# alenxav/bWGR

Measured on AMD Instinct MI355X. Metric: MCMC iter/sec (full marker sweep), higher is better.
Workload: dtype f32 scalars, fixed-point / f64 residual, int8 genotypes; 1 GPU; c4: synthetic n=10000 x p=1000000 int8, BayesB pi=0.99 (1.2% of the markers in the model at the last sweep), exact chain (blocked sweep, block=128, 40 slabs x 256 rows + 1 sequencer, the chain alone on the GPU: 80 streamers x 128 rows, engine generation 3, lag 12 blocks); n=10000, p=1000000, model=BayesB, df=5, chains=1

## Files before the change

### bwgr_amd/csrc/bwgr_hip.hip

```cpp
#include <hip/hip_runtime.h>
#include <stdint.h>
#include <stdio.h>
#include <stdarg.h>
#include <string.h>
#include <math.h>
#include <vector>
#include <random>
#include <chrono>
#include <algorithm>
#include <mutex>
#include <atomic>
#include <memory>
#include <utility>
#include <type_traits>
#include "../../include/bwgr.h"
#include "devbufs.h"
#include "traits.h"
#include "rng.hip.h"
#include "sweep.hip.h"
#include "sweep3.hip.h"
#include "sweep2w.hip.h"
#include "sweep3p.hip.h"
#include "mrr.hip.h"
#include "uvb.hip.h"
// ... 544 lines not shown
    const uint4 v0 = *reinterpret_cast<const uint4 *>(base + (size_t)j * R), v1 = *reinterpret_cast<const uint4 *>(base + (size_t)(j + 1) * R);
    const uint4 v2 = *reinterpret_cast<const uint4 *>(base + (size_t)(j + 2) * R), v3 = *reinterpret_cast<const uint4 *>(base + (size_t)(j + 3) * R);
    const double c0 = (double)coef[j], c1 = (double)coef[j + 1], c2 = (double)coef[j + 2], c3 = (double)coef[j + 3];
    GEMV_COL(v0, c0) GEMV_COL(v1, c1) GEMV_COL(v2, c2) GEMV_COL(v3, c3)
  }
  for (; j < jb; ++j) { const uint4 v0 = *reinterpret_cast<const uint4 *>(base + (size_t)j * R); const double c0 = (double)coef[j]; GEMV_COL(v0, c0) }
#undef GEMV_COL
#undef GEMV_ADD
  double *o = part + (int64_t)c * ld + i0;
#pragma unroll
  for (int k = 0; k < 16; ++k) o[k] = acc[k];
}
__global__ void k_hat_finish(const double *part, int64_t ld, int nchunks, int n, float MU, float *hat, const double *cen_off = nullptr) {
  const int i = blockIdx.x * blockDim.x + threadIdx.x;
  if (i >= n) return;
  double s = cen_off ? -*cen_off : 0.0;
  for (int c = 0; c < nchunks; ++c) s += part[(int64_t)c * ld + i];
  const float f = (float)s;
  hat[i] = f + MU;
}


struct WgrScalars {
  double mu, Ve, Va, Sb, Se, MSx, vy, bb, B0, VE, VA, sumD, cxx;
  double Vp, VP, Sk;
};
template <typename XT>
__global__ void k_stats64(const XT *X, int R, int n, int p, double *xx, double *vx) {
  const int lane = threadIdx.x & 63;
  const int64_t j = (int64_t)blockIdx.x * (blockDim.x >> 6) + (threadIdx.x >> 6);
  if (j >= p) return;
  double s1 = 0, s2 = 0;
  for (int i = lane; i < n; i += 64) { const double v = (double)xval(X, xoff(i, j, R, p)); s1 += v; s2 = fma(v, v, s2); }
  s1 = wave_sum(s1); s2 = wave_sum(s2);
  s1 = __shfl(s1, 0, 64); s2 = __shfl(s2, 0, 64);
  const double mean = s1 / (double)n;
  double sv = 0;
  for (int i = lane; i < n; i += 64) { const double dev = (double)xval(X, xoff(i, j, R, p)) - mean; sv = fma(dev, dev, sv); }
  sv = wave_sum(sv);
  if (lane == 0) { xx[j] = s2; vx[j] = sv / (double)(n - 1); }
}
__global__ void k_dsum_stage1(const double *v, int64_t n, double *part, int square) {
  __shared__ double red[17];
  double s = 0;
  for (int64_t i = (int64_t)blockIdx.x * blockDim.x + threadIdx.x; i < n; i += (int64_t)gridDim.x * blockDim.x) s += square ? v[i] * v[i] : v[i];
  s = block_sum(s, red);
  if (threadIdx.x == 0) part[blockIdx.x] = s;
}
__global__ void k_wgr_init(const double *y, double *eR, int n, int64_t ld, const double *part, const double *part2, int p,
                           double df, double R2, WgrScalars *ws) {
  __shared__ double red[17];
  double s = 0;
  for (int i = threadIdx.x; i < n; i += blockDim.x) s += y[i];
  s = block_sum(s, red);
  const double mu = s / (double)n;
  double sv = 0;
  for (int i = threadIdx.x; i < n; i += blockDim.x) { const double dev = y[i] - mu; sv += dev * dev; }
  sv = block_sum(sv, red);
  double ms = 0, sx = 0;
  for (int i = threadIdx.x; i < 256; i += blockDim.x) { ms += part[i]; sx += part2[i]; }
  ms = block_sum(ms, red);
  sx = block_sum(sx, red);
  for (int64_t i = threadIdx.x; i < ld; i += blockDim.x) eR[i] = (i < n) ? (y[i] - mu) : 0.0;
  if (threadIdx.x == 0) {
    WgrScalars w; memset(&w, 0, sizeof(w));
    w.mu = mu; w.vy = sv / (double)(n - 1); w.MSx = ms; w.Ve = 1.0; w.Va = ms;
    w.Sb = (R2) * df * w.vy / ms; w.Se = (1 - R2) * df * w.vy; w.cxx = sx / (double)p;
    w.Sk = R2 * w.vy * (df + 2); w.Vp = 1.0;
    *ws = w;
  }
}
__global__ void k_wgr_marker_init(double *bR, double *dR, double *VbR, double *LR, double *B, double *D, double *VB, int p, const WgrScalars *ws) {
  const double Va = ws->Va, Ve = ws->Ve;
  for (int j = blockIdx.x * blockDim.x + threadIdx.x; j < p; j += gridDim.x * blockDim.x) {
    bR[j] = 0; dR[j] = 1; VbR[j] = Va; LR[j] = Va / Ve; B[j] = 0; D[j] = 0; VB[j] = 0;
  }
}
__global__ void k_wgr_pre(const double *bR, const double *dR, const double *LR, const double *xx64, const double *eR, float *bf, float *df_,
                          float *Lf, float *xxf, double *e64, int p, int n, int64_t ld, float pi, const WgrScalars *ws, ChainScalars *sc) {
  const int64_t gid = (int64_t)blockIdx.x * blockDim.x + threadIdx.x, gsz = (int64_t)gridDim.x * blockDim.x;
  for (int64_t j = gid; j < p; j += gsz) { bf[j] = (float)bR[j]; df_[j] = (float)dR[j]; Lf[j] = (float)LR[j]; xxf[j] = (float)xx64[j]; }
  for (int64_t i = gid; i < ld; i += gsz) e64[i] = (i < n) ? (double)(float)eR[i] : 0.0;
  if (gid == 0) {
    ChainScalars c; memset(&c, 0, sizeof(c));
    const float Ve = (float)ws->Ve;
    c.ve = Ve; c.pi = pi; c.C = -0.5f / sqrtf(Ve); c.odds = pi / (1.0f - pi); c.dfp1 = 1.0f;
    c.inc_rate = 1.0f - pi;
    c.nredo = sc->nredo;
    *sc = c;
  }
}
__global__ void k_wgr_post(const float *bf, const float *df_, double *bR, double *dR, double *VbR, int p, int use_d, int iv, int de,
                           double dfv, uint32_t iter, Rng rng, const WgrScalars *ws) {
  const double Sb = ws->Sb, Ve = ws->Ve, MSx = ws->MSx;
  for (int j = blockIdx.x * blockDim.x + threadIdx.x; j < p; j += gridDim.x * blockDim.x) {
    const double b = (double)bf[j];
    bR[j] = b;
    if (use_d) dR[j] = (double)df_[j];
    if (iv) VbR[j] = de ? sqrt(b * b * Ve / MSx) : (Sb + b * b) / rng_chisq(rng, dfv + 1.0, (uint32_t)j, iter, RNG_CHI);
  }
}
__global__ __launch_bounds__(1024) void k_wgr_scal(const double *e64, int n, double n_dof, int p, const double *bbpart, int iv, double dfv, uint32_t iter, Rng rng, WgrScalars *ws) {
  __shared__ double red[17];
  double ee = 0;
  for (int i = threadIdx.x; i < n; i += blockDim.x) { const double v = (double)(float)e64[i]; ee += v * v; }
  ee = block_sum(ee, red);
  double bb = 0;
  for (int i = threadIdx.x; i < 256; i += blockDim.x) bb += bbpart[i];
  bb = block_sum(bb, red);
  if (threadIdx.x == 0) {
    if (!iv) ws->Va = (bb + ws->Sb) / rng_chisq(rng, dfv + (double)p, RNG_GLOBAL_MARKER, iter, RNG_G_VB);
    ws->Ve = (ee + ws->Se) / rng_chisq(rng, n_dof + dfv, RNG_GLOBAL_MARKER, iter, RNG_G_VE);
    ws->bb = bb;
  }
}
__global__ void k_wgr_L(const double *bR, const double *dR, double *VbR, double *LR, double *B, double *D, double *VB, int p, int iv, int accumulate, const WgrScalars *ws) {
  const double Ve = ws->Ve, Va = ws->Va;
  for (int j = blockIdx.x * blockDim.x + threadIdx.x; j < p; j += gridDim.x * blockDim.x) {
    if (!iv) VbR[j] = Va;
    LR[j] = Ve / VbR[j];
    if (accumulate) { B[j] += bR[j]; D[j] += dR[j]; if (iv) VB[j] += VbR[j]; }
  }
}
__global__ void k_wgr_efinish(const double *part, int64_t ld, int nchunks, int n, const double *y, double *eR, const WgrScalars *ws) {
  const int i = blockIdx.x * blockDim.x + threadIdx.x;
  if (i >= n) return;
  double s = 0;
  for (int c = 0; c < nchunks; ++c) s += part[(int64_t)c * ld + i];
  eR[i] = y[i] - ws->mu - s;
}
__global__ __launch_bounds__(1024) void k_wgr_mu(double *eR, int n, int iv, int accumulate, uint32_t iter, Rng rng, WgrScalars *ws) {
  __shared__ double red[17];
  double s = 0;
  for (int i = threadIdx.x; i < n; i += blockDim.x) s += eR[i];
  s = block_sum(s, red);
  const double mu0 = s / (double)n + (ws->Ve / (double)n) * rng_normal(rng, RNG_GLOBAL_MARKER, iter, RNG_G_MU, 0);
  for (int i = threadIdx.x; i < n; i += blockDim.x) eR[i] -= mu0;
  __syncthreads();
  if (threadIdx.x == 0) {
    ws->mu += mu0;
    if (accumulate) { ws->B0 += ws->mu; ws->VE += ws->Ve; if (!iv) ws->VA += ws->Va; }
  }
}
__global__ void k_wgr_pre_k(const double *hR, const double *Vd, const double *eR, float *hf, float *dhf, float *xxKf, float *Lkf, double *e64,
                            int pk, int n, int64_t ld, const WgrScalars *ws, ChainScalars *sc) {
  const int64_t gid = (int64_t)blockIdx.x * blockDim.x + threadIdx.x, gsz = (int64_t)gridDim.x * blockDim.x;
  const double Ve = ws->Ve, Vp = ws->Vp;
  for (int64_t k = gid; k < pk; k += gsz) { hf[k] = (float)hR[k]; dhf[k] = 0.0f; xxKf[k] = 1.0f; Lkf[k] = (float)(Ve / (Vd[k] * Vp)); }
  for (int64_t i = gid; i < ld; i += gsz) e64[i] = (i < n) ? (double)(float)eR[i] : 0.0;
  if (gid == 0) {
    ChainScalars c; memset(&c, 0, sizeof(c));
    const float Vef = (float)Ve;
    c.ve = Vef; c.pi = 0.0f; c.C = -0.5f / sqrtf(Vef); c.odds = 0.0f; c.dfp1 = 1.0f;
    *sc = c;
  }
}
__global__ void k_wgr_post_k(const float *hf, double *hR, const double *e64, double *eR, int pk, int n) {
  const int64_t gid = (int64_t)blockIdx.x * blockDim.x + threadIdx.x, gsz = (int64_t)gridDim.x * blockDim.x;
  for (int64_t k = gid; k < pk; k += gsz) hR[k] = (double)hf[k];
  for (int64_t i = gid; i < n; i += gsz) eR[i] = (double)(float)e64[i];
}
__global__ __launch_bounds__(1024) void k_wgr_vp(const double *hR, const double *Vd, int pk, double dfv, uint32_t iter, Rng rng, WgrScalars *ws) {
  __shared__ double red[17];
  double s = 0;
  for (int k = threadIdx.x; k < pk; k += blockDim.x) s += hR[k] * hR[k] / Vd[k];
  s = block_sum(s, red);
  if (threadIdx.x == 0) ws->Vp = (s + ws->Sk) / rng_chisq(rng, dfv + (double)pk, RNG_GLOBAL_MARKER, iter, RNG_G_VK);
}
__global__ void k_uh(const double *Ud, const double *coef, int n, int pk, double scale, double *out, int accumulate_into_neg) {
  const int i = blockIdx.x * blockDim.x + threadIdx.x;
  if (i >= n) return;
  double s = 0;
  for (int k = 0; k < pk; ++k) s = fma(Ud[(size_t)k * n + i], coef[k] * scale, s);
  if (accumulate_into_neg) out[i] -= s; else out[i] = s;
}
__global__ void k_wgr_accum_k(const double *hR, double *H, int pk, WgrScalars *ws) {
  for (int k = blockIdx.x * blockDim.x + threadIdx.x; k < pk; k += gridDim.x * blockDim.x) H[k] += hR[k];
  if (blockIdx.x == 0 && threadIdx.x == 0) ws->VP += ws->Vp;
}
__global__ void k_add_vec(double *a, const double *b, int n) {
  const int i = blockIdx.x * blockDim.x + threadIdx.x;
  if (i < n) a[i] += b[i];
}
template <typename XT>
__global__ void k_gather_rows(const XT *Xb, int Rb, const int *use, int nb, XT *Xo, int Ro, int64_t ldo, int64_t p) {
  const int64_t total = p * ldo;
  for (int64_t idx = (int64_t)blockIdx.x * blockDim.x + threadIdx.x; idx < total; idx += (int64_t)gridDim.x * blockDim.x) {
    const int64_t j = idx / ldo, i = idx - j * ldo;
    XT v = (XT)0;
    if (i < nb) v = Xb[xoff(use[i], j, Rb, p)];
    Xo[xoff(i, j, Ro, p)] = v;
  }
}
__global__ __launch_bounds__(256) void k_gather_rows_i8(const int8_t *Xb, int Rb, int64_t ldb, const int *use, int nb, int8_t *Xo, int Ro,
                                                         int64_t ldo, int64_t p, int mpw) {
  extern __shared__ __attribute__((aligned(16))) unsigned char col[];
  const int64_t j0 = (int64_t)blockIdx.x * mpw;
  const int nm = (int)min((int64_t)mpw, p - j0);
  const int cin = (int)(ldb / 16), cout = (int)(ldo / 16);
  for (int c = threadIdx.x; c < nm * cin; c += 256) {
    const int jj = c / cin, ci = c - jj * cin;
    const int64_t i = 16 * (int64_t)ci;
    reinterpret_cast<uint4 *>(col + (size_t)jj * ldb)[ci] = *reinterpret_cast<const uint4 *>(Xb + xoff(i, j0 + jj, Rb, p));
  }
  __syncthreads();
  for (int co = threadIdx.x; co < cout; co += 256) {
    int ui[16];
#pragma unroll
    for (int k = 0; k < 16; ++k) { const int i = 16 * co + k; ui[k] = (i < nb) ? use[i] : -1; }
    for (int jj = 0; jj < nm; ++jj) {
      const unsigned char *cj = col + (size_t)jj * ldb;
      uint32_t w[4];
#pragma unroll
      for (int q = 0; q < 4; ++q) {
        uint32_t v = 0;
#pragma unroll
        for (int k = 0; k < 4; ++k) { const int u = ui[4 * q + k]; v |= ((u >= 0) ? (uint32_t)cj[u] : 0u) << (8 * k); }
        w[q] = v;
      }
      *reinterpret_cast<uint4 *>(Xo + xoff(16 * (int64_t)co, j0 + jj, Ro, p)) = make_uint4(w[0], w[1], w[2], w[3]);
    }
  }
}
__global__ void k_gather_e(const double *eR, const int *use, int nb, int64_t ldo, double *e64) {
  for (int64_t i = (int64_t)blockIdx.x * blockDim.x + threadIdx.x; i < ldo; i += (int64_t)gridDim.x * blockDim.x)
    e64[i] = (i < nb) ? (double)(float)eR[use[i]] : 0.0;
}
__global__ void k_scale_d(double *v, int64_t n, double s) {
  for (int64_t i = (int64_t)blockIdx.x * blockDim.x + threadIdx.x; i < n; i += (int64_t)gridDim.x * blockDim.x) v[i] *= s;
}
__global__ void k_set_bg(ChainScalars *sc, float bg) { sc->bg = bg; }
__global__ void k_wgr_final(double *B, double *D, double *VB, int p, double mc, const double *dpart, int iv, WgrScalars *ws) {
  __shared__ double red[17];
  double sd = 0;
  for (int i = threadIdx.x; i < 256; i += blockDim.x) sd += dpart[i];
  sd = block_sum(sd, red);
  const double meanD = sd / mc / (double)p;
  for (int j = threadIdx.x; j < p; j += blockDim.x) { D[j] = D[j] / mc; B[j] = B[j] / mc / meanD; if (iv) VB[j] = VB[j] / mc; }
  if (threadIdx.x == 0) ws->sumD = sd;
}
__global__ void k_hat64_finish(const double *part, int64_t ld, int nchunks, int n, double B0, double *hat) {
  const int i = blockIdx.x * blockDim.x + threadIdx.x;
  if (i >= n) return;
  double s = 0;
  for (int c = 0; c < nchunks; ++c) s += part[(int64_t)c * ld + i];
  hat[i] = B0 + s;
}

__global__ void k_synth(int8_t *X, int64_t ld, int n, int64_t p, int64_t col0, uint32_t k0, uint32_t k1, float *freq) {
  const int64_t quads = ld / 4;
  const int64_t total = p * quads;
  for (int64_t idx = (int64_t)blockIdx.x * blockDim.x + threadIdx.x; idx < total; idx += (int64_t)gridDim.x * blockDim.x) {
    const int64_t j = idx / quads, q = idx - j * quads;
    const uint32_t jg = (uint32_t)(col0 + j);
    const uint4 fj = philox4x32_10(jg, 0u, 33u, 0u, k0, k1);
    const float f = 0.05f + 0.45f * ((float)(fj.x >> 8) * (1.0f / 16777216.0f));
    const uint32_t thr = (uint32_t)(f * 16777216.0f);
    if (q == 0 && freq) freq[j] = f;
    const uint4 a = philox4x32_10((uint32_t)q, jg, 32u, 0u, k0, k1);
    const uint4 c = philox4x32_10((uint32_t)q, jg, 32u, 1u, k0, k1);
    const uint32_t w[8] = {a.x, a.y, a.z, a.w, c.x, c.y, c.z, c.w};
    uint32_t packed = 0;
#pragma unroll
    for (int r = 0; r < 4; ++r) {
      uint32_t g = ((w[2 * r] >> 8) < thr) + ((w[2 * r + 1] >> 8) < thr);
      if (q * 4 + r >= n) g = 0;
      packed |= g << (8 * r);
    }
    *reinterpret_cast<uint32_t *>(X + j * ld + q * 4) = packed;
  }
}

__global__ void k_debug_variates(Rng g, int kind, double nu, uint32_t marker0, uint32_t iter, uint32_t purpose, int count, double *out) {
  const int i = blockIdx.x * blockDim.x + threadIdx.x;
  if (i >= count) return;
  const uint32_t mk = marker0 + (uint32_t)i;
  double v;
  if (kind == 0) v = rng_normal(g, mk, iter, purpose, 0);
  else if (kind == 1) v = rng_uniform(g, mk, iter, purpose, 0);
  else v = rng_chisq(g, nu, mk, iter, purpose);
  out[i] = v;
}

}

namespace {
struct SnapArgs { double *e, *se; float *b, *d, *vb, *sb, *sd, *svb; int64_t ld; int j0, j1; ChainScalars *sc; };
__global__ void k_range_snapshot(const SnapArgs s) {
  const int64_t nt = (int64_t)gridDim.x * blockDim.x, t0 = (int64_t)blockIdx.x * blockDim.x + threadIdx.x;
  for (int64_t i = t0; i < s.ld; i += nt) s.se[i] = s.e[i];
  for (int64_t j = s.j0 + t0; j < s.j1; j += nt) { s.sb[j] = s.b[j]; s.sd[j] = s.d[j]; if (s.vb) s.svb[j] = s.vb[j]; }
  if (t0 == 0) { s.sc->snap_sum_d = s.sc->sum_d; s.sc->snap_sum_b2 = s.sc->sum_b2; }
}
__global__ void k_range_recover(const SnapArgs s) {
  if (s.sc->error != 2u) return;
  const int64_t nt = (int64_t)gridDim.x * blockDim.x, t0 = (int64_t)blockIdx.x * blockDim.x + threadIdx.x;
  for (int64_t i = t0; i < s.ld; i += nt) s.e[i] = s.se[i];
  for (int64_t j = s.j0 + t0; j < s.j1; j += nt) { s.b[j] = s.sb[j]; s.d[j] = s.sd[j]; if (s.vb) s.vb[j] = s.svb[j]; }
}
__global__ void k_range_flag(ChainScalars *sc) {
  if (sc->error == 2u) { sc->error = 0u; sc->redo = 1u; sc->nredo += 1u; sc->sum_d = sc->snap_sum_d; sc->sum_b2 = sc->snap_sum_b2; }
}
__global__ void k_redo_clear(ChainScalars *sc) { sc->redo = 0u; }
}

struct Switches {
  int sweep = -1, lag = -1, solo3 = -1, stream3 = -1, pf3 = -1;
  int r3 = 0, d3 = 0, nfeed = 0, sh_add = 0, max_concurrent = 0, max_pairs = 0;
  float eng3_thr = 0.03f;
  bool occ_guard = true, pf3b = true, draws = true, gram16 = true;
  bool winv = true, wfx = true;
#ifdef BWGR_EXPERIMENTS
  bool fixed3 = false;
#else
  bool fixed3 = true;
#endif
  int wpf = 4, wahead = 5, wnq = 0, wlag_cap = 4;
  bool group_allow_uncentred = false, group_force_comm = false, em_debug = false;
  int64_t kchunk = 0;
#ifdef BWGR_EXPERIMENTS
  int dbg3 = 0, dbgw = 0, wlag_timing = 0; bool no_recover = false;
#endif
};
static Switches read_switches() {
  const auto chr = [](const char *v) { return v ? (int)(unsigned char)v[0] : -1; };
  const auto num = [](const char *v) { return v ? atoi(v) : 0; };
  Switches s;
  s.sweep = chr(getenv("BWGR_SWEEP")); s.lag = chr(getenv("BWGR_LAG")); s.solo3 = chr(getenv("BWGR_SOLO3"));
  s.stream3 = chr(getenv("BWGR_STREAM3")); s.pf3 = chr(getenv("BWGR_PF3"));
  s.r3 = num(getenv("BWGR_R3")); s.d3 = num(getenv("BWGR_D3")); s.nfeed = num(getenv("BWGR_NFEED")); s.sh_add = num(getenv("BWGR_DEBUG_SH_ADD"));
  s.max_concurrent = num(getenv("BWGR_MAX_CONCURRENT")); s.max_pairs = num(getenv("BWGR_MAX_PAIRS"));
  if (const char *v = getenv("BWGR_ENG3_THR")) { const float t = (float)atof(v); if (t > 0.0f) s.eng3_thr = t; }
  s.occ_guard = chr(getenv("BWGR_OCC_GUARD")) != '0'; s.pf3b = chr(getenv("BWGR_PF3B")) != '0'; s.draws = chr(getenv("BWGR_DRAWS")) != '0';
  s.gram16 = chr(getenv("BWGR_GRAM16")) != '0';
  { const int c = chr(getenv("BWGR_FIXED3")); if (c == '0') s.fixed3 = false; else if (c == '1') s.fixed3 = true; }
  s.winv = chr(getenv("BWGR_WINV")) != '0'; s.wfx = chr(getenv("BWGR_WFX")) != '0';
  if (const char *v = getenv("BWGR_WPF")) s.wpf = std::max(0, std::min(8, atoi(v)));
  if (const char *v = getenv("BWGR_WAHEAD")) s.wahead = std::max(1, atoi(v));
  { const int v = num(getenv("BWGR_WNQ")), c = chr(getenv("BWGR_WLAG")); if (v == 1 || v == 2 || v == 4) s.wnq = v; if (c >= '2' && c <= '6') s.wlag_cap = c - '0'; }
  s.group_allow_uncentred = chr(getenv("BWGR_GROUP_ALLOW_UNCENTRED")) == '1'; s.group_force_comm = chr(getenv("BWGR_GROUP_FORCE_COMM")) == '1';
  s.em_debug = getenv("BWGR_EM_DEBUG") != nullptr;
  if (const char *v = getenv("BWGR_KCHUNK")) s.kchunk = std::max<long long>(0, atoll(v));
#ifdef BWGR_EXPERIMENTS
  s.dbg3 = num(getenv("BWGR_DBG3")); s.dbgw = num(getenv("BWGR_DBGW")); s.wlag_timing = num(getenv("BWGR_WLAG_TIMING"));
  s.no_recover = getenv("BWGR_NO_RECOVER") != nullptr;
#endif
  return s;
}

enum PanelKind { PANEL_MAIN = 0, PANEL_ROWS = 1, PANEL_EM = 2 };
struct PanelPlan {
  int m = 0, K = 0, R = 0;
  int64_t ld = 0, nblocks = 0;
  int pstride = 0, nfeed = 2;
  bool lag4_ok = false;
  size_t lds = 0, lds2 = 0, ldsw = 0;
  size_t x_bytes = 0, gram_bytes = 0;
  bool pipelined = false;
  int xdist = 1;
  bool has16 = false;
  int wdist = 0;
  bool try3 = false;
};
template <typename XT> static int max_slab_rows(int m) {
  int best = 0;
  for (int R = 128; R <= 4096; R += 128)
    if (sweep_lds_bytes<XT>(m, R) <= (size_t)160 * 1024 && (size_t)m * R * sizeof(XT) <= (size_t)SW_TCH * 16 * (SW_THREADS - 64)) best = R;
  return best;
}
static int panel_range(int64_t n, int64_t p) {
  if (n < 2 || p < 1) return fail(BWGR_EINVAL, "panel: need n >= 2, p >= 1 (n=%lld p=%lld)", (long long)n, (long long)p);
  if (n > 0x7FFFFF00ll || p > 0x7FFFFF00ll) return fail(BWGR_EINVAL, "panel: n and p must fit 31 bits");
  return BWGR_OK;
}
static int plan_panel(PanelPlan &pl, bool is_f32, int64_t n, int64_t p, int block, int nwg, PanelKind kind, const Switches &sw) {
  pl = PanelPlan();
  CHK(panel_range(n, p));
  const auto lds2_of = [&](int m, int R) { return is_f32 ? sweep2_lds_bytes<float>(m, R) : sweep2_lds_bytes<int8_t>(m, R); };
  const int mmax = is_f32 ? 64 : SW_MAXM;
  int m = block > 0 ? block : mmax;
  if (m > mmax) return fail(BWGR_EINVAL, "panel_create: block %d > %d (limit for this genotype type)", m, mmax);
  m = ((int)std::min<int64_t>(m, ((p + 15) / 16) * 16) + 15) / 16 * 16;
  const int Rmax = is_f32 ? max_slab_rows<float>(m) : max_slab_rows<int8_t>(m);
  int Rpick = Rmax, R2 = 0;
  for (int Rt = 128; Rt <= Rmax; Rt += 128)
    if (lds2_of(m, Rt) <= (size_t)160 * 1024 && (is_f32 || (size_t)m * Rt <= S2I_TILE_BYTES_MAX)) R2 = Rt;
  if (sw.sweep != '1' && R2 > 0 && (n + R2 - 1) / R2 + 1 + 6 <= 256) Rpick = R2;
  const int K = nwg > 0 ? nwg : (int)((n + Rpick - 1) / Rpick);
  const int R = (int)((((n + K - 1) / K) + 127) / 128) * 128;
  if (K > 256 || R > Rmax) return fail(BWGR_EINVAL, "panel_create: n=%lld needs %d slab workgroups of %d rows (limits: 256 workgroups, %d rows)", (long long)n, K, R, Rmax);
  pl.m = m; pl.K = K; pl.R = R; pl.ld = (int64_t)K * R;
  pl.nblocks = (p + m - 1) / m;
  if (pl.nblocks >= (1ll << 24)) return fail(BWGR_EINVAL, "panel_create: %lld marker blocks; the delta granules carry a 24-bit block epoch", (long long)pl.nblocks);
  pl.pstride = ((m * (m - 1) / 2 + 7) / 8) * 8;
  pl.lds = is_f32 ? sweep_lds_bytes<float>(m, R) : sweep_lds_bytes<int8_t>(m, R);
  pl.lds2 = lds2_of(m, R);
  pl.lag4_ok = !is_f32 && s2i_lds_bytes(m, R, 4) <= (size_t)160 * 1024;
  if (pl.lag4_ok) pl.lds2 = std::max(pl.lds2, s2i_lds_bytes(m, R, 4));
#ifdef BWGR_EXPERIMENTS
  if (!is_f32) pl.ldsw = s2w_lds_bytes(m, R, sw.wlag_timing ? sw.wlag_timing : 6);
#else
  if (!is_f32) pl.ldsw = s2w_lds_bytes(m, R, 6);
#endif
  pl.nfeed = std::min(6, std::max(2, (K + 39) / 40 + 1));
  if (sw.nfeed >= 1 && sw.nfeed <= 6) pl.nfeed = sw.nfeed;
  pl.pipelined = sw.sweep != '1' && pl.lds2 <= (size_t)160 * 1024 && K + 1 + pl.nfeed <= 256 && (is_f32 || (size_t)m * R <= S2I_TILE_BYTES_MAX);
  pl.x_bytes = (size_t)pl.ld * (size_t)p * (is_f32 ? 4 : 1);
  pl.gram_bytes = (size_t)pl.nblocks * m * m * (is_f32 ? 8 : 4);
  if (pl.pipelined && kind != PANEL_EM) {
    if (pl.nblocks > 2) pl.xdist = 2;
    if (!is_f32 && pl.nblocks > 3 && pl.lag4_ok && sw.lag != '2' && sw.lag != '3') pl.xdist = 3;
    pl.has16 = !is_f32;
  }
  if (pl.has16 && sw.winv && m <= SW_MAXM)
    for (int d = 1; d <= S2W_MAXDIST && d < pl.nblocks; ++d) {
      if (d <= S2W_NEARD ? d > pl.xdist : (kind != PANEL_MAIN || d > sw.wlag_cap - 1)) break;
      pl.wdist = d;
    }
  pl.try3 = kind == PANEL_MAIN && !is_f32 && pl.pipelined && sw.sweep != '2';
  return BWGR_OK;
}

struct Panel3Plan {
  bool fits = false;
  int R3 = 0, sub3 = 0, K3 = 0;
  int D = 0;
  size_t lds3 = 0;
  bool solo3 = true;
};
static Panel3Plan plan_panel3(const PanelPlan &pp, const Switches &sw, bool gram16) {
  Panel3Plan q;
  if (!pp.try3) return q;
  q.R3 = (pp.R % 256 == 0) ? 256 : 128;
  if ((sw.r3 == 64 || sw.r3 == 128 || sw.r3 == 256) && pp.R % sw.r3 == 0) { q.R3 = sw.r3; q.solo3 = false; }
  q.sub3 = pp.R / q.R3; q.K3 = pp.K * q.sub3;
  q.D = 12;
  if (sw.d3 >= 2 && sw.d3 <= S3_MAXD) q.D = sw.d3;
  q.D = (int)std::min<int64_t>(q.D, std::max<int64_t>(2, pp.nblocks));
  q.lds3 = std::max(std::max(s3_streamer_lds(q.R3), std::max(s3_streamer_dma_lds(128), q.R3 == 256 ? s3_streamer_dma_lds(256) : (size_t)0)), s3_seq_lds(q.D, gram16));
  q.fits = q.K3 <= 255 && q.lds3 <= (size_t)160 * 1024 && (size_t)pp.m * q.R3 <= (size_t)4 * 16 * SW_THREADS;
  if (q.fits && sw.solo3 >= 0) q.solo3 = sw.solo3 != '0';
  return q;
}

extern "C" int bwgr_debug_panel_plan(int is_f32, int64_t n, int64_t p, int block, int nwg, int kind, int xmax, int gram16, int64_t out[BWGR_PANEL_PLAN_NOUT]) {
  if (!out || kind < PANEL_MAIN || kind > PANEL_EM) return fail(BWGR_EINVAL, "debug_panel_plan: null pointer or bad kind");
  const Switches sw = read_switches();
  PanelPlan pl;
  CHK(plan_panel(pl, is_f32 != 0, n, p, block, nwg, (PanelKind)kind, sw));
  const Panel3Plan q = xmax >= 0 ? plan_panel3(pl, sw, gram16 != 0) : Panel3Plan();
  const int64_t v[BWGR_PANEL_PLAN_NOUT] = {pl.m, pl.K, pl.R, pl.ld, pl.nblocks, pl.pstride, pl.nfeed, pl.lag4_ok, (int64_t)pl.lds, (int64_t)pl.lds2, (int64_t)pl.ldsw,
                                           (int64_t)pl.x_bytes, (int64_t)pl.gram_bytes, pl.pipelined, pl.xdist, pl.has16, pl.wdist, pl.try3,
                                           q.fits, q.R3, q.sub3, q.K3, q.D, (int64_t)q.lds3, q.solo3};
  std::copy(v, v + BWGR_PANEL_PLAN_NOUT, out);
  return BWGR_OK;
}

namespace {
struct HipBackend {
  using stream_t = hipStream_t;
  using event_t = hipEvent_t;
  static inline std::atomic<int64_t> live[3];
  static inline thread_local hipError_t last = hipSuccess;
  static void *alloc(size_t bytes) {
    void *q = nullptr;
    const hipError_t e = hipMalloc(&q, bytes);
    if (e != hipSuccess) { last = e; (void)hipGetLastError(); return nullptr; }
    ++live[0];
    return q;
  }
  static void free(void *q) { (void)hipFree(q); --live[0]; }
  static bool stream_create(hipStream_t *s, unsigned flags, int priority) {
    if ((priority ? hipStreamCreateWithPriority(s, flags, priority) : hipStreamCreateWithFlags(s, flags)) != hipSuccess) { (void)hipGetLastError(); return false; }
    ++live[1];
    return true;
  }
  static void stream_sync(hipStream_t s) { (void)hipStreamSynchronize(s); }
  static void stream_destroy(hipStream_t s) { (void)hipStreamDestroy(s); --live[1]; }
  static bool event_create(hipEvent_t *e, unsigned flags) {
    if (hipEventCreateWithFlags(e, flags) != hipSuccess) { (void)hipGetLastError(); return false; }
    ++live[2];
    return true;
  }
  static void event_destroy(hipEvent_t e) { (void)hipEventDestroy(e); --live[2]; }
};
using DevBufs = DevHolder<HipBackend>;
template <typename F> struct Guard {
  F f;
  bool armed = true;
  explicit Guard(F f_) : f(f_) {}
  Guard(const Guard &) = delete;
  ~Guard() { if (armed) f(); }
  void release() { armed = false; }
};
}
extern "C" int bwgr_debug_live(int64_t out[3]) {
  if (!out) return fail(BWGR_EINVAL, "debug_live: null pointer");
  for (int i = 0; i < 3; ++i) out[i] = HipBackend::live[i].load();
  return BWGR_OK;
}
static int no_memory(const char *who) { return fail(BWGR_ENOMEM, "%s: device allocation failed (%s)", who, hipGetErrorString(HipBackend::last)); }
template <typename T> static int own_array(DevBufs &own, T *&ptr, size_t count, const char *who) {
  return (ptr = own.get<std::conditional_t<std::is_void<T>::value, unsigned char, T>>(count)) ? BWGR_OK : no_memory(who);
}

struct PanelData {
  DevBufs own;
  int device = 0, is_f32 = 0;
  int64_t n = 0, p = 0;
  PanelPlan plan;
  Panel3Plan plan3;
  float MSx = 0;
  int xmax = 0;
  bool gram16 = false;
  int winv_nd = 0;
  bool e3_ready = false;
  bool crowded = false;
  void *X = nullptr, *gram = nullptr, *gramp = nullptr;
  void *gx[S2W_NEARD + 1] = {};
  uint16_t *gramp16 = nullptr, *gramx16 = nullptr;
  int *gram16_bad = nullptr;
  void *g3x[S3_MAXD] = {};
  unsigned char *gx12 = nullptr;
  unsigned char *gxt[S2W_MAXDIST] = {};
  float *xx = nullptr, *vx = nullptr, *msx_dev = nullptr;
  int *xmax_dev = nullptr;
  bool cen = false;
  int32_t *csum = nullptr; float *xxc = nullptr;
  Switches sw;
  int nclones = 0;
  int nchains_all = 0;
  std::vector<hipStream_t> pair_streams;
};

struct bwgr_panel {
  PanelData *data = nullptr;
  bool is_root = false;
  DevBufs own;
  hipStream_t stream = nullptr;
  hipStream_t pre_pair_stream = nullptr; bool pre_pair_set = false;
  double *xspec2 = nullptr, *xspec3 = nullptr;
  PreStage ps = {};
  const void *ps_owner = nullptr; int ps_iter = -1;
  double *xpart = nullptr, *qpart = nullptr;
  unsigned long long *dgran = nullptr;
  uint32_t *xflags = nullptr;
  unsigned char *xchg = nullptr; size_t xchg_bytes = 0;
  unsigned long long *stamps = nullptr;
  unsigned long long *qsum3 = nullptr, *lists3 = nullptr;
  uint32_t epoch3 = 0;
  double *snap_e = nullptr; float *snap_b = nullptr, *snap_d = nullptr, *snap_vb = nullptr;
  double *winv = nullptr;
  unsigned long long *qsumw = nullptr;
  double *cpre = nullptr;
  double *draws = nullptr; hipStream_t draws_stream = nullptr; hipEvent_t draws_ready = nullptr, draws_free = nullptr;
  bool draws_valid = false; Rng draws_rng = {}; uint32_t draws_iter = 0, draws_marker0 = 0; int draws_flags = 0, draws_j0 = 0, draws_j1 = 0; const void *draws_sc = nullptr;
  hipEvent_t guard_ev = nullptr; int guard_cus = 0; hipStream_t guard_stream = nullptr; bool guard_listed = false;
  bool force3 = false;
  int debug_withhold = 0;
  int nchains = 0;
};

struct bwgr_chain {
  bwgr_panel *P = nullptr;
  DevBufs own;
  int model = 0, iit = 0, ibi = 0, done = 0, rng_mode = 0;
  float itf = 0, bif = 0, pi = 0, df = 0, R2 = 0, Phi = 0;
  uint64_t seed = 0;
  float *y = nullptr, *b = nullptr, *d = nullptr, *vb = nullptr, *lam = nullptr;
  double *e = nullptr;
  float *B = nullptr, *D = nullptr, *VB = nullptr;
  ChainScalars *sc = nullptr;
  int64_t marker0 = 0, p_total = 0;
  float MSx_eff = 0;
  double *e0 = nullptr;
  int flags_extra = 0;
  std::vector<hipEvent_t> ev;
  float ms_acc = 0; int launch_acc = 0;
  bool finalized = false;
};

__attribute__((constructor)) static void bwgr_more_hw_queues() { setenv("GPU_MAX_HW_QUEUES", "8", 0); }

static hipError_t d2h(hipStream_t st, void *dst, const void *src, size_t bytes) {
  hipError_t e = hipMemcpyAsync(dst, src, bytes, hipMemcpyDeviceToHost, st);
  return e != hipSuccess ? e : hipStreamSynchronize(st);
}
template <typename T> static hipError_t h2d(hipStream_t st, T *dst, const T *src, size_t count) { return hipMemcpyAsync(dst, src, sizeof(T) * count, hipMemcpyHostToDevice, st); }
template <typename T> static hipError_t zero(hipStream_t st, T *dst, size_t count) { return hipMemsetAsync(dst, 0, sizeof(T) * count, st); }

static Rng make_rng(uint64_t seed, int mode) {
  Rng g; g.k0 = (uint32_t)seed; g.k1 = (uint32_t)(seed >> 32); g.degenerate = (mode == BWGR_RNG_DEGENERATE); return g;
}

static int sum_floats(hipStream_t st, const float *v, int64_t n, double *part, float *sum_dev, float *sum) {
  hipLaunchKernelGGL(k_sum_stage1, dim3(256), dim3(256), 0, st, v, n, part);
  hipLaunchKernelGGL(k_sum_stage2, dim3(1), dim3(256), 0, st, part, 256, sum_dev);
  HIPCHK(hipGetLastError());
  HIPCHK(d2h(st, sum, sum_dev, sizeof(float)));
  return BWGR_OK;
}

static int refuse_centred(const char *who) {
  return fail(BWGR_EINVAL, "%s: this panel sweeps implicitly centred columns (bwgr_panel_set_centred), which only the fused chains do; call bwgr_panel_set_centred(P, 0) first", who);
}

static int require_device(int device) {
  int c = 0; bwgr_device_count(&c);
  if (c <= 0) return fail(BWGR_ENODEV, "no HIP device visible: libbwgr_hip has no CPU fallback");
  if (device < 0 || device >= c) return fail(BWGR_EINVAL, "device %d out of range (%d visible)", device, c);
  hipDeviceProp_t prop;
  HIPCHK(hipGetDeviceProperties(&prop, device));
  if (strncmp(prop.gcnArchName, "gfx950", 6) != 0)
    return fail(BWGR_ENODEV, "device %d is %s; this library is built for gfx950 (MI355X) only", device, prop.gcnArchName);
  HIPCHK(hipSetDevice(device));
  return BWGR_OK;
}

static int alloc_exchange(bwgr_panel *P) {
  const size_t K = (size_t)P->data->plan.K;
  const size_t fb = (sizeof(uint32_t) * (K + 1) * SW_FLAG_STRIDE + 255) & ~(size_t)255;
  const size_t gb = (sizeof(unsigned long long) * S2_NSLOT * SW_MAXM + 255) & ~(size_t)255;
  const size_t qb = sizeof(double) * S2_NSLOT * (K + 1) * SW_MAXM;
  P->xchg_bytes = fb + gb + qb;
  CHK(own_array(P->own, P->xchg, P->xchg_bytes, "panel scratch"));
  P->xflags = reinterpret_cast<uint32_t *>(P->xchg);
  P->dgran = reinterpret_cast<unsigned long long *>(P->xchg + fb);
  P->qpart = reinterpret_cast<double *>(P->xchg + fb + gb);
  return BWGR_OK;
}
struct SpinLaunch { const void *fn; int grid, resident, threads; size_t lds; };
struct SweepPlan {
  int engine = 1;
  float gate3 = 0.0f;
  int lag = 2, nfeed = 0;
  bool g16 = false;
  int R3 = 0, K3 = 0, sub = 0, pf = -1, pf2 = -1, dbg3 = 0, qsplit = 0, skip_vb = 0;
  bool fixed3 = false;
  int fx = 0, nd = 0, npf = 0, ahead = 0, nq = 0, wsub = 0, wK3 = 0;
  bool guarded = false;
  bool draws = false;
  int nspins = 0; SpinLaunch spins[3];
};
static void spin_launch(const SpinLaunch &L, hipStream_t st, void **args) { (void)hipLaunchKernel(L.fn, dim3(L.grid), dim3(L.threads), args, L.lds, st); }

static std::mutex g_guard_mu;
static std::vector<bwgr_panel *> g_guard_panels;
static int occupancy_fits(int grid, int per_cu, int cus, int busy, int *need) {
  if (need) *need = 0;
  if (grid < 1 || cus < 1 || busy < 0) return BWGR_EINVAL;
  if (per_cu < 1) return BWGR_EINVAL;
  const int nd = (grid + per_cu - 1) / per_cu;
  if (need) *need = nd;
  return (nd + busy <= cus) ? BWGR_OK : BWGR_EINVAL;
}
extern "C" int bwgr_debug_occupancy_fits(int grid, int per_cu, int cus, int busy, int *need) { return occupancy_fits(grid, per_cu, cus, busy, need); }
static int guard_per_cu(const SpinLaunch &L) {
  static std::mutex mu; static std::vector<std::pair<SpinLaunch, int>> cache;
  std::lock_guard<std::mutex> lk(mu);
  for (auto &c : cache) if (c.first.fn == L.fn && c.first.threads == L.threads && c.first.lds == L.lds) return c.second;
  int nb = 0;
  if (hipOccupancyMaxActiveBlocksPerMultiprocessor(&nb, L.fn, L.threads, L.lds) != hipSuccess) { (void)hipGetLastError(); nb = 0; }
  cache.push_back({L, nb});
  return nb;
}
static int device_cus(int device) {
  static std::mutex mu; static std::vector<int> cus;
  std::lock_guard<std::mutex> lk(mu);
  if ((int)cus.size() <= device) cus.resize(device + 1, 0);
  if (!cus[device]) { hipDeviceProp_t prop; if (hipGetDeviceProperties(&prop, device) == hipSuccess) cus[device] = prop.multiProcessorCount; else (void)hipGetLastError(); }
  return cus[device];
}
static int plan_cus(const SweepPlan &pl, int cus, int busy, int *need_out) {
  int need = 0;
  for (int i = 0; i < pl.nspins; ++i) {
    const SpinLaunch &L = pl.spins[i];
    const int per = guard_per_cu(L);
    int nd = 0;
    if (per < 1) return fail(BWGR_EINVAL, "occupancy guard: a sweep kernel (%d threads, %zu bytes of LDS) does not fit a compute unit", L.threads, L.lds);
    if (occupancy_fits(L.resident, per, cus, busy, &nd) != BWGR_OK)
      return fail(BWGR_EINVAL, "occupancy guard: a sweep launch of %d workgroups (%d per compute unit) needs %d compute units; %d of %d are held by other handles' sweeps "
                  "in flight (their workgroups wait for one another, so all must be resident at once: run fewer chains side by side -- bwgr_panel_max_concurrent -- or "
                  "wait for the others)", L.resident, per, nd, busy, cus);
    need = std::max(need, nd);
  }
  *need_out = need;
  return BWGR_OK;
}
static int guard_busy(const bwgr_panel *P, hipStream_t mine, const bwgr_panel *partner = nullptr) {
  std::vector<std::pair<hipStream_t, int>> per_stream;
  for (bwgr_panel *Q : g_guard_panels) {
    if (Q == P || Q == partner || Q->data->device != P->data->device || Q->guard_cus == 0) continue;
    if (hipEventQuery(Q->guard_ev) == hipSuccess) { Q->guard_cus = 0; continue; }
    (void)hipGetLastError();
    if (Q->guard_stream == mine) continue;
    bool seen = false;
    for (auto &ps : per_stream) if (ps.first == Q->guard_stream) { ps.second = std::max(ps.second, Q->guard_cus); seen = true; }
    if (!seen) per_stream.push_back({Q->guard_stream, Q->guard_cus});
  }
  int busy = 0;
  for (auto &ps : per_stream) busy += ps.second;
  return busy;
}
static int sweep_guard(const bwgr_panel *P, const SweepPlan &pl, hipStream_t st, const bwgr_panel *partner, int *need) {
  *need = 0;
  if (!P->data->sw.occ_guard) return BWGR_OK;
  const int cus = device_cus(P->data->device);
  if (cus < 1) return BWGR_OK;
  std::lock_guard<std::mutex> lk(g_guard_mu);
  return plan_cus(pl, cus, guard_busy(P, st, partner), need);
}
static void guard_mark(bwgr_panel *P, hipStream_t st, int need) {
  if (need <= 0) return;
  std::lock_guard<std::mutex> lk(g_guard_mu);
  if (!P->guard_ev) { if (hipEventCreateWithFlags(&P->guard_ev, hipEventDisableTiming) != hipSuccess) { (void)hipGetLastError(); P->guard_ev = nullptr; return; } }
  if (!P->guard_listed) { g_guard_panels.push_back(P); P->guard_listed = true; }
  if (P->guard_cus > 0 && P->guard_stream == st && hipEventQuery(P->guard_ev) != hipSuccess) { (void)hipGetLastError(); need = std::max(need, P->guard_cus); }
  P->guard_cus = need; P->guard_stream = st;
  (void)hipEventRecord(P->guard_ev, st);
}
static void guard_forget(bwgr_panel *P) {
  std::lock_guard<std::mutex> lk(g_guard_mu);
  for (size_t i = 0; i < g_guard_panels.size(); ++i) if (g_guard_panels[i] == P) { g_guard_panels.erase(g_guard_panels.begin() + i); break; }
  if (P->guard_ev) { (void)hipEventDestroy(P->guard_ev); P->guard_ev = nullptr; }
  P->guard_listed = false; P->guard_cus = 0;
}

static int reset_exchange(bwgr_panel *P) {
  if (P->data->plan.pipelined) {
    HIPCHK(hipMemsetAsync(P->xchg, 0, P->xchg_bytes, P->stream));
  } else if (P->data->plan.K > 1) {
    HIPCHK(hipMemsetAsync(P->xflags, 0, sizeof(uint32_t) * ((size_t)P->data->plan.K + 1) * SW_FLAG_STRIDE, P->stream));
  }
  return BWGR_OK;
}

static void launch_gram(bwgr_panel *P, void *g, int dist);
static int sweep3_build(bwgr_panel *P) {
  PanelData *D = P->data; const PanelPlan &pl = D->plan;
  D->e3_ready = false;
  D->plan3 = plan_panel3(pl, D->sw, D->gram16);
  if (!D->plan3.fits) return BWGR_OK;
  const int m = pl.m; const bool g16 = D->gram16;
  const size_t blk_elems = (size_t)pl.nblocks * m * m;
  int bad = 0;
  std::vector<void *> far;
  {
    DevBufs bufs;
    int32_t *tmp = nullptr;
    for (int d = 1; d < D->plan3.D && d < pl.nblocks; ++d) {
      void *have32 = d <= pl.xdist ? D->gx[d] : nullptr, *have = g16 ? (d == 1 ? (void *)D->gramx16 : nullptr) : have32;
      if (have) { D->g3x[d - 1] = have; continue; }
      void *arr = nullptr;
      CHK(own_array(D->own, arr, blk_elems * (g16 ? 2 : 4), "panel_create"));
      D->g3x[d - 1] = arr; far.push_back(arr);
      if (g16) {
        if (!have32) {
          if (!tmp && !(tmp = bufs.get<int32_t>(blk_elems))) return fail(BWGR_ENOMEM, "panel_create: device allocation failed");
          launch_gram(P, tmp, d);
          have32 = tmp;
        }
        hipLaunchKernelGGL(k_gram_narrow, dim3(2048), dim3(256), 0, P->stream, (const int32_t *)have32 + (size_t)d * m * m, (uint16_t *)arr + (size_t)d * m * m, (int64_t)(pl.nblocks - d) * m * m, D->gram16_bad);
      } else launch_gram(P, arr, d);
      HIPCHK(hipGetLastError());
    }
    if (g16) HIPCHK(hipMemcpyAsync(&bad, D->gram16_bad, sizeof(int), hipMemcpyDeviceToHost, P->stream));
    HIPCHK(hipStreamSynchronize(P->stream));
  }
  if (bad) {
    for (void *q : far) D->own.drop(q);
    for (void *&g : D->g3x) g = nullptr;
    return BWGR_OK;
  }
  if (g16) {
    CHK(own_array(D->own, D->gx12, (size_t)pl.nblocks * m * 2 * m * 2, "panel_create"));
    hipLaunchKernelGGL(k_near_rows, dim3(4096), dim3(256), 0, P->stream, (const uint16_t *)D->g3x[0], (const uint16_t *)(D->plan3.D >= 3 ? D->g3x[1] : nullptr), (uint16_t *)D->gx12, m, (int64_t)pl.nblocks);
    HIPCHK(hipGetLastError());
  }
  for (const void *f : {reinterpret_cast<const void *>(k_sweep3<uint16_t, false>), reinterpret_cast<const void *>(k_sweep3<int32_t, false>), reinterpret_cast<const void *>(k_sweep3<uint16_t, true>),
                        reinterpret_cast<const void *>(k_sweep3<int32_t, true>), reinterpret_cast<const void *>(k_sweep3p<uint16_t>), reinterpret_cast<const void *>(k_sweep3p<int32_t>),
                        reinterpret_cast<const void *>(k_sweep3f)})
    HIPCHK(hipFuncSetAttribute(f, hipFuncAttributeMaxDynamicSharedMemorySize, 160 * 1024));
  D->e3_ready = true;
  return BWGR_OK;
}
static bool stream3_dma_fits(int64_t ncols, int64_t R) { return ncols >= 0 && R > 0 && (uint64_t)ncols * (uint64_t)R < (1ull << 32); }
extern "C" int bwgr_debug_stream3_dma(int64_t ncols, int64_t R) { return stream3_dma_fits(ncols, R) ? 1 : 0; }
static int winv_alloc(bwgr_panel *P) {
  const size_t nb = (size_t)P->data->plan.nblocks;
  if (!P->winv && !P->own.take({{&P->winv, sizeof(double) * S2W_WDOUBLES * nb}, {&P->qsumw, sizeof(unsigned long long) * 4 * 2 * SW_MAXM * nb}}))
    return no_memory("affine sweep");
  return BWGR_OK;
}

static void launch_prestage(bwgr_panel *P, const SweepArgs &a_in, const SweepPlan &pl) {
  SweepArgs a = a_in;
  a.gate3 = pl.gate3;
  const int j0 = a.blk_begin * a.m, j1 = (int)std::min<int64_t>(P->data->p, (int64_t)a.blk_end * a.m);
  const int64_t tasks = 4ll * (j1 - j0);
  const bool s3 = a.gate3 > 0.0f;
  const bool fxa = pl.engine == 4 && pl.fx;
  const int sh_add = P->data->sw.sh_add;
  int xbits = 0; while ((1 << xbits) < std::max(1, P->data->xmax)) ++xbits;
  if (s3 || fxa) hipLaunchKernelGGL(k_escale_reset, dim3(1), dim3(1), 0, P->stream, a.sc);
  const int dflags = a.flags & (SWF_SELECT | SWF_VB_VEC);
  const bool have_draws = P->draws_valid && P->draws_iter == a.iter && P->draws_marker0 == a.marker0 && P->draws_flags == dflags &&
                          P->draws_sc == (const void *)a.sc && P->draws_j0 <= j0 && P->draws_j1 >= j1 && memcmp(&P->draws_rng, &a.rng, sizeof(Rng)) == 0 &&
                          !(a.flags & (SWF_MH | SWF_EM_ANY));
  a.draws = nullptr;
  if (have_draws) { const hipError_t he = hipStreamWaitEvent(P->stream, P->draws_ready, 0); if (he == hipSuccess) a.draws = P->draws; else { fprintf(stderr, "bwgr: draws wait failed: %s\n", hipGetErrorString(he)); (void)hipGetLastError(); } }
  if (a.draws) {
    hipLaunchKernelGGL(k_prestage_fin, dim3((unsigned)std::min<int64_t>(2048, (j1 - j0 + 255) / 256)), dim3(256), 0, P->stream, a, j0, j1);
    { const hipError_t he = hipEventRecord(P->draws_free, P->stream); if (he != hipSuccess) { fprintf(stderr, "bwgr: draws_free record failed: %s\n", hipGetErrorString(he)); (void)hipGetLastError(); } }
    P->draws_valid = false;
  } else hipLaunchKernelGGL(k_prestage, dim3((unsigned)std::min<int64_t>(4096, (tasks + 255) / 256)), dim3(256), 0, P->stream, a, j0, j1);
  if (s3) {
    hipLaunchKernelGGL(k_escale, dim3(1), dim3(1024), 0, P->stream, a.e, P->data->plan.ld, a.sc, xbits, a.gate3, sh_add);
    if (a.flags & SWF_CENTRE) {
      hipLaunchKernelGGL(k_cen_tot, dim3((unsigned)(a.blk_end - a.blk_begin)), dim3(128), 0, P->stream, a, a.blk_begin, 0);
      hipLaunchKernelGGL(k_cen_scan, dim3(1), dim3(1024), 0, P->stream, a, (int)P->data->plan.nblocks, 0);
    }
    hipLaunchKernelGGL(k_spec3, dim3((unsigned)(a.blk_end - a.blk_begin)), dim3(128), 0, P->stream, a, a.blk_begin, P->data->gram16 ? (const uint16_t *)P->data->gramp16 : (const uint16_t *)nullptr);
    if (std::isinf(a.gate3)) return;
  }
  if (pl.engine == 4) {
    if (pl.fx) hipLaunchKernelGGL(k_escale, dim3(1), dim3(1024), 0, P->stream, a.e, P->data->plan.ld, a.sc, xbits, INFINITY, sh_add);
    hipLaunchKernelGGL(k_affine_inv, dim3((unsigned)(a.blk_end - a.blk_begin)), dim3(512), S2W_INV_LDS, P->stream, a, P->winv, (a.flags & SWF_DELTA2) ? 2.0 : 1.0);
    return;
  }
  if (P->data->plan.pipelined) {
    const int sel = (a.flags & SWF_SELECT) ? 1 : 0;
    const unsigned nb = (unsigned)(a.blk_end - a.blk_begin);
    if ((a.flags & SWF_CENTRE) && sel) {
      hipLaunchKernelGGL(k_cen_tot, dim3(nb), dim3(128), 0, P->stream, a, a.blk_begin, 1);
      hipLaunchKernelGGL(k_cen_scan, dim3(1), dim3(1024), 0, P->stream, a, (int)P->data->plan.nblocks, 1);
    }
    if (P->data->is_f32) hipLaunchKernelGGL(k_spec<double>, dim3(nb), dim3(128), 0, P->stream, a, a.blk_begin, sel);
    else hipLaunchKernelGGL(k_spec<int32_t>, dim3(nb), dim3(128), 0, P->stream, a, a.blk_begin, sel);
  }
}

static void draws_ahead(bwgr_panel *P, const SweepArgs &a, const SweepPlan &pl, hipEvent_t before_sweep) {
  if (!pl.draws) return;
  if (!P->draws) {
    int lo = 0, hi = 0;
    (void)hipDeviceGetStreamPriorityRange(&lo, &hi);
    if (hipFuncSetAttribute(reinterpret_cast<const void *>(k_draws), hipFuncAttributeMaxDynamicSharedMemorySize, 96 * 1024) != hipSuccess) { (void)hipGetLastError(); return; }
    if (!P->own.take({{&P->draws, sizeof(double) * 5 * (size_t)P->data->p}, DevBufs::want_stream(&P->draws_stream, hipStreamNonBlocking, lo),
                      DevBufs::want_event(&P->draws_ready, hipEventDisableTiming), DevBufs::want_event(&P->draws_free, hipEventDisableTiming)})) return;
    (void)hipEventRecord(P->draws_free, P->stream);
  }
  const int j0 = a.blk_begin * a.m, j1 = (int)std::min<int64_t>(P->data->p, (int64_t)a.blk_end * a.m);
  { const hipError_t h1 = hipStreamWaitEvent(P->draws_stream, P->draws_free, 0), h2 = hipStreamWaitEvent(P->draws_stream, before_sweep, 0);
    if (h1 != hipSuccess || h2 != hipSuccess) { fprintf(stderr, "bwgr: draws_ahead waits failed: %s / %s\n", hipGetErrorString(h1), hipGetErrorString(h2)); (void)hipGetLastError(); return; } }
  hipLaunchKernelGGL(k_draws, dim3(160), dim3(1024), 96 * 1024, P->draws_stream, a.rng, a.marker0, a.iter + 1u, a.flags, (const ChainScalars *)a.sc, (int64_t)P->data->p, j0, j1, P->draws);
  { const hipError_t h1 = hipGetLastError(); const hipError_t h2 = (h1 == hipSuccess) ? hipEventRecord(P->draws_ready, P->draws_stream) : hipSuccess;
    if (h1 != hipSuccess || h2 != hipSuccess) { fprintf(stderr, "bwgr: k_draws launch / record failed: %s / %s\n", hipGetErrorString(h1), hipGetErrorString(h2)); (void)hipGetLastError(); P->draws_valid = false; return; } }
  P->draws_valid = true; P->draws_rng = a.rng; P->draws_iter = a.iter + 1u; P->draws_marker0 = a.marker0; P->draws_flags = a.flags & (SWF_SELECT | SWF_VB_VEC);
  P->draws_j0 = j0; P->draws_j1 = j1; P->draws_sc = (const void *)a.sc;
}

static SweepPlan plan_sweep(const bwgr_panel *P, const SweepArgs &a, bool redo) {
  SweepPlan pl;
  const Switches &sw = P->data->sw;
  const bool sel = (a.flags & SWF_SELECT) != 0, cen = (a.flags & SWF_CENTRE) != 0;
  const auto spin = [&](const void *fn, int grid, int resident, int threads, size_t lds) { pl.spins[pl.nspins++] = SpinLaunch{fn, grid, resident, threads, lds}; };
  if (P->data->e3_ready && sel && !(a.flags & SWF_EM_ANY) && !redo) pl.gate3 = (sw.eng3_thr >= 1.0f || P->force3) ? INFINITY : sw.eng3_thr;
  const bool winv = sw.winv && P->data->plan.pipelined && !P->data->is_f32 && P->data->winv_nd >= 1 && P->data->plan.K <= 2 * (S2W_QW + S2W_QX) &&
                    !(a.flags & (SWF_SELECT | SWF_EM_ANY | SWF_SERIAL)) && P->data->plan.ldsw > 0 && P->data->plan.ldsw <= (size_t)160 * 1024;
  const bool wfx = sw.wfx && (P->data->plan.R % S2W_FXR) == 0 && P->data->plan.K * (P->data->plan.R / S2W_FXR) <= 255;
  pl.engine = pl.gate3 > 0.0f ? 3 : winv ? 4 : P->data->plan.pipelined ? 2 : 1;
  int lag = 2;
  if (P->data->plan.pipelined && sel) {
    if (P->data->plan.xdist >= 2 && (sw.lag >= 0 || P->data->gram16)) lag = 3;
    if (P->data->plan.xdist >= 3 && P->data->gram16) lag = 4;
  }
  pl.lag = std::min(lag, (sw.lag >= '2' && sw.lag <= '4') ? sw.lag - '0' : 3);
  if (winv) {
    pl.lag = std::min(P->data->winv_nd + 1, sw.wlag_cap);
    if (!wfx) pl.lag = std::min(pl.lag, 4);
#ifdef BWGR_EXPERIMENTS
    if (sw.wlag_timing) pl.lag = sw.wlag_timing;
#endif
  }
  pl.nfeed = (P->data->plan.pipelined && sel) ? P->data->plan.nfeed : 0;
  pl.g16 = P->data->plan.pipelined && P->data->gram16 && sel;
  const bool alone = P->data->plan3.solo3 && !P->data->crowded && P->is_root && P->data->nclones == 0;
  pl.draws = sel && !(a.flags & (SWF_MH | SWF_EM_ANY)) && alone && sw.draws;
  if (pl.gate3 > 0.0f) {
    pl.R3 = P->data->plan3.R3; pl.sub = P->data->plan3.sub3; pl.K3 = P->data->plan3.K3;
#ifdef BWGR_EXPERIMENTS
    pl.dbg3 = sw.dbg3;
#endif
    {
      const int64_t j_lo = (int64_t)a.blk_begin * a.m, j_hi = std::min<int64_t>(P->data->p, (int64_t)a.blk_end * a.m);
      const bool fits32 = stream3_dma_fits(j_hi - j_lo, P->data->plan.R);
      if (sw.stream3 != 'r' && fits32) pl.dbg3 |= (1 << 22);
      if (sw.stream3 == 'd' && fits32) pl.dbg3 |= (1 << 23);
    }
    if (P->force3) {
      const size_t lds = std::max(s3p_streamer_lds(pl.R3), s3_seq_lds(P->data->plan3.D, P->data->gram16));
      spin(P->data->gram16 ? reinterpret_cast<const void *>(k_sweep3p<uint16_t>) : reinterpret_cast<const void *>(k_sweep3p<int32_t>), pl.K3 + 2, pl.K3 + 2, SW_THREADS, lds);
      return pl;
    }
    if (alone && pl.R3 == 256 && 2 * pl.K3 + 1 <= 256) { pl.R3 = 128; pl.sub = P->data->plan.R / 128; pl.K3 = P->data->plan.K * pl.sub; }
    const bool pf_on = (sw.pf3 >= 0 ? sw.pf3 == '1' : alone) && pl.K3 + 2 <= 256;
    pl.pf = pf_on ? ((pl.K3 + 2 > 8) ? 8 : pl.K3 + 1) : -1;
    const bool pf2_on = pf_on && pl.pf == 8 && P->data->gram16 && P->data->gx12 && pl.K3 + 3 > 16 && pl.K3 + 3 <= 256 && sw.pf3b;
    pl.pf2 = pf2_on ? 16 : -1; pl.qsplit = 1; pl.skip_vb = (a.flags & SWF_VB_VEC) ? 1 : 0;
    const int grid = pl.K3 + 1 + (pf_on ? 1 : 0) + (pf2_on ? 1 : 0);
    const void *fn = P->data->gram16 ? (cen ? reinterpret_cast<const void *>(k_sweep3<uint16_t, true>) : reinterpret_cast<const void *>(k_sweep3<uint16_t, false>))
                                  : (cen ? reinterpret_cast<const void *>(k_sweep3<int32_t, true>) : reinterpret_cast<const void *>(k_sweep3<int32_t, false>));
    pl.fixed3 = sw.fixed3 && P->data->gram16 && !cen && P->data->gx12 && P->data->plan.m == S3Shape128::m && P->data->plan.pstride == S3Shape128::pstride &&
                pl.R3 == 128 && (pl.dbg3 & (3 << 22)) == (1 << 22) && pl.qsplit == 1 && !P->debug_withhold;
    spin(pl.fixed3 ? reinterpret_cast<const void *>(k_sweep3f) : fn, grid, grid, SW_THREADS, P->data->plan3.lds3);
  }
  if (!std::isinf(pl.gate3)) {
    if (winv) {
      pl.fx = (wfx && !redo) ? 1 : 0;
      if (!pl.fx) pl.lag = std::min(pl.lag, 4);
      pl.nd = std::min(pl.lag - 1, (int)S2W_MAXDIST);
      pl.npf = sw.wpf; pl.ahead = sw.wahead;
      pl.wsub = P->data->plan.R / S2W_FXR; pl.wK3 = P->data->plan.K * pl.wsub;
      pl.nq = sw.wnq ? sw.wnq : (pl.wK3 > 48 ? 2 : 1);
      const int wgs = pl.fx ? pl.wK3 : P->data->plan.K;
      spin(pl.fx ? reinterpret_cast<const void *>(k_sweep2w<true>) : reinterpret_cast<const void *>(k_sweep2w<false>), wgs + 1 + 8 * pl.npf, wgs + 1 + pl.npf, S2W_THREADS, P->data->plan.ldsw);
    } else if (P->data->plan.pipelined) {
      const void *fn = P->data->is_f32 ? (sel ? reinterpret_cast<const void *>(k_sweep2<float, true>) : reinterpret_cast<const void *>(k_sweep2<float, false>))
                       : pl.g16  ? reinterpret_cast<const void *>(k_sweep2<int8_t, true, uint16_t>)
                       : sel     ? reinterpret_cast<const void *>(k_sweep2<int8_t, true>) : reinterpret_cast<const void *>(k_sweep2<int8_t, false>);
      spin(fn, P->data->plan.K + 1 + pl.nfeed, P->data->plan.K + 1 + pl.nfeed, SW_THREADS, P->data->plan.lds2);
    } else {
      const void *fn = P->data->is_f32 ? (sel ? reinterpret_cast<const void *>(k_sweep<float, true>) : reinterpret_cast<const void *>(k_sweep<float, false>))
                                 : (sel ? reinterpret_cast<const void *>(k_sweep<int8_t, true>) : reinterpret_cast<const void *>(k_sweep<int8_t, false>));
      spin(fn, P->data->plan.K, P->data->plan.K, SW_THREADS, P->data->plan.lds);
    }
  }
#ifdef BWGR_EXPERIMENTS
  const bool no_recover = sw.no_recover;
#else
  constexpr bool no_recover = false;
#endif
  if (!redo && (pl.gate3 > 0.0f || (winv && wfx)) && !P->debug_withhold && !no_recover) {
    const SweepPlan r = plan_sweep(P, a, true);
    for (int i = 0; i < r.nspins; ++i) pl.spins[pl.nspins++] = r.spins[i];
    pl.guarded = true;
  }
  return pl;
}

static void sweep3_args(bwgr_panel *P, const SweepArgs &a, const SweepPlan &pl, Sweep3Args &A) {
  memset(&A, 0, sizeof(A)); A.a = a;
  for (int d = 0; d < S3_MAXD; ++d) A.gx[d] = P->data->g3x[d];
  A.gp = P->data->gram16 ? (const void *)P->data->gramp16 : P->data->gramp;
  A.D = P->data->plan3.D; A.K3 = pl.K3; A.R3 = pl.R3; A.sub = pl.sub; A.g16 = P->data->gram16 ? 1 : 0;
  A.qsum = P->qsum3; A.lists = P->lists3;
  A.gx12 = P->data->gram16 ? P->data->gx12 : nullptr;
  A.dbg = pl.dbg3; A.pf = pl.pf; A.pf2 = pl.pf2; A.qsplit = pl.qsplit; A.skip_vb = pl.skip_vb;
  P->epoch3 = (P->epoch3 + 1) & 0xFFFFFFu; if (P->epoch3 == 0) P->epoch3 = 1;
  A.epoch = P->epoch3;
  (void)hipMemsetAsync(P->qsum3 + (size_t)a.blk_begin * 2 * SW_MAXM, 0, sizeof(unsigned long long) * 2 * SW_MAXM * (size_t)(a.blk_end - a.blk_begin), P->stream);
}
static void launch_sweep_engine(bwgr_panel *P, const SweepArgs &a_in, const SweepPlan &pl, bool redo) {
  SweepArgs a = a_in;
  if (P->debug_withhold) a.flags |= SWF_DEBUG_WITHHOLD;
  a.gate3 = pl.gate3; a.redo_only = redo ? 1 : 0;
  const bool sel = (a.flags & SWF_SELECT) != 0;
  if (redo && pl.engine == 2) {
    if ((a.flags & SWF_CENTRE) && sel) {
      SweepArgs all = a; all.blk_begin = 0; all.blk_end = (int)P->data->plan.nblocks;
      hipLaunchKernelGGL(k_cen_tot, dim3((unsigned)P->data->plan.nblocks), dim3(128), 0, P->stream, all, 0, 2);
      hipLaunchKernelGGL(k_cen_scan, dim3(1), dim3(1024), 0, P->stream, all, (int)P->data->plan.nblocks, 2);
    }
    hipLaunchKernelGGL(k_spec<int32_t>, dim3((unsigned)(a.blk_end - a.blk_begin)), dim3(128), 0, P->stream, a, a.blk_begin, sel ? 1 : 0);
  }
  if (a.gate3 > 0.0f) {
    Sweep3Args A3;
    sweep3_args(P, a, pl, A3);
    const bool cen = (a.flags & SWF_CENTRE) != 0;
    if (cen) hipLaunchKernelGGL(k_cen_begin, dim3(1), dim3(1024), 0, P->stream, a, 0);
    void *args[] = {&A3};
    spin_launch(pl.spins[0], P->stream, args);
    if (cen) hipLaunchKernelGGL(k_cen_end, dim3(64), dim3(256), 0, P->stream, a, 0);
    if (pl.skip_vb) {
      const int j0 = a.blk_begin * a.m, j1 = (int)std::min<int64_t>(P->data->p, (int64_t)a.blk_end * a.m);
      hipLaunchKernelGGL(k_vb_fill, dim3((unsigned)std::min<int64_t>(1024, (j1 - j0 + 255) / 256)), dim3(256), 0, P->stream, a, j0, j1);
    }
    if (std::isinf(a.gate3)) return;
  }
  const SpinLaunch &L = pl.spins[a.gate3 > 0.0f ? 1 : 0];
  a.nfeed = pl.nfeed; a.lag = pl.lag;
  if (pl.engine == 4) {
    S2WArgs A; memset(&A, 0, sizeof(A));
    A.winv = P->winv; A.qsum = P->qsumw; A.fx = pl.fx; A.nd = pl.nd; A.npf = pl.npf; A.ahead = pl.ahead; A.sub = pl.wsub; A.K3 = pl.wK3; A.nq = pl.nq;
#ifdef BWGR_EXPERIMENTS
    A.dbg = P->data->sw.dbgw;
#endif
    for (int d = 0; d < S2W_MAXDIST; ++d) A.gxt[d] = P->data->gxt[d < P->data->winv_nd ? d : 0];
    if (A.fx) (void)hipMemsetAsync(P->qsumw + (size_t)a.blk_begin * A.nq * 2 * SW_MAXM, 0, sizeof(unsigned long long) * A.nq * 2 * SW_MAXM * (size_t)(a.blk_end - a.blk_begin), P->stream);
    void *args[] = {&a, &A}; spin_launch(L, P->stream, args);
    return;
  }
  const bool cen2 = P->data->plan.pipelined && (a.flags & SWF_CENTRE) && sel && !P->data->is_f32;
  if (cen2) hipLaunchKernelGGL(k_cen_begin, dim3(1), dim3(1024), 0, P->stream, a, redo ? 2 : 1);
  SweepArgs ak = a;
  if (pl.g16) { ak.gramp = P->data->gramp16; ak.gramx = P->data->gramx16; }
  void *args[] = {&ak}; spin_launch(L, P->stream, args);
  if (cen2) hipLaunchKernelGGL(k_cen_end, dim3(64), dim3(256), 0, P->stream, a, redo ? 2 : 1);
}
static void launch_sweep_kernel(bwgr_panel *P, const SweepArgs &a, const SweepPlan &pl) {
  const size_t p = (size_t)P->data->p;
  bool guarded = pl.guarded;
  if (guarded && !P->snap_e && !P->own.take({{&P->snap_e, sizeof(double) * (size_t)P->data->plan.ld}, {&P->snap_b, sizeof(float) * p}, {&P->snap_d, sizeof(float) * p}, {&P->snap_vb, sizeof(float) * p}})) guarded = false;
  SnapArgs sn;
  sn.e = a.e; sn.se = P->snap_e; sn.b = a.b; sn.d = a.d; sn.vb = (a.flags & SWF_VB_VEC) ? a.vb : nullptr; sn.sb = P->snap_b; sn.sd = P->snap_d; sn.svb = P->snap_vb;
  sn.ld = P->data->plan.ld; sn.j0 = a.blk_begin * a.m; sn.j1 = (int)std::min<int64_t>(P->data->p, (int64_t)a.blk_end * a.m); sn.sc = a.sc;
  if (guarded) hipLaunchKernelGGL(k_range_snapshot, dim3(256), dim3(256), 0, P->stream, sn);
  launch_sweep_engine(P, a, pl, false);
  if (guarded) {
    hipLaunchKernelGGL(k_range_recover, dim3(256), dim3(256), 0, P->stream, sn);
    hipLaunchKernelGGL(k_range_flag, dim3(1), dim3(1), 0, P->stream, a.sc);
    (void)reset_exchange(P);
    launch_sweep_engine(P, a, plan_sweep(P, a, true), true);
    hipLaunchKernelGGL(k_redo_clear, dim3(1), dim3(1), 0, P->stream, a.sc);
  }
}

static int leave_pair_stream(bwgr_panel *P) {
  if (!P->pre_pair_set) return BWGR_OK;
  hipEvent_t ev;
  HIPCHK(hipEventCreateWithFlags(&ev, hipEventDisableTiming));
  hipError_t he = hipEventRecord(ev, P->stream);
  if (he == hipSuccess) he = hipStreamWaitEvent(P->pre_pair_stream, ev, 0);
  (void)hipEventDestroy(ev);
  if (he != hipSuccess) return fail(BWGR_EHIP, "leaving the pair stream: %s", hipGetErrorString(he));
  P->stream = P->pre_pair_stream; P->pre_pair_set = false;
  return BWGR_OK;
}
static int sweep_begin(bwgr_panel *P, SweepArgs &a, SweepPlan &pl, int *need) {
  CHK(leave_pair_stream(P));
  pl = plan_sweep(P, a, false); a.lag = pl.lag;
  if (pl.engine == 4) CHK(winv_alloc(P));
  CHK(sweep_guard(P, pl, P->stream, nullptr, need));
  return reset_exchange(P);
}
static int launch_sweep(bwgr_panel *P, SweepArgs &a) {
  SweepPlan pl; int need = 0;
  CHK(sweep_begin(P, a, pl, &need));
  P->ps_owner = nullptr;
  launch_prestage(P, a, pl);
  launch_sweep_kernel(P, a, pl);
  HIPCHK(hipGetLastError());
  guard_mark(P, P->stream, need);
  return BWGR_OK;
}

static void fill_panel_args(const bwgr_panel *P, SweepArgs &a) {
  a.X = P->data->X; a.ld = P->data->plan.ld; a.gram = P->data->gram;
  a.n = (int)P->data->n; a.p = (int)P->data->p; a.m = P->data->plan.m; a.K = P->data->plan.K; a.R = P->data->plan.R;
  a.blk_begin = 0; a.blk_end = (int)P->data->plan.nblocks;
  a.xpart = P->xpart; a.xflags = P->xflags; a.stamps = P->stamps; a.ps = P->ps;
  a.gramx = P->data->gx[1]; a.gramx2 = P->data->gx[2]; a.xspec2 = P->xspec2; a.gramx3 = P->data->gx[3]; a.xspec3 = P->xspec3; a.lag = 2; a.nfeed = P->data->plan.nfeed; a.gramp = P->data->gramp; a.pstride = P->data->plan.pstride; a.qpart = P->qpart; a.dgran = P->dgran;
}

template <typename ST, typename XT>
static int upload(bwgr_panel *P, const void *X, int memloc, int64_t ldx) {
  const int64_t n = P->data->n, p = P->data->p;
  XT *dst = reinterpret_cast<XT *>(P->data->X);
  if (memloc == BWGR_DEVICE) {
    hipLaunchKernelGGL((k_convert<ST, XT>), dim3(4096), dim3(256), 0, P->stream, reinterpret_cast<const ST *>(X), ldx, dst, P->data->plan.ld, (int)n, (int64_t)0, p, P->data->plan.R, p);
    HIPCHK(hipGetLastError());
    return BWGR_OK;
  }
  const int64_t col_bytes = ldx * (int64_t)sizeof(ST);
  int64_t cols = std::max<int64_t>(1, ((int64_t)256 << 20) / std::max<int64_t>(1, col_bytes));
  cols = std::min(cols, p);
  DevBufs bufs;
  ST *stage = bufs.get<ST>((size_t)(cols * ldx));
  if (!stage) return fail(BWGR_ENOMEM, "panel_create: device allocation failed");
  for (int64_t j0 = 0; j0 < p; j0 += cols) {
    const int64_t nc = std::min(cols, p - j0);
    const size_t bytes = (size_t)((nc - 1) * col_bytes + n * (int64_t)sizeof(ST));
    HIPCHK(hipMemcpyAsync(stage, reinterpret_cast<const ST *>(X) + j0 * ldx, bytes, hipMemcpyHostToDevice, P->stream));
    hipLaunchKernelGGL((k_convert<ST, XT>), dim3(2048), dim3(256), 0, P->stream, stage, ldx, dst, P->data->plan.ld, (int)n, j0, nc, P->data->plan.R, p);
    HIPCHK(hipStreamSynchronize(P->stream));
  }
  return BWGR_OK;
}

static int scratch_alloc(bwgr_panel *P) {
  const PanelData *D = P->data;
  const size_t nb = (size_t)D->plan.nblocks;
  const char *who = "panel scratch";
  if (D->plan.xdist >= 2) CHK(own_array(P->own, P->xspec2, nb * SW_MAXM, who));
  if (D->plan.xdist >= 3) CHK(own_array(P->own, P->xspec3, nb * SW_MAXM, who));
  if (D->plan.pipelined) CHK(own_array(P->own, P->ps.quick, nb, who));
  if (!P->own.take({{&P->ps.spec, sizeof(SpecBuf) * nb}, {&P->ps.blocks, sizeof(StageBuf) * nb}, {&P->xpart, sizeof(double) * 2 * (size_t)D->plan.K * SW_MAXM}})) return no_memory(who);
  CHK(alloc_exchange(P));
#if defined(BWGR_STAMPS) || defined(BWGR_EXPERIMENTS)
  CHK(own_array(P->own, P->stamps, 256, who));
  HIPCHK(hipMemset(P->stamps, 0, sizeof(unsigned long long) * 256));
#endif
  if (D->e3_ready) {
    if (!P->own.take({{&P->qsum3, sizeof(unsigned long long) * 2 * SW_MAXM * nb}, {&P->lists3, sizeof(unsigned long long) * S3_LSTRIDE * nb}})) return no_memory(who);
    HIPCHK(hipMemsetAsync(P->lists3, 0, sizeof(unsigned long long) * S3_LSTRIDE * nb, P->stream));
  }
  return BWGR_OK;
}

extern "C" int bwgr_panel_destroy(bwgr_panel *P) {
  if (!P) return BWGR_OK;
  PanelData *D = P->data;
  if (P->is_root && D->nclones > 0) return fail(BWGR_EINVAL, "panel_destroy: %d clone(s) of this panel are still alive", D->nclones);
  if (P->nchains > 0) return fail(BWGR_EINVAL, "panel_destroy: %d chain(s) on this panel are still alive (destroy them first)", P->nchains);
  (void)hipSetDevice(D->device);
  guard_forget(P);
  const bool root = P->is_root;
  delete P;
  if (root) delete D;
  else D->nclones--;
  return BWGR_OK;
}

static int panel_measure(bwgr_panel *P) {
  PanelData *D = P->data;
  const int p = (int)D->p, n = (int)D->n, wpb = 4;
  if (D->is_f32) hipLaunchKernelGGL(k_stats<float>, dim3((p + wpb - 1) / wpb), dim3(64 * wpb), 0, P->stream, (const float *)D->X, D->plan.R, n, p, D->xx, D->vx);
  else hipLaunchKernelGGL(k_stats<int8_t>, dim3((p + wpb - 1) / wpb), dim3(64 * wpb), 0, P->stream, (const int8_t *)D->X, D->plan.R, n, p, D->xx, D->vx);
  HIPCHK(hipGetLastError());
  {
    DevBufs bufs;
    double *part = bufs.get<double>(256);
    if (!part) return fail(BWGR_ENOMEM, "panel_create: device allocation failed");
    CHK(sum_floats(P->stream, D->vx, (int64_t)p, part, D->msx_dev, &D->MSx));
  }
  if (!D->is_f32) {
    if (!D->xmax_dev) CHK(own_array(D->own, D->xmax_dev, 1, "panel_create"));
    HIPCHK(hipMemsetAsync(D->xmax_dev, 0, sizeof(int), P->stream));
    hipLaunchKernelGGL(k_absmax_i8, dim3(2048), dim3(256), 0, P->stream, (const int8_t *)D->X, D->plan.x_bytes, D->xmax_dev);
    HIPCHK(hipGetLastError());
    HIPCHK(hipMemcpyAsync(&D->xmax, D->xmax_dev, sizeof(int), hipMemcpyDeviceToHost, P->stream));
    HIPCHK(hipStreamSynchronize(P->stream));
  }
  return BWGR_OK;
}

template <int MAXTJ, typename F> static void with_tj(int tj, F f) {
  if constexpr (MAXTJ > 1) { if (tj < MAXTJ) return with_tj<MAXTJ - 1>(tj, f); }
  f(std::integral_constant<int, MAXTJ>());
}
static void launch_gram(bwgr_panel *P, void *g, int dist) {
  const PanelPlan &pl = P->data->plan;
  const int p = (int)P->data->p, m = pl.m, R = pl.R, tiles = dist ? 2 : 1;
  const dim3 grid((unsigned)(pl.nblocks - dist)), block(256);
  const int64_t ld = pl.ld; hipStream_t st = P->stream;
  const size_t ldsf = (size_t)tiles * m * 65 * sizeof(float), ldsi = (size_t)tiles * m * 33 * sizeof(int32_t);
  const float *Xf = (const float *)P->data->X; double *gd = (double *)g;
  const int8_t *Xi = (const int8_t *)P->data->X; int32_t *gi = (int32_t *)g;
  const bool f32 = P->data->is_f32 != 0;
  if (!f32 && m == 128) hipLaunchKernelGGL(k_gram_mfma_i8, grid, block, 0, st, Xi, ld, R, p, gi, dist);
  else if (!f32 && dist) with_tj<8>(m / 16, [&](auto tj) { hipLaunchKernelGGL(k_gramx_i8<decltype(tj)::value>, grid, block, ldsi, st, Xi, ld, R, p, m, gi, dist); });
  else if (f32 && !dist) with_tj<4>(m / 16, [&](auto tj) { hipLaunchKernelGGL(k_gram_f32<decltype(tj)::value>, grid, block, ldsf, st, Xf, ld, R, p, m, gd); });
  else if (!dist) with_tj<8>(m / 16, [&](auto tj) { hipLaunchKernelGGL(k_gram_i8<decltype(tj)::value>, grid, block, ldsi, st, Xi, ld, R, p, m, gi); });
  else with_tj<4>(m / 16, [&](auto tj) { hipLaunchKernelGGL(k_gramx_f32<decltype(tj)::value>, grid, block, ldsf, st, Xf, ld, R, p, m, gd, dist); });
}

static int gram_range(bool is_f32, int64_t rows, int xmax) {
  const int64_t xm = std::max(xmax, 1);
  if (!is_f32 && rows * xm * xm >= (1ll << 31)) return fail(BWGR_EINVAL, "panel: n * max|x|^2 = %lld does not fit the int32 Gram", (long long)(rows * xm * xm));
  return BWGR_OK;
}
static int panel_build_gram(bwgr_panel *P) {
  PanelData *D = P->data; const PanelPlan &pl = D->plan;
  const int m = pl.m;
  CHK(gram_range(D->is_f32 != 0, D->n, D->xmax));
  launch_gram(P, D->gram, 0);
  HIPCHK(hipGetLastError());
  for (int dist = 1; dist <= pl.xdist && dist < pl.nblocks; ++dist) {
    launch_gram(P, D->gx[dist], dist);
    HIPCHK(hipGetLastError());
  }
  if (D->is_f32) hipLaunchKernelGGL(k_gram_pack<double>, dim3((unsigned)pl.nblocks), dim3(256), 0, P->stream, (const double *)D->gram, (double *)D->gramp, m, pl.pstride, pl.nblocks);
  else hipLaunchKernelGGL(k_gram_pack<int32_t>, dim3((unsigned)pl.nblocks), dim3(256), 0, P->stream, (const int32_t *)D->gram, (int32_t *)D->gramp, m, pl.pstride, pl.nblocks);
  HIPCHK(hipGetLastError());
  D->gram16 = false;
  if (pl.has16) {
    HIPCHK(hipMemsetAsync(D->gram16_bad, 0, sizeof(int), P->stream));
    hipLaunchKernelGGL(k_gram_narrow, dim3(2048), dim3(256), 0, P->stream, (const int32_t *)D->gramp, D->gramp16, (int64_t)pl.nblocks * pl.pstride, D->gram16_bad);
    if (pl.nblocks > 1)
      hipLaunchKernelGGL(k_gram_narrow, dim3(2048), dim3(256), 0, P->stream, (const int32_t *)D->gx[1] + (size_t)m * m, D->gramx16 + (size_t)m * m, (int64_t)(pl.nblocks - 1) * m * m, D->gram16_bad);
    HIPCHK(hipGetLastError());
    int bad = 1;
    HIPCHK(hipMemcpyAsync(&bad, D->gram16_bad, sizeof(int), hipMemcpyDeviceToHost, P->stream));
    HIPCHK(hipStreamSynchronize(P->stream));
    D->gram16 = (bad == 0) && D->sw.gram16;
  }
  D->winv_nd = 0;
  if (D->gram16 && pl.wdist > 0) {
    HIPCHK(hipMemsetAsync(D->gram16_bad, 0, sizeof(int), P->stream));
    int nd = 0;
    DevBufs bufs;
    int32_t *tmpx = nullptr;
    for (int dist = 1; dist <= pl.wdist; ++dist) {
      if (dist > S2W_NEARD) {
        if (!tmpx && !(tmpx = bufs.get<int32_t>((size_t)pl.nblocks * m * m))) { (void)hipGetLastError(); break; }
        launch_gram(P, tmpx, dist);
      }
      const int32_t *src = dist > S2W_NEARD ? tmpx : (const int32_t *)D->gx[dist];
      if (!D->gxt[dist - 1]) CHK(own_array(D->own, D->gxt[dist - 1], (size_t)pl.nblocks * S2W_PBYTES, "panel_create"));
      hipLaunchKernelGGL(k_gx_planes, dim3(4096), dim3(256), 0, P->stream, src, D->gxt[dist - 1], m, (int64_t)pl.nblocks, dist, D->gram16_bad);
      HIPCHK(hipGetLastError());
      nd = dist;
    }
    int bad = 1;
    HIPCHK(hipMemcpyAsync(&bad, D->gram16_bad, sizeof(int), hipMemcpyDeviceToHost, P->stream));
    HIPCHK(hipStreamSynchronize(P->stream));
    D->winv_nd = bad ? 0 : nd;
  }
  HIPCHK(hipStreamSynchronize(P->stream));
  return BWGR_OK;
}

static int panel_setup(bwgr_panel *P) {
  CHK(panel_measure(P));
  CHK(panel_build_gram(P));
  return sweep3_build(P);
}

static int panel_alloc(bwgr_panel **out, int is_f32, int64_t n, int64_t p, int device, int block, int nwg, PanelKind kind, const Switches &sw) {
  *out = nullptr;
  CHK(panel_range(n, p));
  CHK(require_device(device));
  PanelPlan pl;
  CHK(plan_panel(pl, is_f32 != 0, n, p, block, nwg, kind, sw));
  bwgr_panel *P = new bwgr_panel();
  PanelData *D = P->data = new PanelData(); P->is_root = true;
  Guard drop([&] { bwgr_panel_destroy(P); });
  D->device = device; D->n = n; D->p = p; D->is_f32 = is_f32; D->sw = sw; D->plan = pl;
  const size_t packed = (size_t)pl.nblocks * std::max(pl.pstride, 8);
  if (!D->own.take({{&D->X, pl.x_bytes}, {&D->gram, pl.gram_bytes}, {&D->gramp, packed * (is_f32 ? 8 : 4)}, {&D->xx, sizeof(float) * p}, {&D->vx, sizeof(float) * p}, {&D->msx_dev, sizeof(float)}}))
    return no_memory("panel_create");
  for (int d = 1; d <= pl.xdist; ++d) CHK(own_array(D->own, D->gx[d], pl.gram_bytes, "panel_create"));
  if (pl.has16 && !D->own.take({{&D->gramp16, packed * 2}, {&D->gramx16, (size_t)pl.nblocks * pl.m * pl.m * 2}, {&D->gram16_bad, sizeof(int)}})) return no_memory("panel_create");
  for (const void *f : {reinterpret_cast<const void *>(k_sweep<int8_t, true>), reinterpret_cast<const void *>(k_sweep<int8_t, false>), reinterpret_cast<const void *>(k_sweep<float, true>),
                        reinterpret_cast<const void *>(k_sweep<float, false>), reinterpret_cast<const void *>(k_sweep2<int8_t, true>), reinterpret_cast<const void *>(k_sweep2<int8_t, false>),
                        reinterpret_cast<const void *>(k_sweep2<int8_t, true, uint16_t>), reinterpret_cast<const void *>(k_sweep2<float, true>), reinterpret_cast<const void *>(k_sweep2<float, false>),
                        reinterpret_cast<const void *>(k_sweep2w<true>), reinterpret_cast<const void *>(k_sweep2w<false>), reinterpret_cast<const void *>(k_affine_inv)})
    HIPCHK(hipFuncSetAttribute(f, hipFuncAttributeMaxDynamicSharedMemorySize, 160 * 1024));
  drop.release();
  *out = P;
  return BWGR_OK;
}
static int scratch_panel_alloc(bwgr_panel **out, const bwgr_panel *P, int64_t rows, int nwg, PanelKind kind) {
  const PanelData *D = P->data;
  *out = nullptr;
  CHK(gram_range(D->is_f32 != 0, rows, D->xmax));
  CHK(panel_alloc(out, D->is_f32, rows, D->p, D->device, D->plan.m, nwg, kind, D->sw));
  (*out)->stream = P->stream;
  (*out)->data->xmax = D->xmax;
  return BWGR_OK;
}

extern "C" int bwgr_panel_create(bwgr_panel **out, const void *X, int xtype, int memloc, int64_t n, int64_t p,
                                 int64_t ldx, int device, int block, int nwg) {
  if (!out || !X) return fail(BWGR_EINVAL, "panel_create: null pointer");
  *out = nullptr;
  if (ldx < n) return fail(BWGR_EINVAL, "panel_create: need ldx >= n (n=%lld ldx=%lld)", (long long)n, (long long)ldx);
  if (xtype != BWGR_X_I8 && xtype != BWGR_X_F32 && xtype != BWGR_X_F64) return fail(BWGR_EINVAL, "panel_create: bad xtype %d", xtype);
  if (memloc != BWGR_HOST && memloc != BWGR_DEVICE) return fail(BWGR_EINVAL, "panel_create: bad memloc %d", memloc);
  bwgr_panel *P = nullptr;
  CHK(panel_alloc(&P, xtype != BWGR_X_I8, n, p, device, block, nwg, PANEL_MAIN, read_switches()));
  Guard drop([&] { bwgr_panel_destroy(P); });
  if (xtype == BWGR_X_I8) CHK((upload<int8_t, int8_t>(P, X, memloc, ldx)));
  else if (xtype == BWGR_X_F32) CHK((upload<float, float>(P, X, memloc, ldx)));
  else CHK((upload<double, float>(P, X, memloc, ldx)));
  CHK(panel_setup(P));
  CHK(scratch_alloc(P));
  drop.release();
  *out = P;
  return BWGR_OK;
}

#if defined(BWGR_STAMPS) || defined(BWGR_EXPERIMENTS)
extern "C" int bwgr_debug_stamps(bwgr_panel *P, unsigned long long out[256]) {
  HIPCHK(d2h(P->stream, out, P->stamps, sizeof(unsigned long long) * 256));
  HIPCHK(hipMemset(P->stamps, 0, sizeof(unsigned long long) * 256));
  return BWGR_OK;
}
#endif

extern "C" int bwgr_panel_clone(bwgr_panel **out, bwgr_panel *src) {
  if (!out || !src) return fail(BWGR_EINVAL, "panel_clone: null pointer");
  *out = nullptr;
  HIPCHK(hipSetDevice(src->data->device));
  HIPCHK(hipStreamSynchronize(src->stream));
  bwgr_panel *P = new bwgr_panel();
  P->data = src->data; P->data->nclones++;
  Guard drop([&] { bwgr_panel_destroy(P); });
  if (!(P->stream = P->own.stream(hipStreamNonBlocking, 0))) return fail(BWGR_EHIP, "panel_clone: hipStreamCreate failed");
  CHK(scratch_alloc(P));
  HIPCHK(hipStreamSynchronize(P->stream));
  drop.release();
  *out = P;
  return BWGR_OK;
}

extern "C" int bwgr_panel_max_concurrent(const bwgr_panel *P, int selection, int *count) {
  if (!P || !count) return fail(BWGR_EINVAL, "null pointer");
  hipDeviceProp_t prop;
  HIPCHK(hipGetDeviceProperties(&prop, P->data->device));
  SweepArgs a{}; a.flags = selection ? SWF_SELECT : 0u;
  const SweepPlan pl = plan_sweep(P, a, false);
  int wgs = P->data->plan.K + 1 + pl.nfeed;
  if (pl.engine == 3) wgs = std::max(P->data->plan3.K3 + 1, wgs);
  if (pl.engine == 4) wgs = pl.spins[0].resident;
  *count = std::max(1, prop.multiProcessorCount / wgs);
  if (P->data->sw.max_concurrent > 0) *count = P->data->sw.max_concurrent;
  return BWGR_OK;
}

extern "C" int bwgr_panel_max_pairs(const bwgr_panel *P, int *pairs) {
  if (!P || !pairs) return fail(BWGR_EINVAL, "null pointer");
  *pairs = 0;
  if (!P->data->e3_ready || s3p_streamer_lds(P->data->plan3.R3) > (size_t)160 * 1024) return BWGR_OK;
  const int cus = device_cus(P->data->device);
  if (cus < 1) return fail(BWGR_EHIP, "panel_max_pairs: no device properties");
  *pairs = std::max(1, (cus - 40) / (P->data->plan3.K3 + 2));
  if (P->data->sw.max_pairs > 0) *pairs = P->data->sw.max_pairs;
  return BWGR_OK;
}

extern "C" int bwgr_debug_withhold(bwgr_panel *P, int on) {
  if (!P) return fail(BWGR_EINVAL, "null panel");
  P->debug_withhold = on ? 1 : 0;
  return BWGR_OK;
}

extern "C" int bwgr_panel_set_stream(bwgr_panel *P, void *hip_stream) {
  if (!P) return fail(BWGR_EINVAL, "null panel");
  P->stream = reinterpret_cast<hipStream_t>(hip_stream);
  P->pre_pair_set = false;
  return BWGR_OK;
}

extern "C" int bwgr_panel_info(const bwgr_panel *P, int64_t info[8]) {
  if (!P || !info) return fail(BWGR_EINVAL, "null pointer");
  info[0] = P->data->n; info[1] = P->data->p; info[2] = P->data->plan.ld; info[3] = P->data->plan.m; info[4] = P->data->plan.K; info[5] = P->data->plan.R;
  info[6] = (int64_t)P->data->plan.x_bytes; info[7] = (int64_t)(2 * P->data->plan.gram_bytes);
  return BWGR_OK;
}

extern "C" int bwgr_debug_sweep3_kernel(const bwgr_panel *P, int *which) {
  if (!P || !which) return fail(BWGR_EINVAL, "null pointer");
  SweepArgs a{}; a.flags = SWF_SELECT | (P->data->cen ? SWF_CENTRE : 0u);
  a.m = P->data->plan.m; a.pstride = P->data->plan.pstride; a.blk_begin = 0; a.blk_end = (int)P->data->plan.nblocks;
  const SweepPlan pl = plan_sweep(P, a, false);
  *which = pl.engine != 3 ? 0 : (pl.fixed3 ? 2 : 1);
  return BWGR_OK;
}

extern "C" int bwgr_panel_pipeline(const bwgr_panel *P, int selection, int info[4]) {
  if (!P || !info) return fail(BWGR_EINVAL, "null pointer");
  SweepArgs a{}; a.flags = selection ? SWF_SELECT : 0u;
  const SweepPlan pl = plan_sweep(P, a, false);
  info[0] = pl.engine;
  info[1] = pl.engine == 3 ? P->data->plan3.D : pl.lag;
  info[2] = pl.engine == 3 ? 0 : pl.nfeed;
  info[3] = P->data->is_f32 ? 0 : (P->data->gram16 ? 16 : 32);
  return BWGR_OK;
}

extern "C" int bwgr_panel_stats(bwgr_panel *P, float *xx, float *vx, float *MSx) {
  if (!P) return fail(BWGR_EINVAL, "null panel");
  HIPCHK(hipSetDevice(P->data->device));
  if (xx) HIPCHK(d2h(P->stream, xx, P->data->cen ? P->data->xxc : P->data->xx, sizeof(float) * P->data->p));
  if (vx) HIPCHK(d2h(P->stream, vx, P->data->vx, sizeof(float) * P->data->p));
  if (MSx) *MSx = P->data->MSx;
  return BWGR_OK;
}

static int gather_mpw(bool is_f32, int64_t ld) {
  if (is_f32 || ld > 64 * 1024) return 0;
  return (int)std::max<int64_t>(1, std::min<int64_t>(8, (32 * 1024) / ld));
}
static size_t gather_lds(int mpw, int64_t ld) { return (size_t)mpw * (size_t)ld; }
static void launch_gather_rows(bwgr_panel *P, bwgr_panel *PB, const int *use_d, int64_t nbag) {
  const int mpw = gather_mpw(P->data->is_f32, P->data->plan.ld);
  if (P->data->is_f32) hipLaunchKernelGGL(k_gather_rows<float>, dim3(4096), dim3(256), 0, P->stream, (const float *)P->data->X, P->data->plan.R, use_d, (int)nbag, (float *)PB->data->X, PB->data->plan.R, PB->data->plan.ld, P->data->p);
  else if (mpw > 0) {
    hipLaunchKernelGGL(k_gather_rows_i8, dim3((unsigned)((P->data->p + mpw - 1) / mpw)), dim3(256), gather_lds(mpw, P->data->plan.ld), P->stream, (const int8_t *)P->data->X, P->data->plan.R, P->data->plan.ld,
                       use_d, (int)nbag, (int8_t *)PB->data->X, PB->data->plan.R, PB->data->plan.ld, P->data->p, mpw);
  } else hipLaunchKernelGGL(k_gather_rows<int8_t>, dim3(4096), dim3(256), 0, P->stream, (const int8_t *)P->data->X, P->data->plan.R, use_d, (int)nbag, (int8_t *)PB->data->X, PB->data->plan.R, PB->data->plan.ld, P->data->p);
}

static thread_local int g_last_redo = 0;
extern "C" int bwgr_debug_last_redo(int *count) {
  if (!count) return fail(BWGR_EINVAL, "null pointer");
  *count = g_last_redo;
  return BWGR_OK;
}

static int kmup_sweep(bwgr_panel *PS, float *b, float *d, const float *xx, const float *L, double *e64, float Ve, float pi, float bg,
                      int kmup2, uint64_t seed, uint32_t iter, int rng_mode, const char *who) {
  DevBufs bufs;
  const size_t p = (size_t)PS->data->p, pb = sizeof(float) * p;
  float *db = bufs.get<float>(p), *dd = bufs.get<float>(p), *dxx = bufs.get<float>(p), *dL = bufs.get<float>(p), *dvb = bufs.get<float>(p);
  ChainScalars *sc = bufs.get<ChainScalars>(1);
  if (!db || !dd || !dxx || !dL || !dvb || !sc) return fail(BWGR_ENOMEM, "%s: device allocation failed", who);
  HIPCHK(hipMemcpyAsync(db, b, pb, hipMemcpyHostToDevice, PS->stream));
  HIPCHK(hipMemcpyAsync(dd, d, pb, hipMemcpyHostToDevice, PS->stream));
  HIPCHK(hipMemcpyAsync(dxx, xx, pb, hipMemcpyHostToDevice, PS->stream));
  HIPCHK(hipMemcpyAsync(dL, L, pb, hipMemcpyHostToDevice, PS->stream));
  ChainScalars h; memset(&h, 0, sizeof(h));
  h.ve = Ve; h.pi = pi; h.C = -0.5f / sqrtf(Ve); h.odds = pi / (1.0f - pi); h.dfp1 = 1.0f; h.bg = bg;
  h.inc_rate = 1.0f - pi;
  HIPCHK(hipMemcpyAsync(sc, &h, sizeof(h), hipMemcpyHostToDevice, PS->stream));
  SweepArgs a; memset(&a, 0, sizeof(a));
  fill_panel_args(PS, a);
  a.flags = SWF_LAM_VEC | (pi > 0 ? (SWF_SELECT | SWF_ALT_B2) : 0) | (kmup2 ? SWF_KMUP2 : 0);
  a.e = e64; a.b = db; a.d = dd; a.vb = dvb; a.xx = dxx; a.lam = dL; a.sc = sc;
  a.iter = iter; a.rng = make_rng(seed, rng_mode);
  CHK(launch_sweep(PS, a));
  HIPCHK(hipMemcpyAsync(b, db, pb, hipMemcpyDeviceToHost, PS->stream));
  HIPCHK(hipMemcpyAsync(d, dd, pb, hipMemcpyDeviceToHost, PS->stream));
  HIPCHK(hipMemcpyAsync(&h, sc, sizeof(h), hipMemcpyDeviceToHost, PS->stream));
  HIPCHK(hipStreamSynchronize(PS->stream));
  g_last_redo = (int)h.nredo;
  if (h.error) return sweep_error(h.error, who);
  return BWGR_OK;
}

extern "C" int bwgr_kmup(bwgr_panel *P, float *b, float *d, const float *xx, float *e, const float *L, float Ve,
                         float pi, uint64_t seed, uint32_t iter, int rng_mode) {
  if (P && P->data->cen) return refuse_centred("kmup");
  if (!P || !b || !d || !xx || !e || !L) return fail(BWGR_EINVAL, "kmup: null pointer");
  HIPCHK(hipSetDevice(P->data->device));
  DevBufs bufs;
  float *de = bufs.get<float>((size_t)P->data->n);
  double *de64 = bufs.get<double>((size_t)P->data->plan.ld);
  if (!de || !de64) return fail(BWGR_ENOMEM, "kmup: device allocation failed");
  HIPCHK(hipMemcpyAsync(de, e, sizeof(float) * P->data->n, hipMemcpyHostToDevice, P->stream));
  hipLaunchKernelGGL(k_f2d, dim3(64), dim3(256), 0, P->stream, de, de64, P->data->n, P->data->plan.ld);
  CHK(kmup_sweep(P, b, d, xx, L, de64, Ve, pi, 0.0f, 0, seed, iter, rng_mode, "kmup"));
  hipLaunchKernelGGL(k_d2f, dim3(64), dim3(256), 0, P->stream, de64, de, P->data->n);
  HIPCHK(hipGetLastError());
  HIPCHK(d2h(P->stream, e, de, sizeof(float) * P->data->n));
  return BWGR_OK;
}

extern "C" int bwgr_kmup2(bwgr_panel *P, const int *Use, int64_t nuse, float *b, float *d, const float *xx, const float *E,
                          float *e_out, const float *L, float Ve, float pi, uint64_t seed, uint32_t iter, int rng_mode) {
  if (P && P->data->cen) return refuse_centred("kmup2");
  if (!P || !Use || !b || !d || !xx || !E || !e_out || !L) return fail(BWGR_EINVAL, "kmup2: null pointer");
  if (nuse < 2 || nuse > 0x7FFFFF00ll) return fail(BWGR_EINVAL, "kmup2: need 2 <= length(Use) < 2^31 (got %lld)", (long long)nuse);
  for (int64_t k = 0; k < nuse; ++k)
    if (Use[k] < 0 || Use[k] >= P->data->n) return fail(BWGR_EINVAL, "kmup2: Use[%lld] = %d is outside 0..%lld", (long long)k, Use[k], (long long)P->data->n - 1);
  HIPCHK(hipSetDevice(P->data->device));
  bwgr_panel *PB = nullptr;
  CHK(scratch_panel_alloc(&PB, P, nuse, 0, PANEL_ROWS));
  Guard drop([&] { bwgr_panel_destroy(PB); });
  CHK(scratch_alloc(PB));
  DevBufs bufs;
  int *use_d = bufs.get<int>((size_t)nuse);
  float *dE = bufs.get<float>((size_t)P->data->n), *deo = bufs.get<float>((size_t)nuse);
  double *dE64 = bufs.get<double>((size_t)P->data->n), *e64 = bufs.get<double>((size_t)PB->data->plan.ld);
  if (!use_d || !dE || !deo || !dE64 || !e64) return fail(BWGR_ENOMEM, "kmup2: device allocation failed");
  HIPCHK(hipMemcpyAsync(use_d, Use, sizeof(int) * (size_t)nuse, hipMemcpyHostToDevice, P->stream));
  HIPCHK(hipMemcpyAsync(dE, E, sizeof(float) * P->data->n, hipMemcpyHostToDevice, P->stream));
  launch_gather_rows(P, PB, use_d, nuse);
  HIPCHK(hipGetLastError());
  CHK(panel_build_gram(PB));
  hipLaunchKernelGGL(k_f2d, dim3(64), dim3(256), 0, P->stream, dE, dE64, P->data->n, P->data->n);
  hipLaunchKernelGGL(k_gather_e, dim3(64), dim3(256), 0, P->stream, dE64, use_d, (int)nuse, PB->data->plan.ld, e64);
  HIPCHK(hipGetLastError());
  CHK(kmup_sweep(PB, b, d, xx, L, e64, Ve, pi, (float)P->data->n / (float)nuse, 1, seed, iter, rng_mode, "kmup2"));
  hipLaunchKernelGGL(k_d2f, dim3(64), dim3(256), 0, P->stream, e64, deo, nuse);
  HIPCHK(hipGetLastError());
  HIPCHK(d2h(P->stream, e_out, deo, sizeof(float) * (size_t)nuse));
  return BWGR_OK;
}

static bool per_marker_vb(int model) { return model == BWGR_BAYESA || model == BWGR_BAYESB || model == BWGR_BAYESL || model == BWGR_BAYESDPI; }
static bool has_d(int model) { return model == BWGR_BAYESB || model == BWGR_BAYESC || model == BWGR_BAYESCPI || model == BWGR_BAYESDPI; }

extern "C" int bwgr_chain_destroy(bwgr_chain *C) {
  if (!C) return BWGR_OK;
  if (C->P && C->P->ps_owner == C) C->P->ps_owner = nullptr;
// ... 1461 lines not shown
```

### bwgr_amd/csrc/sweep.hip.h

```cpp
#pragma once
#include <hip/hip_runtime.h>
#include <stdint.h>
#include "rng.hip.h"

namespace bwgr {

static constexpr int SW_THREADS = 512;
static constexpr int SW_MAXM = 128;
static constexpr int SW_FLAG_STRIDE = 32;
static constexpr uint64_t SW_TIMEOUT_TICKS = 400000000ull;

enum : int {
  SWF_SELECT = 1,
  SWF_ALT_B2 = 2,
  SWF_MH = 4,
  SWF_LAM_VEC = 8,
  SWF_VB_VEC = 16,
  SWF_KMUP2 = 32,
  SWF_DELTA2 = 64,
  SWF_EM_SEL = 128,
  SWF_EM_EN = 256,
  SWF_EM_BL = 512,
  SWF_EM_LASSO = 1024,
  SWF_EM_ANY = SWF_EM_SEL | SWF_EM_EN | SWF_EM_BL | SWF_EM_LASSO,
  SWF_SERIAL = 1 << 19,
  SWF_DEBUG_WITHHOLD = 1 << 20,
  SWF_CENTRE = 1 << 21
};

struct ChainScalars {
  float ve, vb, lam, pi;
  float Sb, Se, C, odds;
  float mu, dfp1, vy, MSx;
  float MU, VE, VBs, Pi;
  double sum_d, sum_b2;
  uint32_t error;
  float bg;
  int e3_sh;
  uint32_t e3_dex;
  float inc_rate;
  uint32_t redo;
  double snap_sum_d, snap_sum_b2;
  uint32_t nredo;
  double cen_u0, cen_c;
};

struct StageBuf;
struct SpecBuf {
  double spec[128];
  double xspec[128];
  double gjj[128];
};
struct QuickBuf {
  double zc[128], ha[128], hr[128];
};
struct PreStage {
  StageBuf *blocks;
  SpecBuf *spec;
  QuickBuf *quick;
};

struct SweepArgs {
  const void *X; int64_t ld;
  const void *gram;
  const void *gramx;
  const void *gramx2;
  double *xspec2;
  const void *gramx3;
  double *xspec3;
  int lag;
  int nfeed;
  const void *gramp;
  int pstride;
  int n, p, m, K, R;
  int blk_begin, blk_end;
  int flags;
  double *e;
  float *b, *d, *vb;
  const float *xx, *lam;
  ChainScalars *sc;
  uint32_t iter;
  uint32_t marker0;
  Rng rng;
  PreStage ps;
  double *xpart;
  double *qpart;
  unsigned long long *dgran;
  uint32_t *xflags;
  unsigned long long *stamps;
  const double *draws;
  int redo_only;
  float gate3;
  const int32_t *csum; double *cpre; double ninv;
};

template <typename XT> struct XTraits;
template <> struct XTraits<int8_t> { using GT = int32_t; static constexpr int PER16 = 16; static constexpr int MAXM = 128; };
template <> struct XTraits<float> { using GT = double; static constexpr int PER16 = 4; static constexpr int MAXM = 64; };

template <typename XT> __host__ __device__ inline int tile_rp(int R) { return R + XTraits<XT>::PER16; }

struct StageBuf {
  float b0[SW_MAXM], xxb0[SW_MAXM], b2[SW_MAXM], drej[SW_MAXM];
  double rden[SW_MAXM], sdz1[SW_MAXM], chi[SW_MAXM];
  float tacc[SW_MAXM], trej[SW_MAXM];
};

template <typename XT> __host__ __device__ inline size_t sweep_lds_bytes(int m, int R) {
  size_t s = 0;
  s += (size_t)2 * m * tile_rp<XT>(R) * sizeof(XT);
  s = (s + 15) & ~(size_t)15;
  s += (size_t)m * m * sizeof(typename XTraits<XT>::GT);
  s = (s + 15) & ~(size_t)15;
  s += (size_t)R * sizeof(double);
  s += 2 * sizeof(StageBuf);
  s += (size_t)(SW_THREADS / 64) * SW_MAXM * sizeof(double);
  s += 4 * SW_MAXM * sizeof(double);
  s += 2 * SW_MAXM * sizeof(float);
  s += 64;
  return s;
}

__device__ __forceinline__ double readlane_f64(double v, int l) {
  const int lo = __builtin_amdgcn_readlane(__double2loint(v), l);
  const int hi = __builtin_amdgcn_readlane(__double2hiint(v), l);
  return __hiloint2double(hi, lo);
}
__device__ __forceinline__ float readlane_f32(float v, int l) {
  return __int_as_float(__builtin_amdgcn_readlane(__float_as_int(v), l));
}

typedef __attribute__((address_space(1))) uint32_t gu32_t;
typedef __attribute__((address_space(1))) unsigned long long gu64_t;
__device__ __forceinline__ uint32_t ld_agent_u32(const uint32_t *p) {
  return __hip_atomic_load((const gu32_t *)p, __ATOMIC_RELAXED, __HIP_MEMORY_SCOPE_AGENT);
}
__device__ __forceinline__ void st_agent_u32(uint32_t *p, uint32_t v) {
  __hip_atomic_store((gu32_t *)p, v, __ATOMIC_RELAXED, __HIP_MEMORY_SCOPE_AGENT);
}
__device__ __forceinline__ unsigned long long ld_agent_raw64(const unsigned long long *p) {
  return __hip_atomic_load((const gu64_t *)p, __ATOMIC_RELAXED, __HIP_MEMORY_SCOPE_AGENT);
}
__device__ __forceinline__ void st_agent_raw64(unsigned long long *p, unsigned long long v) {
  __hip_atomic_store((gu64_t *)p, v, __ATOMIC_RELAXED, __HIP_MEMORY_SCOPE_AGENT);
}
__device__ __forceinline__ void st_agent_u64(double *p, double v) {
  st_agent_raw64(reinterpret_cast<unsigned long long *>(p), (unsigned long long)__double_as_longlong(v));
}
__device__ __forceinline__ double ld_agent_f64(const double *p) {
  return __longlong_as_double((long long)ld_agent_raw64(reinterpret_cast<const unsigned long long *>(p)));
}

__host__ __device__ inline size_t xoff(int64_t i, int64_t j, int R, int64_t p) {
  const int64_t w = i / R;
  return (size_t)((w * p + j) * R + (i - w * R));
}

static constexpr int SW_TCH = 5;
#define BWGR_TILE_EACH(X) X(0, tp0) X(1, tp1) X(2, tp2) X(3, tp3) X(4, tp4)
#define BWGR_ISSUE1(u, name) { const int c_ = (tid - 64) + (u) * (SW_THREADS - 64); if (c_ < tot_) name = src_[c_]; }
#define TILE_ISSUE(j0_, mB_) do { const int tot_ = (mB_) * (R / PER); \
    const uint4 *src_ = reinterpret_cast<const uint4 *>(X + (size_t)(j0_) * R); BWGR_TILE_EACH(BWGR_ISSUE1) } while (0)
#define BWGR_COMMIT1(u, name) { const int c_ = (tid - 64) + (u) * (SW_THREADS - 64); if (c_ < tot_) { \
    const int jj_ = (int)(((float)c_ + 0.5f) * rcpr_), ii_ = c_ - jj_ * cpr_;    \
    *reinterpret_cast<uint4 *>((dst_) + (size_t)jj_ * Rp + ii_ * PER) = name; } }
#define TILE_COMMIT(dstp, mB_) do { XT *dst_ = (dstp); const int cpr_ = R / PER; const int tot_ = (mB_) * cpr_; \
    const float rcpr_ = 1.0f / (float)cpr_; BWGR_TILE_EACH(BWGR_COMMIT1) } while (0)

__global__ void k_prestage(const SweepArgs a, int j_begin, int j_end) {
  const ChainScalars &sc = *a.sc;
  const float ve = sc.ve, lam_common = sc.lam, dfp1 = sc.dfp1;
  const int64_t nm = j_end - j_begin;
  __shared__ uint32_t dex_s;
  if (threadIdx.x == 0) dex_s = 0u;
  __syncthreads();
  for (int64_t task = (int64_t)blockIdx.x * blockDim.x + threadIdx.x; task < 4 * nm; task += (int64_t)gridDim.x * blockDim.x) {
    const int piece = (int)(task / nm);
    const int j = j_begin + (int)(task - (int64_t)piece * nm);
    StageBuf &st = a.ps.blocks[j / a.m];
    const int t = j % a.m;
    const float b0 = a.b[j];
    const float xxj = a.xx[j];
    const float lamj = (a.flags & SWF_LAM_VEC) ? a.lam[j] : lam_common;
    const bool k2 = (a.flags & SWF_KMUP2) != 0;
    const float den = k2 ? (xxj * sc.bg + lamj) : (xxj + lamj);
    const float sd = sqrtf(ve / den);
    const uint32_t mk = a.marker0 + (uint32_t)j;
    const bool sel = (a.flags & SWF_SELECT) != 0;
    if (piece == 0) {
      st.b0[t] = b0;
      st.xxb0[t] = k2 ? b0 : xxj * b0;
      st.rden[t] = 1.0 / (double)den;
      const double sdz1 = (a.flags & SWF_EM_BL) ? 1.0 / (double)(xxj + sc.Sb)
                                                : (double)sd * (a.draws ? a.draws[j] : rng_normal(a.rng, mk, a.iter, RNG_Z1, 0));
      st.sdz1[t] = sdz1;
      if (!sel && !(a.flags & SWF_EM_ANY)) atomicMax(&dex_s, (__float_as_uint(fmaxf(fabsf(b0), fabsf((float)sdz1))) >> 23) & 0xFFu);
    } else if (piece == 1) {
      const float b2 = sel ? (float)((double)0.0f + (double)sd * (a.draws ? a.draws[(size_t)a.p + j] : rng_normal(a.rng, mk, a.iter, RNG_Z2, 0))) : 0.0f;
      st.b2[t] = b2;
      const float drej = sel ? (b2 - b0) : 0.0f;
      st.drej[t] = drej;
      if (sel) atomicMax(&dex_s, (__float_as_uint(drej) >> 23) & 0xFFu);
    } else if (piece == 2) {
      if (a.draws) {
        float ta = -INFINITY, tr = INFINITY;
        const double la = a.draws[2 * (size_t)a.p + j], lr = a.draws[3 * (size_t)a.p + j];
        if (sc.odds > 0.0f && lr == lr) {
          const double lo = log((double)sc.odds);
          if (la == la) ta = (float)(la - lo);
          tr = (float)(lr - lo);
          ta = nextafterf(ta, -INFINITY); tr = nextafterf(tr, INFINITY);
          if (!(ta < tr)) { ta = -INFINITY; tr = INFINITY; }
        }
        st.tacc[t] = ta; st.trej[t] = tr;
        continue;
      }
      const double uj = sel ? rng_uniform(a.rng, mk, a.iter, RNG_U, 0) : 0.0;
      float ta = -INFINITY, tr = INFINITY;
      if (sel && uj > 0.0) {
        const double eta = 1e-6, ua = uj * (1.0 + eta), ur = uj * (1.0 - eta);
        if (a.flags & SWF_MH) {
          const double omp = (double)(1.0f - sc.pi);
          if (omp > 0.0) { ta = (float)log(omp / ua); tr = (float)log(omp / ur); }
        } else if (sc.odds > 0.0f) {
          const double lo = log((double)sc.odds);
          if (ua < 1.0) ta = (float)(log1p(-ua) - log(ua) - lo);
          tr = (float)(log1p(-ur) - log(ur) - lo);
        }
        ta = nextafterf(ta, -INFINITY); tr = nextafterf(tr, INFINITY);
        if (!(ta < tr)) { ta = -INFINITY; tr = INFINITY; }
      }
      st.tacc[t] = ta; st.trej[t] = tr;
    } else {
      st.chi[t] = a.draws ? a.draws[4 * (size_t)a.p + j] : ((a.flags & SWF_VB_VEC) ? rng_chisq(a.rng, (double)dfp1, mk, a.iter, RNG_CHI) : 1.0);
    }
  }
  if (j_end > j_begin && (a.m < SW_MAXM || (j_end % a.m) != 0)) {
    const int blk0 = j_begin / a.m, blk1 = (j_end - 1) / a.m;
    for (int blk = blk0 + (int)blockIdx.x; blk <= blk1; blk += (int)gridDim.x) {
      StageBuf &st = a.ps.blocks[blk];
      for (int t = min(a.m, j_end - blk * a.m) + (int)threadIdx.x; t < SW_MAXM; t += (int)blockDim.x) {
        st.b0[t] = 0.0f; st.xxb0[t] = 0.0f; st.b2[t] = 0.0f; st.drej[t] = 0.0f;
        st.rden[t] = 0.0; st.sdz1[t] = 0.0; st.chi[t] = 1.0;
        st.tacc[t] = -INFINITY; st.trej[t] = -INFINITY;
      }
    }
  }
  __syncthreads();
  if (threadIdx.x == 0 && dex_s != 0u) atomicMax(&a.sc->e3_dex, dex_s);
}
__global__ void k_draws(Rng rng, uint32_t marker0, uint32_t iter, int flags, const ChainScalars *sc_in, int64_t p, int j_begin, int j_end, double *out) {
  const float dfp1 = sc_in->dfp1;
  const int64_t nm = j_end - j_begin;
  const bool sel = (flags & SWF_SELECT) != 0;
  for (int64_t task = (int64_t)blockIdx.x * blockDim.x + threadIdx.x; task < 4 * nm; task += (int64_t)gridDim.x * blockDim.x) {
    const int piece = (int)(task / nm);
    const int j = j_begin + (int)(task - (int64_t)piece * nm);
    const uint32_t mk = marker0 + (uint32_t)j;
    if (piece == 0) out[j] = rng_normal(rng, mk, iter, RNG_Z1, 0);
    else if (piece == 1) out[(size_t)p + j] = sel ? rng_normal(rng, mk, iter, RNG_Z2, 0) : 0.0;
    else if (piece == 2) {
      const double uj = sel ? rng_uniform(rng, mk, iter, RNG_U, 0) : 0.0;
      double la = NAN, lr = NAN;
      if (sel && uj > 0.0) {
        const double eta = 1e-6, ua = uj * (1.0 + eta), ur = uj * (1.0 - eta);
        if (ua < 1.0) la = log1p(-ua) - log(ua);
        lr = log1p(-ur) - log(ur);
      }
      out[2 * (size_t)p + j] = la; out[3 * (size_t)p + j] = lr;
    } else out[4 * (size_t)p + j] = (flags & SWF_VB_VEC) ? rng_chisq(rng, (double)dfp1, mk, iter, RNG_CHI) : 1.0;
  }
}
__global__ __launch_bounds__(256) void k_prestage_fin(const SweepArgs a, int j_begin, int j_end) {
  const ChainScalars &sc = *a.sc;
  const float ve = sc.ve, lam_common = sc.lam;
  __shared__ uint32_t dex_s;
  __shared__ double lo_s;
  if (threadIdx.x == 0) { dex_s = 0u; lo_s = (sc.odds > 0.0f) ? log((double)sc.odds) : 0.0; }
  __syncthreads();
  const bool odds_pos = sc.odds > 0.0f;
  const double lo = lo_s;
  const bool k2 = (a.flags & SWF_KMUP2) != 0;
  const size_t p = (size_t)a.p;
  uint32_t dex = 0u;
  for (int j = j_begin + (int)(blockIdx.x * blockDim.x + threadIdx.x); j < j_end; j += (int)(gridDim.x * blockDim.x)) {
    StageBuf &st = a.ps.blocks[j / a.m];
    const int t = j % a.m;
    const float b0 = a.b[j];
    const float xxj = a.xx[j];
    const float lamj = (a.flags & SWF_LAM_VEC) ? a.lam[j] : lam_common;
    const float den = k2 ? (xxj * sc.bg + lamj) : (xxj + lamj);
    const float sd = sqrtf(ve / den);
    st.b0[t] = b0;
    st.xxb0[t] = k2 ? b0 : xxj * b0;
    st.rden[t] = 1.0 / (double)den;
    st.sdz1[t] = (double)sd * a.draws[j];
    const float b2 = (float)((double)0.0f + (double)sd * a.draws[p + j]);
    st.b2[t] = b2;
    const float drej = b2 - b0;
    st.drej[t] = drej;
    dex = max(dex, (__float_as_uint(drej) >> 23) & 0xFFu);
    float ta = -INFINITY, tr = INFINITY;
    const double la = a.draws[2 * p + j], lr = a.draws[3 * p + j];
    if (odds_pos && lr == lr) {
      if (la == la) ta = (float)(la - lo);
      tr = (float)(lr - lo);
      ta = nextafterf(ta, -INFINITY); tr = nextafterf(tr, INFINITY);
      if (!(ta < tr)) { ta = -INFINITY; tr = INFINITY; }
    }
    st.tacc[t] = ta; st.trej[t] = tr;
    st.chi[t] = a.draws[4 * p + j];
  }
  if (dex) atomicMax(&dex_s, dex);
  if (j_end > j_begin && (a.m < SW_MAXM || (j_end % a.m) != 0)) {
    const int blk0 = j_begin / a.m, blk1 = (j_end - 1) / a.m;
    for (int blk = blk0 + (int)blockIdx.x; blk <= blk1; blk += (int)gridDim.x) {
      StageBuf &st = a.ps.blocks[blk];
      for (int t = min(a.m, j_end - blk * a.m) + (int)threadIdx.x; t < SW_MAXM; t += (int)blockDim.x) {
        st.b0[t] = 0.0f; st.xxb0[t] = 0.0f; st.b2[t] = 0.0f; st.drej[t] = 0.0f;
        st.rden[t] = 0.0; st.sdz1[t] = 0.0; st.chi[t] = 1.0;
        st.tacc[t] = -INFINITY; st.trej[t] = -INFINITY;
      }
    }
  }
  __syncthreads();
  if (threadIdx.x == 0 && dex_s != 0u) atomicMax(&a.sc->e3_dex, dex_s);
}
__device__ inline void stage_block(StageBuf &st, int blk, const SweepArgs &a, int tid0, int nthreads) {
  constexpr int NCH = (int)(sizeof(StageBuf) / 16);
  static_assert(sizeof(StageBuf) % 16 == 0, "StageBuf must be a multiple of 16 bytes");
  const uint4 *src = reinterpret_cast<const uint4 *>(a.ps.blocks + blk);
  uint4 *dst = reinterpret_cast<uint4 *>(&st);
  for (int c = tid0; c < NCH; c += nthreads) dst[c] = src[c];
}

#ifdef BWGR_STAMPS
#define STAMP(k) do { if (tid == 0) { const unsigned long long t_ = __builtin_amdgcn_s_memtime(); ph[k] += t_ - tlast; tlast = t_; } } while (0)
#else
#define STAMP(k) do { } while (0)
#endif

template <typename GT>
__device__ __forceinline__ void put_gram4(GT *gram_s, double *gdiag_s, int m, int e0, const GT v[4]) {
  const int row = (int)(((float)e0 + 0.5f) * (1.0f / (float)m)), col0 = e0 - row * m;
#pragma unroll
  for (int c = 0; c < 4; ++c) {
    const int col = col0 + c;
    gram_s[e0 + c] = (col > row) ? v[c] : (GT)0;
    if (col == row) gdiag_s[row] = (double)v[c];
  }
}

struct LaneConst {
  float b0, xxb0, b2, drej;
  double rden, sdz1, gjj;
  float tacc, trej;
  uint32_t mk;
};
__device__ __forceinline__ float lane_b1(double r, const LaneConst &c) {
  return (float)fma(r + (double)c.xxb0, c.rden, c.sdz1);
}
__device__ __forceinline__ float lane_em(double r, const LaneConst &c, int flags, float Cc, float Pi0, float L1, float *dout) {
  const double ols = r + (double)c.xxb0;
  if (flags & SWF_EM_SEL) {
    const float b1 = (float)(ols * c.rden);
    const double D1 = (double)(b1 - c.b0), D2 = (double)(0.0f - c.b0);
    const double diffd = 2.0 * r * (D1 - D2) + c.gjj * (D2 * D2 - D1 * D1);
    const float LR = Pi0 * (float)exp((double)(Cc * (float)diffd));
    const float d = 1.0f / (1.0f + LR);
    *dout = d;
    return b1 * d;
  }
  *dout = 1.0f;
  if (flags & SWF_EM_LASSO) {
    const double yx = fma(c.gjj, (double)c.b0, r);
    *dout = (float)yx;
    const bool pos = yx > 0.0;
    const float b1 = (float)((yx - (pos ? (double)L1 : -(double)L1)) * c.rden);
    return pos ? fmaxf(b1, 0.0f) : fminf(b1, 0.0f);
  }
  const bool pos = ols > 0.0;
  const double sl = pos ? (double)L1 : -(double)L1;
  if (flags & SWF_EM_EN) {
    const float b1 = (float)((ols - sl) * c.rden);
    return pos ? fmaxf(b1, 0.0f) : fminf(b1, 0.0f);
  }
  const double half = 0.5 * ols * c.sdz1;
  const double G = 0.5 * (ols - sl) * c.rden;
  const bool keep = pos ? (G > 0.0) : (G < 0.0);
  return (float)(keep ? G + half : half);
}
__device__ __attribute__((noinline)) bool lane_accept_exact(double diffd, uint32_t mk, int flags, float Cc, float odds, float one_minus_pi,
                                                            Rng rng, uint32_t iter) {
  float pj;
  if (flags & SWF_MH) {
    const float diff = (float)(-diffd);
    pj = one_minus_pi * expf(Cc * diff);
    if (pj > 1.0f) pj = 1.0f;
  } else {
    const float diff = (float)diffd;
    const float LR = odds * expf(Cc * diff);
    pj = 1.0f / (1.0f + LR);
  }
  return rng_uniform(rng, mk, iter, RNG_U, 0) < (double)pj;
}
__device__ __forceinline__ bool lane_accept(double r, float b1, const LaneConst &c, int flags, float Cc, float odds,
                                            float one_minus_pi, const Rng &rng, uint32_t iter) {
  const float d1f = b1 - c.b0;
  const float d2f = (flags & SWF_ALT_B2) ? (c.b2 - c.b0) : (0.0f - c.b0);
  const double D1 = (double)d1f, D2 = (double)d2f;
  const double diffd = 2.0 * r * (D1 - D2) + c.gjj * (D2 * D2 - D1 * D1);
  const float x = Cc * (float)diffd;
  const bool sure_acc = x < c.tacc, sure_rej = x > c.trej;
  if (__builtin_expect(__ballot(!(sure_acc || sure_rej)) == 0ull, 1)) return sure_acc;
  const bool exact = lane_accept_exact(diffd, c.mk, flags, Cc, odds, one_minus_pi, rng, iter);
  return sure_acc ? true : (sure_rej ? false : exact);
}

__device__ __forceinline__ void lane_quick(const LaneConst &c, int flags, float Cc, double &zc, double &ha, double &hr) {
  const double b0 = (double)c.b0, D2 = (double)((flags & SWF_ALT_B2) ? (c.b2 - c.b0) : (0.0f - c.b0));
  const double k1 = fma((double)c.xxb0, c.rden, c.sdz1) - b0;
  const double gr = c.gjj * c.rden;
  const double A = c.rden * (2.0 - gr), Bh = (k1 - D2) - gr * k1, C0 = c.gjj * (D2 * D2 - k1 * k1);
  zc = -Bh / A;
  const double Qmin = fma(Bh, zc, C0);
  const double qa = (double)c.tacc / (double)Cc, qr = (double)c.trej / (double)Cc;
  auto err = [&](double h, double q) {
    const double ra = fabs(zc) + h;
    const double d1 = fma(c.rden, ra, fabs(k1)), t = d1 + fabs(b0);
    const double eD = 6.1e-8 * (t + d1);
    return 4.0 * (2.0 * (ra + c.gjj * d1) * eD + c.gjj * eD * eD) + 2.5e-7 * fabs(q)
           + 1e-13 * (2.0 * ra * (d1 + fabs(D2)) + c.gjj * (D2 * D2 + d1 * d1));
  };
  ha = INFINITY; hr = -1.0;
  if (A > 0.0 && fabs(zc) < 1e300 && Cc < 0.0f) {
    if (fabs(qa) < INFINITY) {
      const double num = (qa - Qmin) + err(sqrt(fmax(0.0, (qa - Qmin) / A)), qa);
      ha = (num > 0.0) ? sqrt(num / A) * (1.0 + 1e-12) : -1.0;
    }
    if (qr == INFINITY) hr = INFINITY;
    else if (fabs(qr) < INFINITY) {
      const double num = (qr - Qmin) - err(sqrt(fmax(0.0, (qr - Qmin) / A)), qr);
      hr = (num > 0.0) ? sqrt(num / A) * (1.0 - 1e-12) : -1.0;
    }
  }
}
template <typename GT, bool CEN = false>
__device__ __forceinline__ void quick_rounds(double (&r)[2], const LaneConst (&lc)[2], const double (&zc)[2], const double (&ha)[2], const double (&hr)[2],
                                             unsigned long long (&accmask)[2], const GT *gp, int m, int mB,
                                             int lane, int flags, float Cc, float odds, float one_minus_pi, const Rng &rng, uint32_t iter,
                                             const double *cs = nullptr, double ninv = 0.0, double *cenU = nullptr) {
  const int ngrp = (mB + 63) >> 6;
  const GT *gl = gp + lane;
#pragma unroll
  for (int q = 0; q < 2; ++q) {
    if (q < ngrp) {
      const int base = 64 * q, cnt = min(64, mB - base);
      const int kk = base + lane;
      const int tab = (kk * (m - 1) - kk * (kk - 1) / 2 - lane - 1) * (int)sizeof(GT);
      unsigned long long livem = (cnt >= 64) ? ~0ull : ((1ull << cnt) - 1ull);
      unsigned long long am = 0ull;
      double rq = r[q], ro = r[1], z = rq - zc[q];
      const double haq = ha[q], hrq = hr[q], drejd = (double)lc[q].drej;
      const float b0q = lc[q].b0;
      {
        unsigned long long cand, accm;
        int js;
        float b1;
        double cd, corr, gm0;
        GT g0, g1;
      qr_top:
        cand = livem & ~__ballot(fabs(z) < hrq);
        if (cand == 0ull) goto qr_done;
        js = (int)__builtin_ctzll(cand);
        {
          const GT *row = reinterpret_cast<const GT *>(reinterpret_cast<const char *>(gl) + __builtin_amdgcn_readlane(tab, js));
          g0 = row[0]; g1 = row[64];
        }
        accm = __ballot(fabs(z) > haq);
        b1 = lane_b1(rq, lc[q]);
        cd = (double)(b1 - b0q) - drejd;
        livem &= (~1ull << js);
        if (__builtin_expect(!((accm >> js) & 1ull), 0)) goto qr_sliver;
      qr_apply:
        corr = readlane_f64(cd, js);
        am |= (1ull << js);
        if constexpr (CEN) {
          const double xk = readlane_f64(cs[q], js) * ninv;
          *cenU = fma(xk, corr, *cenU);
          gm0 = (lane > js) ? ((double)g0 - cs[q] * xk) : 0.0;
          rq = fma(-gm0, corr, rq);
          z = fma(-gm0, corr, z);
          if (q == 0) ro = fma(-((double)g1 - cs[1] * xk), corr, ro);
          goto qr_top;
        }
        gm0 = (double)((lane > js) ? g0 : (GT)0);
        rq = fma(-gm0, corr, rq);
        z = fma(-gm0, corr, z);
        if (q == 0) ro = fma(-(double)g1, corr, ro);
        goto qr_top;
      qr_sliver:
        if ((__ballot(lane_accept(rq, b1, lc[q], flags, Cc, odds, one_minus_pi, rng, iter)) >> js) & 1ull) goto qr_apply;
        goto qr_top;
      qr_done:;
      }
      r[q] = rq;
      if (q == 0) r[1] = ro;
      accmask[q] |= am;
    }
  }
}

template <typename GT>
__global__ __launch_bounds__(128) void k_spec(const SweepArgs a, int blk_begin, int select) {
  if (a.redo_only ? (a.sc->redo == 0u) : (a.gate3 > 0.0f && a.sc->inc_rate < a.gate3)) return;
  const int blk = blk_begin + blockIdx.x, j = threadIdx.x, m = a.m;
  const int mB = min(m, a.p - blk * m);
  const GT *G = reinterpret_cast<const GT *>(a.gram) + (size_t)blk * m * m;
  SpecBuf &sp = a.ps.spec[blk];
  __shared__ float dr[128], drp[128];
  const StageBuf &st = a.ps.blocks[blk];
  dr[j] = (j < mB) ? st.drej[j] : 0.0f;
  drp[j] = (blk > blk_begin) ? a.ps.blocks[blk - 1].drej[j] : 0.0f;
  __syncthreads();
  double s = 0.0, xs = 0.0, gjj = 0.0;
  const bool cen = (a.flags & SWF_CENTRE) != 0 && select;
  __shared__ double cs_s[128];
  const double sj = (cen && j < mB) ? (double)a.csum[blk * m + j] : 0.0;
  if (cen) { cs_s[j] = sj * (double)dr[j]; __syncthreads(); }
  if (j < mB) {
    gjj = (double)G[(size_t)j * m + j];
    if (cen) {
      double ib = 0.0;
      for (int k = 0; k < j; ++k) ib += cs_s[k];
      s = -(sj * a.ninv) * (a.cpre[blk] + ib);
      gjj -= sj * sj * a.ninv;
    }
    if (select) {
      for (int k = 0; k < j; ++k) s = fma((double)G[(size_t)k * m + j], (double)dr[k], s);
      if (blk > blk_begin) {
        const GT *Gx = reinterpret_cast<const GT *>(a.gramx) + (size_t)blk * m * m;
        for (int k = 0; k < m; ++k) xs = fma((double)Gx[(size_t)k * m + j], (double)drp[k], xs);
      }
    }
  }
  sp.spec[j] = s; sp.xspec[j] = xs; sp.gjj[j] = gjj;
  if (select && a.ps.quick) {
    double zc = 0.0, ha = INFINITY, hr = INFINITY;
    if (j < mB) {
      LaneConst c;
      c.b0 = st.b0[j]; c.xxb0 = st.xxb0[j]; c.b2 = st.b2[j]; c.drej = st.drej[j];
      c.rden = st.rden[j]; c.sdz1 = st.sdz1[j]; c.gjj = gjj; c.tacc = st.tacc[j]; c.trej = st.trej[j]; c.mk = 0u;
      lane_quick(c, a.flags, a.sc->C, zc, ha, hr);
    }
    QuickBuf &qb = a.ps.quick[blk];
    qb.zc[j] = zc; qb.ha[j] = ha; qb.hr[j] = hr;
  }
  for (int dist = 2; dist < a.lag; ++dist) {
    double xs2 = 0.0;
    __syncthreads();
    drp[j] = (blk - dist >= blk_begin) ? a.ps.blocks[blk - dist].drej[j] : 0.0f;
    __syncthreads();
    if (j < mB && select && blk - dist >= blk_begin) {
      const GT *Gxd = reinterpret_cast<const GT *>(dist == 2 ? a.gramx2 : a.gramx3) + (size_t)blk * m * m;
      for (int k = 0; k < m; ++k) xs2 = fma((double)Gxd[(size_t)k * m + j], (double)drp[k], xs2);
    }
    (dist == 2 ? a.xspec2 : a.xspec3)[(size_t)blk * SW_MAXM + j] = xs2;
  }
}

template <typename XT, bool SELECT>
__global__ __launch_bounds__(SW_THREADS) void k_sweep(const SweepArgs a) {
  using GT = typename XTraits<XT>::GT;
  constexpr int PER = XTraits<XT>::PER16;
  constexpr int GPT = 16 / sizeof(GT);
  constexpr int MAXMX = XTraits<XT>::MAXM;
  constexpr int GCH = (MAXMX * MAXMX / GPT + (SW_THREADS - 64) - 1) / (SW_THREADS - 64);
  extern __shared__ __attribute__((aligned(16))) unsigned char smem[];
  const int tid = threadIdx.x, lane = tid & 63, wave = tid >> 6;
  const int wg = blockIdx.x;
  const int m = a.m, R = a.R, K = a.K;
  const int Rp = tile_rp<XT>(R);
  const int row0 = wg * R;
  if ((a.flags & SWF_DEBUG_WITHHOLD) && wg == 0 && K > 1) return;

  size_t off = 0;
  XT *tile0 = reinterpret_cast<XT *>(smem);
  XT *tile1 = tile0 + (size_t)m * Rp;
  off = ((size_t)2 * m * Rp * sizeof(XT) + 15) & ~(size_t)15;
  GT *gram_s = reinterpret_cast<GT *>(smem + off);
  off = (off + (size_t)m * m * sizeof(GT) + 15) & ~(size_t)15;
  double *e_s = reinterpret_cast<double *>(smem + off); off += (size_t)R * sizeof(double);
  StageBuf *stage = reinterpret_cast<StageBuf *>(smem + off); off += 2 * sizeof(StageBuf);
  double *part_s = reinterpret_cast<double *>(smem + off); off += (size_t)(SW_THREADS / 64) * SW_MAXM * sizeof(double);
  double *r0_s = reinterpret_cast<double *>(smem + off); off += SW_MAXM * sizeof(double);
  double *spec_s = reinterpret_cast<double *>(smem + off); off += SW_MAXM * sizeof(double);
  double *gdiag_s = reinterpret_cast<double *>(smem + off); off += SW_MAXM * sizeof(double);
  double *delta_s = reinterpret_cast<double *>(smem + off); off += SW_MAXM * sizeof(double);
  float *bnew_s = reinterpret_cast<float *>(smem + off); off += SW_MAXM * sizeof(float);
  float *dnew_s = reinterpret_cast<float *>(smem + off); off += SW_MAXM * sizeof(float);
  int *ctrl_s = reinterpret_cast<int *>(smem + off);

  const XT *X = reinterpret_cast<const XT *>(a.X) + (size_t)wg * a.p * R;
  const GT *gram = reinterpret_cast<const GT *>(a.gram);

  const float Cc = a.sc->C, odds = a.sc->odds;
  const double dscale = (a.flags & SWF_DELTA2) ? 2.0 : 1.0;
  const float one_minus_pi = 1.0f - a.sc->pi, Sb = a.sc->Sb;

  const int nb = a.blk_end - a.blk_begin;
  const int mpad = (m <= 64) ? 64 : 128;
  const int ngroups = SW_THREADS / mpad;
  const int rows_per_group = R / ngroups;
  const int gchunks = m * m / GPT;

  uint4 tp0 = make_uint4(0, 0, 0, 0), tp1 = tp0, tp2 = tp0, tp3 = tp0, tp4 = tp0;
  for (int i = tid; i < R; i += SW_THREADS) e_s[i] = a.e[row0 + i];
  if (tid == 0) ctrl_s[0] = 1;

  auto spec_matvec = [&](const StageBuf &stn, int mBn) {
    if (SELECT) {
      const int part = tid >> 7, j = tid & 127;
      if (j < mBn) {
        double acc = 0.0;
        const int k0 = part * 32, k1 = min(k0 + 32, min(j, mBn));
        for (int k = k0; k < k1; ++k) acc = fma((double)gram_s[(size_t)k * m + j], (double)stn.drej[k], acc);
        part_s[part * SW_MAXM + j] = acc;
      }
      __syncthreads();
// ... 344 lines not shown
```

### bwgr_amd/csrc/sweep3.hip.h

```cpp
#pragma once
#include "sweep2.hip.h"

namespace bwgr {

#ifdef BWGR_STAMPS
#define S3ST_DECL unsigned long long ph3[8] = {0, 0, 0, 0, 0, 0, 0, 0}, tl3 = __builtin_amdgcn_s_memtime()
#define S3ST(k, cond) do { if ((BWGR_STAMPS == 1 || (BWGR_STAMPS == 2 && ((k) == 0 || (k) == 1 || (k) == 4)) || (BWGR_STAMPS == 3 && ((k) == 0 || (k) == 4) && blockIdx.x == 0 && threadIdx.x == 0) || (BWGR_STAMPS == 4 && (k) <= 5 && blockIdx.x == 0 && threadIdx.x == 0)) && (cond)) { const unsigned long long t_ = __builtin_amdgcn_s_memtime(); ph3[k] += t_ - tl3; tl3 = t_; } } while (0)
#define S3ST_FLUSH(base, cond) do { if ((cond) && a.stamps) for (int k_ = 0; k_ < 8; ++k_) atomicAdd(&a.stamps[(base) + k_], ph3[k_]); } while (0)
#else
#define S3ST_DECL do { } while (0)
#define S3ST(k, cond) do { } while (0)
#define S3ST_FLUSH(base, cond) do { } while (0)
#endif

static constexpr int S3_MAXD = 16;
static constexpr int S3_LSTRIDE = 2 * SW_MAXM + 2;
static constexpr int S3_ND = 7;
static constexpr int S3_RING = S3_MAXD * SW_MAXM;
static constexpr int S3_GPD_BYTES = 16384;
static constexpr int S3_ROWSLOT = 1024;
static constexpr int S3_NRX = 8;
static constexpr int S3_OS = 12;
static constexpr int S3_NFW = 4;
static constexpr int S3_NFL = 8;
static constexpr int S3_QRAW_BYTES = SW_MAXM * 16;

struct S3ShapeAny { static constexpr bool fixed = false; };
struct S3Shape128 { static constexpr bool fixed = true; static constexpr int m = SW_MAXM, pstride = SW_MAXM * (SW_MAXM - 1) / 2; };
static_assert(S3Shape128::m == 128 && S3Shape128::pstride == 8128 && S3Shape128::pstride % 8 == 0, "the packed block's stride needs no padding at m = 128");
template <typename SH, typename ARGS> __device__ __forceinline__ int s3_m(const ARGS &a) { if constexpr (SH::fixed) return SH::m; else return a.m; }
template <typename SH, typename ARGS> __device__ __forceinline__ int s3_pstride(const ARGS &a) { if constexpr (SH::fixed) return SH::pstride; else return a.pstride; }

struct Sweep3Args {
  SweepArgs a;
  const void *gx[S3_MAXD];
  const void *gp;
  int D;
  int K3, R3, sub;
  int g16;
  unsigned long long *qsum;
  unsigned long long *lists;
  uint32_t epoch;
  int dbg;
  int pf;
  int pf2;
  int qsplit;
  int skip_vb;
  const unsigned char *gx12;
};

__global__ void k_near_rows(const uint16_t *g1, const uint16_t *g2, uint16_t *out, int m, int64_t nblocks) {
  const int64_t total = nblocks * m * 2 * m;
  for (int64_t t = (int64_t)blockIdx.x * blockDim.x + threadIdx.x; t < total; t += (int64_t)gridDim.x * blockDim.x) {
    const int j = (int)(t % m), d = (int)((t / m) & 1), k = (int)((t / (2 * m)) % m);
    const int64_t b = t / ((int64_t)2 * m * m);
    const uint16_t *g = d ? g2 : g1;
    out[t] = (g && b + d + 1 < nblocks) ? g[((b + d + 1) * m + k) * m + j] : (uint16_t)0;
  }
}

__global__ void k_escale_reset(ChainScalars *sc) { sc->e3_dex = 0u; }
__global__ __launch_bounds__(1024) void k_escale(const double *e, int64_t ld, ChainScalars *sc, int xbits, float gate3, int sh_add = 0) {
  if (!(sc->inc_rate < gate3)) { if (threadIdx.x == 0) sc->e3_dex = 0u; return; }
  __shared__ uint32_t mx;
  if (threadIdx.x == 0) mx = 0u;
  __syncthreads();
  uint32_t ex = 0u;
  for (int64_t i = threadIdx.x; i < ld; i += blockDim.x) ex = max(ex, (uint32_t)((__double2hiint(e[i]) & 0x7FFFFFFF) >> 20));
  atomicMax(&mx, ex);
  __syncthreads();
  if (threadIdx.x == 0) {
    const int ke = (int)mx - 1022;
    const int kd = (int)sc->e3_dex - 126 + xbits;
    int k = max(ke, kd);
    k = max(-200, min(200, k));
    sc->e3_sh = 44 - k + sh_add;
    sc->e3_dex = 0u;
  }
}
__device__ __forceinline__ double s3_pow2(int k) { return __hiloint2double((1023 + k) << 20, 0); }

__device__ __forceinline__ bool cen_active(const SweepArgs &a, int mode) {
  if (mode == 2) return a.sc->redo != 0u;
  const bool three = a.gate3 > 0.0f && a.sc->inc_rate < a.gate3;
  return mode == 0 ? three : !three;
}
__global__ __launch_bounds__(128) void k_cen_tot(const SweepArgs a, int blk_begin, int mode) {
  if (!cen_active(a, mode)) return;
  const int blk = blk_begin + blockIdx.x, j = threadIdx.x, m = a.m;
  const int mB = min(m, a.p - blk * m);
  const int sh = a.sc->e3_sh;
  const double S = s3_pow2(mode == 0 ? sh : 0), invS = s3_pow2(mode == 0 ? -sh : 0);
  __shared__ double red[128];
  const double dj = (j < mB) ? (double)a.ps.blocks[blk].drej[j] : 0.0;
  red[j] = (j < mB) ? (double)a.csum[blk * m + j] * (mode == 0 ? rint(dj * S) * invS : dj) : 0.0;
  __syncthreads();
  for (int o = 64; o > 0; o >>= 1) { if (j < o) red[j] += red[j + o]; __syncthreads(); }
  if (j == 0) a.cpre[blk + 1] = red[0];
}
__global__ __launch_bounds__(1024) void k_cen_scan(const SweepArgs a, int nblocks, int mode) {
  if (!cen_active(a, mode)) return;
  __shared__ double part[1024];
  const int t = threadIdx.x, per = (nblocks + 1023) / 1024;
  const int b0 = min(nblocks, t * per), b1 = min(nblocks, b0 + per);
  double s = 0.0;
  for (int b = b0; b < b1; ++b) s += a.cpre[b + 1];
  part[t] = s;
  __syncthreads();
  if (t == 0) { double run = 0.0; for (int i = 0; i < 1024; ++i) { const double v = part[i]; part[i] = run; run += v; } }
  __syncthreads();
  double run = part[t];
  for (int b = b0; b < b1; ++b) { run += a.cpre[b + 1]; a.cpre[b + 1] = run; }
  if (t == 0) a.cpre[0] = 0.0;
}
__global__ __launch_bounds__(1024) void k_cen_begin(const SweepArgs a, int mode) {
  if (!cen_active(a, mode)) return;
  __shared__ double red[1024];
  const int t = threadIdx.x;
  double s = 0.0;
  for (int64_t i = t; i < a.ld; i += 1024) s += a.e[i];
  red[t] = s;
  __syncthreads();
  for (int o = 512; o > 0; o >>= 1) { if (t < o) red[t] += red[t + o]; __syncthreads(); }
  if (t == 0) { a.sc->cen_u0 = -(red[0] + a.cpre[a.blk_begin]) * a.ninv; a.sc->cen_c = 0.0; }
}
__global__ void k_cen_end(const SweepArgs a, int mode) {
  if (!cen_active(a, mode) || a.sc->error != 0u) return;
  const double shift = (a.cpre[a.blk_end] - a.cpre[a.blk_begin]) * a.ninv + a.sc->cen_c;
  for (int64_t i = (int64_t)blockIdx.x * blockDim.x + threadIdx.x; i < a.n; i += (int64_t)gridDim.x * blockDim.x) a.e[i] += shift;
}

__global__ __launch_bounds__(128) void k_spec3(const SweepArgs a, int blk_begin, const uint16_t *gp16 = nullptr) {
  if (!(a.sc->inc_rate < a.gate3)) return;
  const int blk = blk_begin + blockIdx.x, j = threadIdx.x, m = a.m;
  const int mB = min(m, a.p - blk * m);
  const int32_t *G = reinterpret_cast<const int32_t *>(a.gram) + (size_t)blk * m * m;
  SpecBuf &sp = a.ps.spec[blk];
  __shared__ double dr[128];
  __shared__ double cs[128];
  const bool cen = (a.flags & SWF_CENTRE) != 0;
  const int sh = a.sc->e3_sh;
  const double S = s3_pow2(sh), invS = s3_pow2(-sh);
  dr[j] = (j < mB) ? rint((double)a.ps.blocks[blk].drej[j] * S) * invS : 0.0;
  const int sj = (cen && j < mB) ? a.csum[blk * m + j] : 0;
  cs[j] = (double)sj * dr[j];
  __syncthreads();
  double s0 = 0.0, s1 = 0.0, s2 = 0.0, s3 = 0.0, gjj = 0.0, ib = 0.0;
  if (j < mB) {
    gjj = (double)G[(size_t)j * m + j];
    int k = 0;
    if (gp16) {
      const uint16_t *Gp = gp16 + (size_t)blk * a.pstride + (j - 1);
      int pr = 0;
      for (; k + 4 <= j; k += 4) {
        const int p0 = pr, p1 = p0 + (m - 2 - k), p2 = p1 + (m - 3 - k), p3 = p2 + (m - 4 - k);
        s0 = fma((double)Gp[p0], dr[k], s0);
        s1 = fma((double)Gp[p1], dr[k + 1], s1);
        s2 = fma((double)Gp[p2], dr[k + 2], s2);
        s3 = fma((double)Gp[p3], dr[k + 3], s3);
        pr = p3 + (m - 5 - k);
      }
      for (; k < j; ++k) { s0 = fma((double)Gp[pr], dr[k], s0); pr += m - 2 - k; }
    } else {
    for (; k + 4 <= j; k += 4) {
      s0 = fma((double)G[(size_t)k * m + j], dr[k], s0);
      s1 = fma((double)G[(size_t)(k + 1) * m + j], dr[k + 1], s1);
      s2 = fma((double)G[(size_t)(k + 2) * m + j], dr[k + 2], s2);
      s3 = fma((double)G[(size_t)(k + 3) * m + j], dr[k + 3], s3);
    }
    for (; k < j; ++k) s0 = fma((double)G[(size_t)k * m + j], dr[k], s0);
    }
    if (cen) for (int k2 = 0; k2 < j; ++k2) ib += cs[k2];
  }
  double spec = (s0 + s1) + (s2 + s3);
  if (cen) {
    spec -= ((double)sj * a.ninv) * (a.cpre[blk] + ib);
    gjj = __hiloint2double(sj, (j < mB) ? (int)G[(size_t)j * m + j] : 0);
  }
  sp.spec[j] = spec; sp.xspec[j] = 0.0; sp.gjj[j] = gjj;
}

__global__ void k_vb_fill(const SweepArgs a, int j_begin, int j_end) {
  const float Sb = a.sc->Sb;
  for (int j = j_begin + (int)(blockIdx.x * blockDim.x + threadIdx.x); j < j_end; j += (int)(gridDim.x * blockDim.x)) {
    const float bn = a.b[j];
    a.vb[j] = (float)((double)(Sb + bn * bn) / a.ps.blocks[j / a.m].chi[j % a.m]);
  }
}

__device__ __forceinline__ void s3_put_digits7(long long q, int8_t *dst, int stride) {
  const unsigned long long u = ((unsigned long long)q + 0x0080808080808080ull) ^ 0x0080808080808080ull;
  const uint32_t lo = (uint32_t)u, hi = (uint32_t)(u >> 32);
  dst[0] = (int8_t)lo; dst[stride] = (int8_t)(lo >> 8); dst[2 * stride] = (int8_t)(lo >> 16); dst[3 * stride] = (int8_t)(lo >> 24);
  dst[4 * stride] = (int8_t)hi; dst[5 * stride] = (int8_t)(hi >> 8); dst[6 * stride] = (int8_t)(hi >> 16);
}

__device__ __forceinline__ unsigned long long s3_hdr(uint32_t epoch, int count) { return ((unsigned long long)epoch << 40) | (0xFFull << 32) | (unsigned long long)(uint32_t)count; }
__device__ __forceinline__ bool s3_epoch_is(unsigned long long w, uint32_t epoch) { return (uint32_t)(w >> 40) == epoch; }

typedef unsigned int s3_u4 __attribute__((ext_vector_type(4)));

#pragma clang diagnostic push
#pragma clang diagnostic ignored "-Winline-asm"
__device__ __forceinline__ void s3_dma16(const void *gsrc, const void *lds_base) {
  const uint32_t la = (uint32_t)__builtin_amdgcn_readfirstlane((int)(uint32_t)(uintptr_t)(__attribute__((address_space(3))) const unsigned char *)lds_base);
  asm volatile("s_mov_b32 m0, %1\n\ts_nop 0\n\tglobal_load_lds_dwordx4 %0, off" : : "v"(gsrc), "s"(la) : "memory", "m0");
}
__device__ __forceinline__ void s3_dma4(const void *gsrc, const void *lds_base) {
  const uint32_t la = (uint32_t)__builtin_amdgcn_readfirstlane((int)(uint32_t)(uintptr_t)(__attribute__((address_space(3))) const unsigned char *)lds_base);
  asm volatile("s_mov_b32 m0, %1\n\ts_nop 0\n\tglobal_load_lds_dword %0, off" : : "v"(gsrc), "s"(la) : "memory", "m0");
}
__device__ __forceinline__ void s3_dma4s(const unsigned char *gbase, uint32_t voff, uint32_t la) {
  asm volatile("s_mov_b32 m0, %2\n\ts_nop 0\n\tglobal_load_lds_dword %0, %1" : : "v"(voff), "s"(gbase), "s"(la) : "memory", "m0");
}
__device__ __forceinline__ void s3_dma16s(const unsigned char *gbase, uint32_t voff, uint32_t la) {
  const unsigned long long gb_ = (unsigned long long)(uintptr_t)gbase;
  const unsigned char *sb_ = reinterpret_cast<const unsigned char *>((unsigned long long)(uint32_t)__builtin_amdgcn_readfirstlane((int)(uint32_t)gb_) |
                                                                    ((unsigned long long)(uint32_t)__builtin_amdgcn_readfirstlane((int)(uint32_t)(gb_ >> 32)) << 32));
  asm volatile("s_mov_b32 m0, %2\n\ts_nop 0\n\tglobal_load_lds_dwordx4 %0, %1" : : "v"(voff), "s"(sb_), "s"(la) : "memory", "m0");
}
__device__ __forceinline__ void s3_dma16s_sc1(const unsigned char *gbase, uint32_t voff, uint32_t la) {
  const unsigned long long gb_ = (unsigned long long)(uintptr_t)gbase;
  const unsigned char *sb_ = reinterpret_cast<const unsigned char *>((unsigned long long)(uint32_t)__builtin_amdgcn_readfirstlane((int)(uint32_t)gb_) |
                                                                    ((unsigned long long)(uint32_t)__builtin_amdgcn_readfirstlane((int)(uint32_t)(gb_ >> 32)) << 32));
  asm volatile("s_mov_b32 m0, %2\n\ts_nop 0\n\tglobal_load_lds_dwordx4 %0, %1 sc1" : : "v"(voff), "s"(sb_), "s"(la) : "memory", "m0");
}
#pragma clang diagnostic pop

__device__ __forceinline__ void s3_wait_vmcnt(int n) {
  switch (n) {
#define S3_WV(N_) case N_: asm volatile("s_waitcnt vmcnt(" #N_ ")" ::: "memory"); break;
    S3_WV(1) S3_WV(2) S3_WV(3) S3_WV(4) S3_WV(5) S3_WV(6) S3_WV(7) S3_WV(8) S3_WV(9) S3_WV(10) S3_WV(11) S3_WV(12) S3_WV(13) S3_WV(14) S3_WV(15) S3_WV(16)
    S3_WV(17) S3_WV(18) S3_WV(19) S3_WV(20) S3_WV(21) S3_WV(22) S3_WV(23) S3_WV(24) S3_WV(25) S3_WV(26) S3_WV(27) S3_WV(28) S3_WV(29) S3_WV(30) S3_WV(31) S3_WV(32)
#undef S3_WV
    default: asm volatile("s_waitcnt vmcnt(0)" ::: "memory"); break;
  }
}

__device__ __forceinline__ int s3_stream_index(const Sweep3Args &A) {
  const int x = (int)blockIdx.x;
  return x - 1 - ((A.pf >= 0 && x > A.pf) ? 1 : 0) - ((A.pf2 >= 0 && x > A.pf2) ? 1 : 0);
}

__host__ __device__ inline size_t s3_streamer_dma_lds(int R3 = 128) {
  const size_t Rp = (size_t)R3 + 16;
  return (R3 == 128 ? 4 : 3) * (size_t)SW_MAXM * R3 + 2 * 16 * Rp + 2 * 16 * (size_t)S2_DP + (size_t)64 * S3_OS * 4 * 4 + (size_t)8 * 32 * S3_OS * 4 + 64 + (size_t)4 * SW_MAXM * 4;
}
__host__ __device__ inline size_t s3_streamer_lds(int R3) {
  const size_t Rp = (size_t)R3 + 16;
  return 2 * (size_t)SW_MAXM * Rp + 2 * 16 * Rp + 2 * 16 * (size_t)S2_DP + (size_t)64 * S3_OS * 4 * 4 + (size_t)8 * 32 * S3_OS * 4 + 64;
}
__host__ __device__ inline size_t s3_seq_lds(int D, bool g16) {
  size_t s = 3 * sizeof(StageBuf) + 3 * 2 * SW_MAXM * sizeof(double);
  s += 2 * SW_MAXM * sizeof(double) + 2 * S3_NFW * SW_MAXM * sizeof(double);
  s += 2 * 3 * SW_MAXM * sizeof(float);
  (void)D;
  s += (size_t)S3_RING * (sizeof(double) + sizeof(long long) + sizeof(int));
  s += (size_t)2 * S3_NFW * S3_NFL * SW_MAXM * (g16 ? 2 : 4);
  if (g16) s += (size_t)3 * S3_GPD_BYTES + (size_t)S3_NRX * S3_ROWSLOT;
  s += (size_t)3 * S3_QRAW_BYTES;
  return s + 256 + 512;
}

__device__ __forceinline__ void s3_streamer(const Sweep3Args &A) {
#ifdef BWGR_EXPERIMENTS
  const int SDBG = A.dbg;
#else
  constexpr int SDBG = 0;
#endif
  extern __shared__ __attribute__((aligned(16))) unsigned char smem[];
  const SweepArgs &a = A.a;
  const int tid = threadIdx.x, lane = tid & 63, wave = tid >> 6;
  const int m16 = lane & 15, grp = lane >> 4;
  const int w = s3_stream_index(A);
  const unsigned long long *lists_w = A.lists;
  const int m = a.m, R = a.R, R3 = A.R3, Rp = R3 + 16, D = A.D;
  const int slab = w / A.sub, hsub = w - slab * A.sub;
  const int nb = a.blk_end - a.blk_begin;
  const int NU = R3 >> 6;
  const int ND = 8 - NU;
  const int cprs = (R3 == 256) ? 4 : (R3 == 128 ? 3 : 2);
  const int8_t *Xs = reinterpret_cast<const int8_t *>(a.X) + (size_t)slab * a.p * R + (size_t)hsub * R3;
  const int64_t row0 = (int64_t)slab * R + (int64_t)hsub * R3;
  uint32_t *abortw = a.xflags + (size_t)a.K * SW_FLAG_STRIDE;
  const size_t tile_b = (size_t)SW_MAXM * Rp;
  int8_t *tile0 = reinterpret_cast<int8_t *>(smem);
  size_t off = 2 * tile_b;
  int8_t *edig0 = reinterpret_cast<int8_t *>(smem + off); off += (size_t)2 * 16 * Rp;
  int8_t *ddig0 = reinterpret_cast<int8_t *>(smem + off); off += (size_t)2 * 16 * S2_DP;
  int *outu = reinterpret_cast<int *>(smem + off); off += (size_t)64 * S3_OS * 4 * 4;
  off += (size_t)8 * 32 * S3_OS * 4;
  uint32_t *ctl_s = reinterpret_cast<uint32_t *>(smem + off);
  const int sh = a.sc->e3_sh;
  const double S = s3_pow2(sh), invS = s3_pow2(-sh);
  auto blk_j0 = [&](int b) { return (a.blk_begin + b) * m; };
  auto blk_m = [&](int b) { return min(m, a.p - (a.blk_begin + b) * m); };

  for (int i = tid; i < (int)((2 * 16 * Rp + 2 * 16 * S2_DP) / 4); i += SW_THREADS) reinterpret_cast<uint32_t *>(edig0)[i] = 0u;
  if (tid < 16) ctl_s[tid] = 0u;
  long long e_own = 0;
  const bool upd = wave < NU;
  if (upd) e_own = __double2ll_rn(a.e[row0 + 64 * wave + lane] * S);

  s3_u4 ta0 = {0, 0, 0, 0}, ta1 = ta0, ta2 = ta0, ta3 = ta0, tb0 = ta0, tb1 = ta0, tb2 = ta0, tb3 = ta0;
#define S3_TILE_EACH(X) X(0, tp0) X(1, tp1) X(2, tp2) X(3, tp3)
#define S3_ISSUE1(u, name) { const int cc_ = min(tid + (u) * SW_THREADS, tot_ - 1); const int jj_ = min(cc_ >> cprs, mBt_ - 1), ii_ = cc_ & ((1 << cprs) - 1); \
    name = __builtin_nontemporal_load(reinterpret_cast<const s3_u4 *>(Xs + (size_t)(j0t_ + jj_) * R + ii_ * 16)); }
#define S3_TILE_ISSUE(b_) do { const int j0t_ = blk_j0(b_), mBt_ = blk_m(b_), tot_ = m << cprs; S3_TILE_EACH(S3_ISSUE1) } while (0)
#define S3_COMMIT1(u, name) { const int c_ = tid + (u) * SW_THREADS; if (c_ < tot_) { const int jj_ = c_ >> cprs, ii_ = c_ & ((1 << cprs) - 1); \
    *reinterpret_cast<s3_u4 *>(dst_ + (size_t)jj_ * Rp + ii_ * 16) = name; } }
#define S3_TILE_COMMIT(b_) do { int8_t *dst_ = tile0 + (size_t)((b_) & 1) * tile_b; const int tot_ = m << cprs; S3_TILE_EACH(S3_COMMIT1) } while (0)

  auto fold_list = [&](int bs, unsigned long long pre) -> int {
    const int Bs = a.blk_begin + bs;
    const unsigned long long *L = lists_w + (size_t)Bs * S3_LSTRIDE;
    const int8_t *col = Xs + (size_t)(Bs * m) * R + 64 * wave + lane;
    const uint64_t t0 = wall_clock64();
    unsigned spins = 0;
    unsigned long long hv = __builtin_amdgcn_readfirstlane((uint32_t)pre) | ((unsigned long long)__builtin_amdgcn_readfirstlane((uint32_t)(pre >> 32)) << 32);
    while (!s3_epoch_is(hv, A.epoch)) {
      hv = ld_agent_raw64(L);
      hv = __builtin_amdgcn_readfirstlane((uint32_t)hv) | ((unsigned long long)__builtin_amdgcn_readfirstlane((uint32_t)(hv >> 32)) << 32);
      if (s3_epoch_is(hv, A.epoch)) break;
      if ((++spins & 63u) == 0u) {
        if (ld_agent_u32(abortw) != 0u) return 0;
        if (wall_clock64() - t0 > SW_TIMEOUT_TICKS) { st_agent_u32(abortw, 1u); return 0; }
      }
      __builtin_amdgcn_s_sleep(1);
    }
    const int cnt = (int)(uint32_t)hv;
    for (int c0 = 0; c0 < cnt; c0 += 31) {
      const int nw = min(62, 2 * (cnt - c0));
      unsigned long long wv = pre;
      bool have = (c0 == 0);
      for (;;) {
        const bool mine = lane >= 1 && lane <= nw;
        if (!have) wv = mine ? ld_agent_raw64(L + 2 * c0 + lane) : 0ull;
        if (__ballot(mine && !s3_epoch_is(wv, A.epoch)) == 0ull) break;
        have = false;
        if ((++spins & 63u) == 0u) {
          if (ld_agent_u32(abortw) != 0u) return 0;
          if (wall_clock64() - t0 > SW_TIMEOUT_TICKS) { st_agent_u32(abortw, 1u); return 0; }
        }
        __builtin_amdgcn_s_sleep(1);
      }
      const uint32_t wlo = (uint32_t)wv, whi = (uint32_t)(wv >> 32);
      for (int e0 = 0; e0 < nw / 2; e0 += 8) {
        int xb[8]; long long cq[8];
#pragma unroll
        for (int u = 0; u < 8; ++u) {
          const int ee = min(e0 + u, nw / 2 - 1);
          const uint32_t a0 = __builtin_amdgcn_readlane(wlo, 1 + 2 * ee), a1 = __builtin_amdgcn_readlane(whi, 1 + 2 * ee);
          const uint32_t b0 = __builtin_amdgcn_readlane(wlo, 2 + 2 * ee);
          const int k = (int)(a1 & 0xFFu);
          cq[u] = (e0 + u < nw / 2) ? (long long)(((unsigned long long)b0 << 32) | (unsigned long long)a0) : 0ll;
          xb[u] = upd ? (int)col[(size_t)k * R] : 0;
        }
#pragma unroll
        for (int u = 0; u < 8; ++u) e_own -= (long long)xb[u] * cq[u];
      }
    }
    return 1;
  };

  {
    s3_u4 &tp0 = ta0, &tp1 = ta1, &tp2 = ta2, &tp3 = ta3;
    S3_TILE_ISSUE(0);
    S3_TILE_COMMIT(0);
    if (nb > 2) S3_TILE_ISSUE(2);
  }
  if (nb > 1) { s3_u4 &tp0 = tb0, &tp1 = tb1, &tp2 = tb2, &tp3 = tb3; S3_TILE_ISSUE(1); }
  float drej_pre = a.ps.blocks[a.blk_begin].drej[tid & (SW_MAXM - 1)];
  unsigned long long lpre = 0ull;
  __syncthreads();
  S3ST_DECL;
  [[maybe_unused]] const bool st_u = (w == 0 && tid == 0), st_d = (w == 0 && tid == 64 * NU);

  auto step = [&](int b, s3_u4 &tp0, s3_u4 &tp1, s3_u4 &tp2, s3_u4 &tp3) -> bool {
    const int mB = blk_m(b), par = b & 1;
    S3ST(0, st_u || st_d);
    int8_t *tile = tile0 + (size_t)par * tile_b;
    int8_t *edig = edig0 + (size_t)par * 16 * Rp;
    int8_t *ddig = ddig0 + (size_t)par * 16 * S2_DP;
    if (b >= D && upd && !(SDBG & 512)) { if (!fold_list(b - D, lpre)) ctl_s[0] = 1u; }
    S3ST(1, st_u);
    if (upd) {
      if ((unsigned long long)(e_own + (1ll << 54)) >> 55) ctl_s[1] = 1u;
      s3_put_digits7(e_own, edig + 64 * wave + lane, Rp);
    } else if (tid >= SW_THREADS - SW_MAXM) {
      const double qd = (tid - (SW_THREADS - SW_MAXM) < mB) ? rint((double)drej_pre * S) : 0.0;
      if (!(fabs(qd) < 18014398509481984.0)) ctl_s[1] = 1u;
      s3_put_digits7((long long)qd, ddig + (tid - (SW_THREADS - SW_MAXM)), S2_DP);
    }
    S3ST(2, st_u);
#if defined(BWGR_STAMPS) && BWGR_STAMPS == 2
    S3ST(0, st_u || st_d);
    asm volatile("s_waitcnt lgkmcnt(0)\n\ts_barrier" ::: "memory");
    S3ST(4, st_u || st_d);
#else
    asm volatile("s_waitcnt lgkmcnt(0)\n\ts_barrier" ::: "memory");
    S3ST(3, st_u || st_d);
#endif
    if (ctl_s[0]) { if (tid == 0) a.sc->error = 1u; return false; }
    if (b + 1 < nb) S3_TILE_COMMIT(b + 1);
    S3ST(6, st_u || st_d);
    {
      const int bn1 = min(b + 1, nb - 1);
      drej_pre = a.ps.blocks[a.blk_begin + bn1].drej[tid & (SW_MAXM - 1)];
      lpre = ld_agent_raw64(lists_w + (size_t)(a.blk_begin + max(bn1 - D, 0)) * S3_LSTRIDE + lane);
    }
    S3ST(7, st_u || st_d);
    if (b + 3 < nb && !(SDBG & 16)) S3_TILE_ISSUE(b + 3);
    S3ST(4, st_u || st_d);
    if (upd) {
      const int rowoff = 4 * (16 * wave + m16);
      s2_v4i acc0 = {0, 0, 0, 0}, acc1 = acc0, acc2 = acc0, acc3 = acc0;
      for (int s0 = 0; s0 < ((SDBG & 256) ? 0 : mB); s0 += 64) {
        const int8_t *tp = tile + __mul24(s0 + 4 * grp, Rp) + rowoff;
        uint32_t c[4][4];
#pragma unroll
        for (int u = 0; u < 4; ++u)
#pragma unroll
          for (int q = 0; q < 4; ++q)
            c[u][q] = *reinterpret_cast<const uint32_t *>(tp + (16 * u + q) * Rp);
        const int8_t *bp = ddig + (size_t)m16 * S2_DP + s0 + 4 * grp;
        const s2_v4i bv = {*reinterpret_cast<const int *>(bp), *reinterpret_cast<const int *>(bp + 16),
                           *reinterpret_cast<const int *>(bp + 32), *reinterpret_cast<const int *>(bp + 48)};
        uint32_t rw[4][4];
#pragma unroll
        for (int u = 0; u < 4; ++u) {
          const uint32_t t0 = __builtin_amdgcn_perm(c[u][1], c[u][0], 0x05010400u), t1 = __builtin_amdgcn_perm(c[u][1], c[u][0], 0x07030602u);
          const uint32_t t2 = __builtin_amdgcn_perm(c[u][3], c[u][2], 0x05010400u), t3 = __builtin_amdgcn_perm(c[u][3], c[u][2], 0x07030602u);
          rw[0][u] = __builtin_amdgcn_perm(t2, t0, 0x05040100u); rw[1][u] = __builtin_amdgcn_perm(t2, t0, 0x07060302u);
          rw[2][u] = __builtin_amdgcn_perm(t3, t1, 0x05040100u); rw[3][u] = __builtin_amdgcn_perm(t3, t1, 0x07060302u);
        }
        acc0 = __builtin_amdgcn_mfma_i32_16x16x64_i8(s2_v4i{(int)rw[0][0], (int)rw[0][1], (int)rw[0][2], (int)rw[0][3]}, bv, acc0, 0, 0, 0);
        acc1 = __builtin_amdgcn_mfma_i32_16x16x64_i8(s2_v4i{(int)rw[1][0], (int)rw[1][1], (int)rw[1][2], (int)rw[1][3]}, bv, acc1, 0, 0, 0);
        acc2 = __builtin_amdgcn_mfma_i32_16x16x64_i8(s2_v4i{(int)rw[2][0], (int)rw[2][1], (int)rw[2][2], (int)rw[2][3]}, bv, acc2, 0, 0, 0);
        acc3 = __builtin_amdgcn_mfma_i32_16x16x64_i8(s2_v4i{(int)rw[3][0], (int)rw[3][1], (int)rw[3][2], (int)rw[3][3]}, bv, acc3, 0, 0, 0);
      }
      int *ou = outu + (size_t)wave * 64 * S3_OS;
      if (m16 < 8) {
        int *op = ou + (size_t)(4 * (4 * grp)) * S3_OS + m16;
#pragma unroll
        for (int reg = 0; reg < 4; ++reg) {
          op[(4 * reg + 0) * S3_OS] = acc0[reg]; op[(4 * reg + 1) * S3_OS] = acc1[reg];
          op[(4 * reg + 2) * S3_OS] = acc2[reg]; op[(4 * reg + 3) * S3_OS] = acc3[reg];
        }
      }
      asm volatile("s_waitcnt lgkmcnt(0)" ::: "memory");
      {
        const int4 o0 = *reinterpret_cast<const int4 *>(ou + (size_t)lane * S3_OS);
        const int4 o1 = *reinterpret_cast<const int4 *>(ou + (size_t)lane * S3_OS + 4);
        long long v = (long long)o0.x + ((long long)o0.y << 8) + ((long long)o0.z << 16) + ((long long)o0.w << 24);
        v += ((long long)o1.x << 32) + ((long long)o1.y << 40) + ((long long)o1.z << 48);
        e_own -= v;
      }
      S3ST(5, st_u);
    } else {
      for (int gm = wave - NU; 16 * gm < m; gm += 2 * ND) {
        const int gm2 = gm + ND;
        const bool two = 16 * gm2 < m;
        const int8_t *bp = edig + (size_t)m16 * Rp + 16 * grp;
        const int8_t *ap = tile + (size_t)(16 * gm + m16) * Rp + 16 * grp;
        const int8_t *ap2 = tile + (size_t)(16 * (two ? gm2 : gm) + m16) * Rp + 16 * grp;
        s2_v4i acc = {0, 0, 0, 0}, acc2 = acc;
        for (int r = 0; r < ((SDBG & 256) ? 0 : R3); r += 64) {
          const s2_v4i bv = *reinterpret_cast<const s2_v4i *>(bp + r);
          acc = __builtin_amdgcn_mfma_i32_16x16x64_i8(bv, *reinterpret_cast<const s2_v4i *>(ap + r), acc, 0, 0, 0);
          acc2 = __builtin_amdgcn_mfma_i32_16x16x64_i8(bv, *reinterpret_cast<const s2_v4i *>(ap2 + r), acc2, 0, 0, 0);
        }
        if (grp < 2) {
          const long long w1 = (long long)acc[0] + ((long long)acc[1] << 8) + ((long long)acc[2] << 16) + ((long long)acc[3] << 24);
          const long long w2 = (long long)acc2[0] + ((long long)acc2[1] << 8) + ((long long)acc2[2] << 16) + ((long long)acc2[3] << 24);
          unsigned long long *qs = A.qsum + ((size_t)(a.blk_begin + b) * SW_MAXM + 16 * gm + m16) * 2 + grp;
          if (!(SDBG & 8)) {
            __hip_atomic_fetch_add((gu64_t *)qs, (unsigned long long)((w1 << 8) + 1), __ATOMIC_RELAXED, __HIP_MEMORY_SCOPE_AGENT);
            if (two) __hip_atomic_fetch_add((gu64_t *)(qs + (size_t)(16 * (gm2 - gm)) * 2), (unsigned long long)((w2 << 8) + 1), __ATOMIC_RELAXED, __HIP_MEMORY_SCOPE_AGENT);
          }
        }
// ... 960 lines not shown
```

Baseline: 107.8 iter/s.

## Fuse guard snapshot, recovery, qsum clear and vb fill into existing kernels

```diff
diff --git a/bwgr_amd/csrc/bwgr_hip.hip b/bwgr_amd/csrc/bwgr_hip.hip
--- a/bwgr_amd/csrc/bwgr_hip.hip
+++ b/bwgr_amd/csrc/bwgr_hip.hip
@@ -870,6 +870,19 @@
   if (sc->error == 2u) { sc->error = 0u; sc->redo = 1u; sc->nredo += 1u; sc->sum_d = sc->snap_sum_d; sc->sum_b2 = sc->snap_sum_b2; }
 }
 __global__ void k_redo_clear(ChainScalars *sc) { sc->redo = 0u; }
+__global__ __launch_bounds__(256) void k_sweep_post(const SnapArgs s, const SweepArgs a, int vb_fill) {
+  const int64_t nt = (int64_t)gridDim.x * blockDim.x, t0 = (int64_t)blockIdx.x * blockDim.x + threadIdx.x;
+  if (s.sc->error == 2u) {
+    for (int64_t i = t0; i < s.ld; i += nt) s.e[i] = s.se[i];
+    for (int64_t j = s.j0 + t0; j < s.j1; j += nt) { s.b[j] = a.ps.blocks[j / a.m].b0[j % a.m]; s.d[j] = s.sd[j]; }
+  } else if (vb_fill) {
+    const float Sb = a.sc->Sb;
+    for (int64_t j = s.j0 + t0; j < s.j1; j += nt) {
+      const float bn = a.b[j];
+      a.vb[j] = (float)((double)(Sb + bn * bn) / a.ps.blocks[j / a.m].chi[j % a.m]);
+    }
+  }
+}
 }
 
 struct Switches {
@@ -878,6 +891,7 @@
   float eng3_thr = 0.03f;
   bool occ_guard = true, pf3b = true, draws = true, gram16 = true;
   bool winv = true, wfx = true;
+  bool train = true;
 #ifdef BWGR_EXPERIMENTS
   bool fixed3 = false;
 #else
@@ -902,6 +916,7 @@
   s.occ_guard = chr(getenv("BWGR_OCC_GUARD")) != '0'; s.pf3b = chr(getenv("BWGR_PF3B")) != '0'; s.draws = chr(getenv("BWGR_DRAWS")) != '0';
   s.gram16 = chr(getenv("BWGR_GRAM16")) != '0';
   { const int c = chr(getenv("BWGR_FIXED3")); if (c == '0') s.fixed3 = false; else if (c == '1') s.fixed3 = true; }
+  s.train = chr(getenv("BWGR_TRAIN")) != '0';
   s.winv = chr(getenv("BWGR_WINV")) != '0'; s.wfx = chr(getenv("BWGR_WFX")) != '0';
   if (const char *v = getenv("BWGR_WPF")) s.wpf = std::max(0, std::min(8, atoi(v)));
   if (const char *v = getenv("BWGR_WAHEAD")) s.wahead = std::max(1, atoi(v));
@@ -1087,6 +1102,7 @@
   void *X = nullptr, *gram = nullptr, *gramp = nullptr;
   void *gx[S2W_NEARD + 1] = {};
   uint16_t *gramp16 = nullptr, *gramx16 = nullptr;
+  int32_t *gdiag = nullptr;
   int *gram16_bad = nullptr;
   void *g3x[S3_MAXD] = {};
   unsigned char *gx12 = nullptr;
@@ -1118,6 +1134,7 @@
   unsigned long long *qsum3 = nullptr, *lists3 = nullptr;
   uint32_t epoch3 = 0;
   double *snap_e = nullptr; float *snap_b = nullptr, *snap_d = nullptr, *snap_vb = nullptr;
+  bool snap_staged = false;
   double *winv = nullptr;
   unsigned long long *qsumw = nullptr;
   double *cpre = nullptr;
@@ -1207,6 +1224,7 @@
   bool fixed3 = false;
   int fx = 0, nd = 0, npf = 0, ahead = 0, nq = 0, wsub = 0, wK3 = 0;
   bool guarded = false;
+  bool fused = false, fused_guard = false;
   bool draws = false;
   int nspins = 0; SpinLaunch spins[3];
 };
@@ -1361,6 +1379,10 @@
   return BWGR_OK;
 }
 
+static bool snap_alloc(bwgr_panel *P) {
+  const size_t p = (size_t)P->data->p;
+  return P->snap_e || P->own.take({{&P->snap_e, sizeof(double) * (size_t)P->data->plan.ld}, {&P->snap_b, sizeof(float) * p}, {&P->snap_d, sizeof(float) * p}, {&P->snap_vb, sizeof(float) * p}});
+}
 static void launch_prestage(bwgr_panel *P, const SweepArgs &a_in, const SweepPlan &pl) {
   SweepArgs a = a_in;
   a.gate3 = pl.gate3;
@@ -1370,7 +1392,12 @@
   const bool fxa = pl.engine == 4 && pl.fx;
   const int sh_add = P->data->sw.sh_add;
   int xbits = 0; while ((1 << xbits) < std::max(1, P->data->xmax)) ++xbits;
-  if (s3 || fxa) hipLaunchKernelGGL(k_escale_reset, dim3(1), dim3(1), 0, P->stream, a.sc);
+  StageTail tl = STAGE_TAIL_AS_BEFORE;
+  tl.dex = (s3 || fxa || !P->data->sw.train) ? 1 : 0;
+  P->snap_staged = false;
+  if (pl.fused) {
+    if (pl.fused_guard && snap_alloc(P)) { tl.snap_d = P->snap_d; P->snap_staged = true; }
+  } else if (s3 || fxa) hipLaunchKernelGGL(k_escale_reset, dim3(1), dim3(1), 0, P->stream, a.sc);
   const int dflags = a.flags & (SWF_SELECT | SWF_VB_VEC);
   const bool have_draws = P->draws_valid && P->draws_iter == a.iter && P->draws_marker0 == a.marker0 && P->draws_flags == dflags &&
                           P->draws_sc == (const void *)a.sc && P->draws_j0 <= j0 && P->draws_j1 >= j1 && memcmp(&P->draws_rng, &a.rng, sizeof(Rng)) == 0 &&
@@ -1378,17 +1405,18 @@
   a.draws = nullptr;
   if (have_draws) { const hipError_t he = hipStreamWaitEvent(P->stream, P->draws_ready, 0); if (he == hipSuccess) a.draws = P->draws; else { fprintf(stderr, "bwgr: draws wait failed: %s\n", hipGetErrorString(he)); (void)hipGetLastError(); } }
   if (a.draws) {
-    hipLaunchKernelGGL(k_prestage_fin, dim3((unsigned)std::min<int64_t>(2048, (j1 - j0 + 255) / 256)), dim3(256), 0, P->stream, a, j0, j1);
+    hipLaunchKernelGGL(k_prestage_fin, dim3((unsigned)std::min<int64_t>(2048, (j1 - j0 + 255) / 256)), dim3(256), 0, P->stream, a, j0, j1, tl);
     { const hipError_t he = hipEventRecord(P->draws_free, P->stream); if (he != hipSuccess) { fprintf(stderr, "bwgr: draws_free record failed: %s\n", hipGetErrorString(he)); (void)hipGetLastError(); } }
     P->draws_valid = false;
-  } else hipLaunchKernelGGL(k_prestage, dim3((unsigned)std::min<int64_t>(4096, (tasks + 255) / 256)), dim3(256), 0, P->stream, a, j0, j1);
+  } else hipLaunchKernelGGL(k_prestage, dim3((unsigned)std::min<int64_t>(4096, (tasks + 255) / 256)), dim3(256), 0, P->stream, a, j0, j1, tl);
   if (s3) {
-    hipLaunchKernelGGL(k_escale, dim3(1), dim3(1024), 0, P->stream, a.e, P->data->plan.ld, a.sc, xbits, a.gate3, sh_add);
+    hipLaunchKernelGGL(k_escale, dim3(1), dim3(1024), 0, P->stream, a.e, P->data->plan.ld, a.sc, xbits, a.gate3, sh_add, P->snap_staged ? P->snap_e : (double *)nullptr);
     if (a.flags & SWF_CENTRE) {
       hipLaunchKernelGGL(k_cen_tot, dim3((unsigned)(a.blk_end - a.blk_begin)), dim3(128), 0, P->stream, a, a.blk_begin, 0);
       hipLaunchKernelGGL(k_cen_scan, dim3(1), dim3(1024), 0, P->stream, a, (int)P->data->plan.nblocks, 0);
     }
-    hipLaunchKernelGGL(k_spec3, dim3((unsigned)(a.blk_end - a.blk_begin)), dim3(128), 0, P->stream, a, a.blk_begin, P->data->gram16 ? (const uint16_t *)P->data->gramp16 : (const uint16_t *)nullptr);
+    hipLaunchKernelGGL(k_spec3, dim3((unsigned)(a.blk_end - a.blk_begin)), dim3(128), 0, P->stream, a, a.blk_begin, P->data->gram16 ? (const uint16_t *)P->data->gramp16 : (const uint16_t *)nullptr,
+                       pl.fused ? Spec3Train{(const int32_t *)P->data->gdiag, P->qsum3} : Spec3Train{nullptr, nullptr});
     if (std::isinf(a.gate3)) return;
   }
   if (pl.engine == 4) {
@@ -1438,6 +1466,7 @@
                     !(a.flags & (SWF_SELECT | SWF_EM_ANY | SWF_SERIAL)) && P->data->plan.ldsw > 0 && P->data->plan.ldsw <= (size_t)160 * 1024;
   const bool wfx = sw.wfx && (P->data->plan.R % S2W_FXR) == 0 && P->data->plan.K * (P->data->plan.R / S2W_FXR) <= 255;
   pl.engine = pl.gate3 > 0.0f ? 3 : winv ? 4 : P->data->plan.pipelined ? 2 : 1;
+  pl.fused = sw.train && pl.gate3 > 0.0f;
   int lag = 2;
   if (P->data->plan.pipelined && sel) {
     if (P->data->plan.xdist >= 2 && (sw.lag >= 0 || P->data->gram16)) lag = 3;
@@ -1513,6 +1542,7 @@
     const SweepPlan r = plan_sweep(P, a, true);
     for (int i = 0; i < r.nspins; ++i) pl.spins[pl.nspins++] = r.spins[i];
     pl.guarded = true;
+    pl.fused_guard = pl.fused;
   }
   return pl;
 }
@@ -1527,9 +1557,9 @@
   A.dbg = pl.dbg3; A.pf = pl.pf; A.pf2 = pl.pf2; A.qsplit = pl.qsplit; A.skip_vb = pl.skip_vb;
   P->epoch3 = (P->epoch3 + 1) & 0xFFFFFFu; if (P->epoch3 == 0) P->epoch3 = 1;
   A.epoch = P->epoch3;
-  (void)hipMemsetAsync(P->qsum3 + (size_t)a.blk_begin * 2 * SW_MAXM, 0, sizeof(unsigned long long) * 2 * SW_MAXM * (size_t)(a.blk_end - a.blk_begin), P->stream);
-}
-static void launch_sweep_engine(bwgr_panel *P, const SweepArgs &a_in, const SweepPlan &pl, bool redo) {
+  if (!pl.fused) (void)hipMemsetAsync(P->qsum3 + (size_t)a.blk_begin * 2 * SW_MAXM, 0, sizeof(unsigned long long) * 2 * SW_MAXM * (size_t)(a.blk_end - a.blk_begin), P->stream);
+}
+static void launch_sweep_engine(bwgr_panel *P, const SweepArgs &a_in, const SweepPlan &pl, bool redo, const SnapArgs *post = nullptr) {
   SweepArgs a = a_in;
   if (P->debug_withhold) a.flags |= SWF_DEBUG_WITHHOLD;
   a.gate3 = pl.gate3; a.redo_only = redo ? 1 : 0;
@@ -1550,7 +1580,9 @@
     void *args[] = {&A3};
     spin_launch(pl.spins[0], P->stream, args);
     if (cen) hipLaunchKernelGGL(k_cen_end, dim3(64), dim3(256), 0, P->stream, a, 0);
-    if (pl.skip_vb) {
+    if (post) {
+      hipLaunchKernelGGL(k_sweep_post, dim3((unsigned)std::max<int64_t>(1, std::min<int64_t>(1024, (post->j1 - post->j0 + 255) / 256))), dim3(256), 0, P->stream, *post, a, pl.skip_vb);
+    } else if (pl.skip_vb) {
       const int j0 = a.blk_begin * a.m, j1 = (int)std::min<int64_t>(P->data->p, (int64_t)a.blk_end * a.m);
       hipLaunchKernelGGL(k_vb_fill, dim3((unsigned)std::min<int64_t>(1024, (j1 - j0 + 255) / 256)), dim3(256), 0, P->stream, a, j0, j1);
     }
@@ -1577,16 +1609,19 @@
   if (cen2) hipLaunchKernelGGL(k_cen_end, dim3(64), dim3(256), 0, P->stream, a, redo ? 2 : 1);
 }
 static void launch_sweep_kernel(bwgr_panel *P, const SweepArgs &a, const SweepPlan &pl) {
-  const size_t p = (size_t)P->data->p;
   bool guarded = pl.guarded;
-  if (guarded && !P->snap_e && !P->own.take({{&P->snap_e, sizeof(double) * (size_t)P->data->plan.ld}, {&P->snap_b, sizeof(float) * p}, {&P->snap_d, sizeof(float) * p}, {&P->snap_vb, sizeof(float) * p}})) guarded = false;
+  if (guarded && !snap_alloc(P)) guarded = false;
+  const bool post = guarded && pl.fused_guard;
+  const bool staged = P->snap_staged; P->snap_staged = false;
   SnapArgs sn;
   sn.e = a.e; sn.se = P->snap_e; sn.b = a.b; sn.d = a.d; sn.vb = (a.flags & SWF_VB_VEC) ? a.vb : nullptr; sn.sb = P->snap_b; sn.sd = P->snap_d; sn.svb = P->snap_vb;
   sn.ld = P->data->plan.ld; sn.j0 = a.blk_begin * a.m; sn.j1 = (int)std::min<int64_t>(P->data->p, (int64_t)a.blk_end * a.m); sn.sc = a.sc;
-  if (guarded) hipLaunchKernelGGL(k_range_snapshot, dim3(256), dim3(256), 0, P->stream, sn);
-  launch_sweep_engine(P, a, pl, false);
+  if (post) {
+    if (!staged) { SnapArgs se = sn; se.j1 = se.j0; hipLaunchKernelGGL(k_range_snapshot, dim3(64), dim3(256), 0, P->stream, se); }
+  } else if (guarded) hipLaunchKernelGGL(k_range_snapshot, dim3(256), dim3(256), 0, P->stream, sn);
+  launch_sweep_engine(P, a, pl, false, post ? &sn : nullptr);
   if (guarded) {
-    hipLaunchKernelGGL(k_range_recover, dim3(256), dim3(256), 0, P->stream, sn);
+    if (!post) hipLaunchKernelGGL(k_range_recover, dim3(256), dim3(256), 0, P->stream, sn);
     hipLaunchKernelGGL(k_range_flag, dim3(1), dim3(1), 0, P->stream, a.sc);
     (void)reset_exchange(P);
     launch_sweep_engine(P, a, plan_sweep(P, a, true), true);
@@ -1751,6 +1786,11 @@
   if (D->is_f32) hipLaunchKernelGGL(k_gram_pack<double>, dim3((unsigned)pl.nblocks), dim3(256), 0, P->stream, (const double *)D->gram, (double *)D->gramp, m, pl.pstride, pl.nblocks);
   else hipLaunchKernelGGL(k_gram_pack<int32_t>, dim3((unsigned)pl.nblocks), dim3(256), 0, P->stream, (const int32_t *)D->gram, (int32_t *)D->gramp, m, pl.pstride, pl.nblocks);
   HIPCHK(hipGetLastError());
+  if (!D->is_f32) {
+    if (!D->gdiag) CHK(own_array(D->own, D->gdiag, (size_t)pl.nblocks * m, "panel_create"));
+    hipLaunchKernelGGL(k_gram_diag, dim3((unsigned)std::max<int64_t>(1, std::min<int64_t>(2048, ((int64_t)pl.nblocks * m + 255) / 256))), dim3(256), 0, P->stream, (const int32_t *)D->gram, D->gdiag, m, (int64_t)pl.nblocks);
+    HIPCHK(hipGetLastError());
+  }
   D->gram16 = false;
   if (pl.has16) {
     HIPCHK(hipMemsetAsync(D->gram16_bad, 0, sizeof(int), P->stream));
diff --git a/bwgr_amd/csrc/sweep.hip.h b/bwgr_amd/csrc/sweep.hip.h
--- a/bwgr_amd/csrc/sweep.hip.h
+++ b/bwgr_amd/csrc/sweep.hip.h
@@ -167,7 +167,9 @@
 #define TILE_COMMIT(dstp, mB_) do { XT *dst_ = (dstp); const int cpr_ = R / PER; const int tot_ = (mB_) * cpr_; \
     const float rcpr_ = 1.0f / (float)cpr_; BWGR_TILE_EACH(BWGR_COMMIT1) } while (0)
 
-__global__ void k_prestage(const SweepArgs a, int j_begin, int j_end) {
+struct StageTail { int dex; float *snap_d; };
+static constexpr StageTail STAGE_TAIL_AS_BEFORE = {1, nullptr};
+__global__ void k_prestage(const SweepArgs a, int j_begin, int j_end, const StageTail tl = STAGE_TAIL_AS_BEFORE) {
   const ChainScalars &sc = *a.sc;
   const float ve = sc.ve, lam_common = sc.lam, dfp1 = sc.dfp1;
   const int64_t nm = j_end - j_begin;
@@ -189,6 +191,7 @@
     const bool sel = (a.flags & SWF_SELECT) != 0;
     if (piece == 0) {
       st.b0[t] = b0;
+      if (tl.snap_d) tl.snap_d[j] = a.d[j];
       st.xxb0[t] = k2 ? b0 : xxj * b0;
       st.rden[t] = 1.0 / (double)den;
       const double sdz1 = (a.flags & SWF_EM_BL) ? 1.0 / (double)(xxj + sc.Sb)
@@ -247,7 +250,7 @@
     }
   }
   __syncthreads();
-  if (threadIdx.x == 0 && dex_s != 0u) atomicMax(&a.sc->e3_dex, dex_s);
+  if (threadIdx.x == 0 && tl.dex && dex_s != 0u) atomicMax(&a.sc->e3_dex, dex_s);
 }
 __global__ void k_draws(Rng rng, uint32_t marker0, uint32_t iter, int flags, const ChainScalars *sc_in, int64_t p, int j_begin, int j_end, double *out) {
   const float dfp1 = sc_in->dfp1;
@@ -271,7 +274,7 @@
     } else out[4 * (size_t)p + j] = (flags & SWF_VB_VEC) ? rng_chisq(rng, (double)dfp1, mk, iter, RNG_CHI) : 1.0;
   }
 }
-__global__ __launch_bounds__(256) void k_prestage_fin(const SweepArgs a, int j_begin, int j_end) {
+__global__ __launch_bounds__(256) void k_prestage_fin(const SweepArgs a, int j_begin, int j_end, const StageTail tl = STAGE_TAIL_AS_BEFORE) {
   const ChainScalars &sc = *a.sc;
   const float ve = sc.ve, lam_common = sc.lam;
   __shared__ uint32_t dex_s;
@@ -292,6 +295,7 @@
     const float den = k2 ? (xxj * sc.bg + lamj) : (xxj + lamj);
     const float sd = sqrtf(ve / den);
     st.b0[t] = b0;
+    if (tl.snap_d) tl.snap_d[j] = a.d[j];
     st.xxb0[t] = k2 ? b0 : xxj * b0;
     st.rden[t] = 1.0 / (double)den;
     st.sdz1[t] = (double)sd * a.draws[j];
@@ -324,7 +328,7 @@
     }
   }
   __syncthreads();
-  if (threadIdx.x == 0 && dex_s != 0u) atomicMax(&a.sc->e3_dex, dex_s);
+  if (threadIdx.x == 0 && tl.dex && dex_s != 0u) atomicMax(&a.sc->e3_dex, dex_s);
 }
 __device__ inline void stage_block(StageBuf &st, int blk, const SweepArgs &a, int tid0, int nthreads) {
   constexpr int NCH = (int)(sizeof(StageBuf) / 16);
diff --git a/bwgr_amd/csrc/sweep3.hip.h b/bwgr_amd/csrc/sweep3.hip.h
--- a/bwgr_amd/csrc/sweep3.hip.h
+++ b/bwgr_amd/csrc/sweep3.hip.h
@@ -60,13 +60,13 @@
 }
 
 __global__ void k_escale_reset(ChainScalars *sc) { sc->e3_dex = 0u; }
-__global__ __launch_bounds__(1024) void k_escale(const double *e, int64_t ld, ChainScalars *sc, int xbits, float gate3, int sh_add = 0) {
+__global__ __launch_bounds__(1024) void k_escale(const double *e, int64_t ld, ChainScalars *sc, int xbits, float gate3, int sh_add = 0, double *snap_e = nullptr) {
   if (!(sc->inc_rate < gate3)) { if (threadIdx.x == 0) sc->e3_dex = 0u; return; }
   __shared__ uint32_t mx;
   if (threadIdx.x == 0) mx = 0u;
   __syncthreads();
   uint32_t ex = 0u;
-  for (int64_t i = threadIdx.x; i < ld; i += blockDim.x) ex = max(ex, (uint32_t)((__double2hiint(e[i]) & 0x7FFFFFFF) >> 20));
+  for (int64_t i = threadIdx.x; i < ld; i += blockDim.x) { const double ei = e[i]; if (snap_e) snap_e[i] = ei; ex = max(ex, (uint32_t)((__double2hiint(ei) & 0x7FFFFFFF) >> 20)); }
   atomicMax(&mx, ex);
   __syncthreads();
   if (threadIdx.x == 0) {
@@ -76,6 +76,7 @@
     k = max(-200, min(200, k));
     sc->e3_sh = 44 - k + sh_add;
     sc->e3_dex = 0u;
+    if (snap_e) { sc->snap_sum_d = sc->sum_d; sc->snap_sum_b2 = sc->sum_b2; }
   }
 }
 __device__ __forceinline__ double s3_pow2(int k) { return __hiloint2double((1023 + k) << 20, 0); }
@@ -130,7 +131,28 @@
   for (int64_t i = (int64_t)blockIdx.x * blockDim.x + threadIdx.x; i < a.n; i += (int64_t)gridDim.x * blockDim.x) a.e[i] += shift;
 }
 
-__global__ __launch_bounds__(128) void k_spec3(const SweepArgs a, int blk_begin, const uint16_t *gp16 = nullptr) {
+__device__ __forceinline__ void spec3_tri(const uint16_t *Gp, const double *dr, int j, int m, double &s0, double &s1, double &s2, double &s3) {
+  int k = 0;
+  int pr = 0;
+  for (; k + 4 <= j; k += 4) {
+    const int p0 = pr, p1 = p0 + (m - 2 - k), p2 = p1 + (m - 3 - k), p3 = p2 + (m - 4 - k);
+    s0 = fma((double)Gp[p0], dr[k], s0);
+    s1 = fma((double)Gp[p1], dr[k + 1], s1);
+    s2 = fma((double)Gp[p2], dr[k + 2], s2);
+    s3 = fma((double)Gp[p3], dr[k + 3], s3);
+    pr = p3 + (m - 5 - k);
+  }
+  for (; k < j; ++k) { s0 = fma((double)Gp[pr], dr[k], s0); pr += m - 2 - k; }
+}
+struct Spec3Train { const int32_t *gdiag; unsigned long long *qz; };
+__global__ void k_gram_diag(const int32_t *gram, int32_t *gdiag, int m, int64_t nblocks) {
+  const int64_t total = nblocks * m;
+  for (int64_t t = (int64_t)blockIdx.x * blockDim.x + threadIdx.x; t < total; t += (int64_t)gridDim.x * blockDim.x) {
+    const int64_t blk = t / m; const int j = (int)(t - blk * m);
+    gdiag[t] = gram[((size_t)blk * m + j) * m + j];
+  }
+}
+__global__ __launch_bounds__(128) void k_spec3(const SweepArgs a, int blk_begin, const uint16_t *gp16 = nullptr, const Spec3Train tr = Spec3Train{nullptr, nullptr}) {
   if (!(a.sc->inc_rate < a.gate3)) return;
   const int blk = blk_begin + blockIdx.x, j = threadIdx.x, m = a.m;
   const int mB = min(m, a.p - blk * m);
@@ -138,6 +160,10 @@
   SpecBuf &sp = a.ps.spec[blk];
   __shared__ double dr[128];
   __shared__ double cs[128];
+  if (tr.qz) {
+    ulonglong2 *qz = reinterpret_cast<ulonglong2 *>(tr.qz + (size_t)blk * 2 * SW_MAXM);
+    for (int t = j; t < SW_MAXM; t += 128) qz[t] = make_ulonglong2(0ull, 0ull);
+  }
   const bool cen = (a.flags & SWF_CENTRE) != 0;
   const int sh = a.sc->e3_sh;
   const double S = s3_pow2(sh), invS = s3_pow2(-sh);
@@ -147,20 +173,10 @@
   __syncthreads();
   double s0 = 0.0, s1 = 0.0, s2 = 0.0, s3 = 0.0, gjj = 0.0, ib = 0.0;
   if (j < mB) {
-    gjj = (double)G[(size_t)j * m + j];
+    gjj = (double)(tr.gdiag ? tr.gdiag[(size_t)blk * m + j] : G[(size_t)j * m + j]);
     int k = 0;
     if (gp16) {
-      const uint16_t *Gp = gp16 + (size_t)blk * a.pstride + (j - 1);
-      int pr = 0;
-      for (; k + 4 <= j; k += 4) {
-        const int p0 = pr, p1 = p0 + (m - 2 - k), p2 = p1 + (m - 3 - k), p3 = p2 + (m - 4 - k);
-        s0 = fma((double)Gp[p0], dr[k], s0);
-        s1 = fma((double)Gp[p1], dr[k + 1], s1);
-        s2 = fma((double)Gp[p2], dr[k + 2], s2);
-        s3 = fma((double)Gp[p3], dr[k + 3], s3);
-        pr = p3 + (m - 5 - k);
-      }
-      for (; k < j; ++k) { s0 = fma((double)Gp[pr], dr[k], s0); pr += m - 2 - k; }
+      spec3_tri(gp16 + (size_t)blk * a.pstride + (j - 1), dr, j, m, s0, s1, s2, s3);
     } else {
     for (; k + 4 <= j; k += 4) {
       s0 = fma((double)G[(size_t)k * m + j], dr[k], s0);
@@ -175,7 +191,7 @@
   double spec = (s0 + s1) + (s2 + s3);
   if (cen) {
     spec -= ((double)sj * a.ninv) * (a.cpre[blk] + ib);
-    gjj = __hiloint2double(sj, (j < mB) ? (int)G[(size_t)j * m + j] : 0);
+    gjj = __hiloint2double(sj, (j < mB) ? (int)(tr.gdiag ? tr.gdiag[(size_t)blk * m + j] : G[(size_t)j * m + j]) : 0);
   }
   sp.spec[j] = spec; sp.xspec[j] = 0.0; sp.gjj[j] = gjj;
 }
```

Result: no change. 108.3 iter/s, median of 6 (+0.5%).
